# ubc-vision/quadraturefields

Measured on AMD Instinct MI355X. Metric: rays/sec at 800x800 Lego (mesh-quadrature render: ray/mesh intersection + hash-grid/MLP field + compositing), higher is better.
Workload: dtype f32; 1 GPU; Lego 800x800 (configs[1]), 1xMI355X per frame, fp32 hash-grid + tiny-MLP HIP kernels; rays_per_frame=640000, max_hits=25, triangles=983040, log2_hashmap_size=19, up_sample=1, bvh_fallback_frames=0, overflow_repaired_frames=8, reorigin_rule_redone_frames=0, camera_mismatch_frames=0, frames_in_flight=1

## Files before the change

include/qf_hip.h:

```cpp
#ifndef QF_HIP_H
#define QF_HIP_H

#include <stdint.h>

#ifdef __cplusplus
extern "C" {
#endif

#define QF_OK 0
#define QF_ERR_INVALID_ARGUMENT (-1)
#define QF_ERR_HIP (-2)
#define QF_ERR_UNSUPPORTED (-3)
#define QF_ERR_NO_DEVICE (-4)

#define QF_ABI_VERSION 6
#define QF_MAX_LEVELS 16
#define QF_MAX_LOBES 8

const char *qf_status_string(int status);
int qf_abi_version(void);
int qf_device_cu_count(void);

typedef struct qf_grid_desc {
    uint32_t n_levels;
    uint32_t n_features;
    uint32_t log2_hashmap_size;
    uint32_t base_resolution;
    float per_level_scale;
    uint32_t hashed_mask;
    uint32_t offset[QF_MAX_LEVELS + 1];
    uint32_t resolution[QF_MAX_LEVELS];
    float scale[QF_MAX_LEVELS];
} qf_grid_desc;

int qf_grid_desc_init(qf_grid_desc *desc , uint32_t n_levels,
                      uint32_t log2_hashmap_size, uint32_t base_resolution,
                      double per_level_scale);

int qf_grid_encode(const qf_grid_desc *desc , const float *table ,
                   const float *x01, int64_t n, float *out , void *stream);

int qf_grid_encode_backward(const qf_grid_desc *desc , const float *table, const float *x01,
                            const float *dfeat, int64_t n, float *grad_table, float *grad_x01, void *stream);
int64_t qf_grid_backward_workspace_bytes(int64_t n);
int qf_grid_encode_backward_ws(const qf_grid_desc *desc, const float *table, const float *x01,
                               const float *dfeat, int64_t n, float *grad_table, float *grad_x01,
                               void *workspace, int64_t workspace_bytes, void *stream);

int qf_grid_encode_double_backward(const qf_grid_desc *desc , const float *table, const float *x01,
                                   const float *dfeat, const float *v, int64_t n, float *g_dfeat,
                                   float *g_x01, float *grad_table,
                                   void *workspace ,
                                   int64_t workspace_bytes, void *stream);

int qf_grid_mlp_forward(const qf_grid_desc *grid , const float *table, const float *base_w,
                        const float *x01, int64_t n, float *out16, void *stream);

#define QF_HEAD_NONE 0
#define QF_HEAD_NGP 1
#define QF_HEAD_SG 2
#define QF_HEAD_SG_FEATURES 3

typedef struct qf_field_desc {
    qf_grid_desc grid;
    float aabb[6];
    int32_t head;
    int32_t n_lobes;
} qf_field_desc;

typedef struct qf_sg_head {
    const float *w1, *b1, *w2, *b2, *wout, *bout;
} qf_sg_head;

int qf_field_forward(const qf_field_desc *desc , const float *table,
                     const float *base_w, const float *head_ngp_w, const qf_sg_head *head_sg ,
                     const float *xyz, const float *dirs, int64_t n, const int64_t *n_device, const int32_t *order,
                     float *rgb, float *sigma, float *geo, float *features,
                     float *enc_out ,
                     void *stream);

typedef struct qf_sg_head_bf16 {
    const uint16_t *w1, *b1, *w2;
    const float *b2;
    const uint16_t *wout;
    const float *bout;
} qf_sg_head_bf16;
int qf_field_forward_bf16(const qf_field_desc *desc , const uint16_t *table ,
                          const uint16_t *base_w, const uint16_t *head_ngp_w,
                          const qf_sg_head_bf16 *head_sg , const float *xyz, const float *dirs,
                          int64_t n, const int64_t *n_device, const int32_t *order, float *rgb, float *sigma, float *geo,
                          void *stream);

typedef qf_sg_head_bf16 qf_sg_head_f16;
int qf_field_forward_f16(const qf_field_desc *desc , const uint16_t *table ,
                         const uint16_t *base_w, const uint16_t *head_ngp_w,
                         const qf_sg_head_f16 *head_sg , const float *xyz, const float *dirs,
                         int64_t n, const int64_t *n_device, const int32_t *order, float *rgb, float *sigma, float *geo,
                         void *stream);

int qf_ngp_mlp_backward(const float *enc , const float *dirs , const uint8_t *selector,
                        const float *d_rgb, const float *d_sigma, const float *base_w, const float *head_w,
                        int64_t n, float *d_enc , float *grad_base_w, float *grad_head_w,
                        void *stream);

int qf_sg_mlp_backward(const float *enc , const uint8_t *selector, const float *d_features,
                       int64_t d_stride, const float *d_sigma, const float *base_w,
                       const qf_sg_head *head , int32_t n_lobes, int64_t n, float *d_enc,
                       float *grad_base_w, const qf_sg_head *grad_head ,
                       void *stream);

int qf_sg_features_to_rgb(const float *features, int64_t feat_stride, const float *dirs,
                          int64_t n, int32_t n_lobes, float *rgb, void *stream);
int qf_sg_features_to_rgb_backward(const float *features, int64_t feat_stride, const float *dirs,
                                   const float *d_rgb, int64_t n, int32_t n_lobes, float *d_features,
                                   int64_t d_stride, void *stream);

int qf_deform_field_forward(const qf_grid_desc *grid , const float *table, float scale,
                            int32_t hidden, const float *w1, const float *b1, const float *w2,
                            const float *b2, const float *wout, const float *bout,
                            const float *xyz, int64_t n, const int64_t *n_device ,
                            const int32_t *order, float *out , float *enc_out ,
                            void *stream);

int qf_deform_field_forward_f16(const qf_grid_desc *grid , const uint16_t *table ,
                                float scale, int32_t hidden, const float *w1, const float *b1, const float *w2,
                                const float *b2, const float *wout, const float *bout,
                                const float *xyz, int64_t n, const int64_t *n_device, const int32_t *order,
                                float *out , float *enc_out , void *stream);

#define QF_ACT_RELU 0
#define QF_ACT_ELU 1
int qf_field_grid_extract(const qf_grid_desc *grid , const float *table, float scale, int32_t hidden,
                          int32_t activation, const float *w1, const float *b1, const float *w2, const float *b2,
                          const float *wout, const float *bout, const float *axis, int32_t n, int32_t x_begin,
                          int32_t x_count, int32_t pool, const float *xyz, int64_t n_points, const int64_t *n_device,
                          float *value, uint16_t *grad_norm, void *stream);

int qf_field_grid_extract_f16(const qf_grid_desc *grid , const uint16_t *table, float scale, int32_t hidden,
                              int32_t activation, const float *w1, const float *b1, const float *w2, const float *b2,
                              const float *wout, const float *bout, const float *axis, int32_t n, int32_t x_begin,
                              int32_t x_count, int32_t pool, const float *xyz, int64_t n_points,
                              const int64_t *n_device, float *value, uint16_t *grad_norm, void *stream);

int qf_deform_mlp_backward(const float *enc, const float *x01, const float *d_out, const float *w1,
                           const float *b1, const float *w2, const float *b2, const float *wout, int64_t n,
                           float *d_enc, float *d_x01, float *g_w1, float *g_b1, float *g_w2, float *g_b2,
                           float *g_wout, float *g_bout, void *stream);

int qf_adam_step(float *param, const float *grad, float *exp_avg, float *exp_avg_sq, int64_t n, double lr, double beta1,
                 double beta2, double eps, double weight_decay, int32_t maximize, int64_t step, void *stream);

int qf_apply_deformation(const float *f , float scaling, const float *dirs, const float *xyz ,
                         const float *ts , int64_t n, float *xyz_out, float *ts_out, float *dh_out,
                         void *stream);

int qf_mark_pack_boundaries(const int64_t *ridx, int64_t n, uint8_t *boundary ,
                            void *stream);
int qf_exponential_integration(const float *feats , int32_t c, const float *tau ,
                               const int64_t *seg_start, int64_t n_seg, int64_t n, int32_t exclusive,
                               float *out , float *weights , void *stream);
int qf_sum_reduce(const float *feats , int32_t c, const int64_t *seg_start,
                  int64_t n_seg, int64_t n, float *out , void *stream);

#define QF_BG_WHITE 0
#define QF_BG_BLACK 1
#define QF_BG_CUSTOM 2
#define QF_BG_NONE 3
int qf_derive_properties(const float *rgb_s , const float *sigma ,
                         const float *depth , const float *deltas ,
                         float delta_const, const int64_t *index_ray , int64_t n,
                         int64_t n_rays, int32_t bg_mode, const float *bkgd ,
                         const int32_t *sample_index, float *out_rgb, float *out_alpha, float *out_depth,
                         float *weights, void *stream);

int qf_derive_properties_backward(const float *rgb_s, const float *sigma, const float *depth,
                                  const float *deltas , float delta_const,
                                  const int64_t *index_ray, int64_t n, int64_t n_rays, int32_t bg_mode,
                                  const float *bkgd , const float *g_rgb,
                                  const float *g_alpha, const float *g_depth, float *grad_rgb_s,
                                  float *grad_sigma, float *grad_depth, void *stream);

int qf_pack_info(const int64_t *ray_indices , int64_t n, int64_t n_rays,
                 int64_t *packed_info , void *stream);
int qf_exclusive_scan(const float *x, const int64_t *packed_info, int64_t n_rays, int64_t n,
                      int32_t mode, float *out, void *stream);
int qf_accumulate_along_rays(const float *weights, const float *values ,
                             int32_t c, const int64_t *packed_info, int64_t n_rays, int64_t n,
                             float *out , void *stream);
int qf_render_from_density(const float *t_starts, const float *t_ends, const float *sigmas,
                           const float *rgbs , const int64_t *packed_info,
                           int64_t n_rays, int64_t n, const float *bkgd ,
                           float *weights, float *trans, float *alphas, float *colors,
                           float *opacities, float *depths, void *stream);

typedef struct qf_bvh qf_bvh;

int qf_bvh_create(const float *tri_verts , int64_t n_tri, qf_bvh **out);
int qf_bvh_create_ex(const float *tri_verts , int64_t n_tri, int32_t sah_depth, qf_bvh **out);
int qf_bvh_refit(qf_bvh *bvh, const float *tri_verts , int64_t n_tri);
int qf_bvh_refit_device(qf_bvh *bvh, const float *d_tri_verts , int64_t n_tri, void *stream);
void qf_bvh_destroy(qf_bvh *bvh);
int64_t qf_bvh_num_triangles(const qf_bvh *bvh);
int64_t qf_bvh_num_nodes(const qf_bvh *bvh);
int64_t qf_bvh_num_wide_nodes(const qf_bvh *bvh);
int32_t qf_bvh_max_depth(const qf_bvh *bvh);
int32_t qf_bvh_max_stack(const qf_bvh *bvh);
int qf_bvh_copy_nodes(const qf_bvh *bvh, float *nodes_host, int64_t capacity_nodes);
int qf_bvh_copy_wide_nodes(const qf_bvh *bvh, float *nodes_host, int64_t capacity_nodes);
int qf_bvh_copy_tri_ids(const qf_bvh *bvh, int32_t *ids_host, int64_t capacity);

int qf_bvh_set_min_separation(qf_bvh *bvh, float min_separation);
float qf_bvh_min_separation(const qf_bvh *bvh);

int qf_bvh_intersect(const qf_bvh *bvh, const float *rays_o, const float *rays_d, int64_t n_rays,
                     int32_t max_hits, int32_t image_width, int32_t *hit_tri, float *hit_t,
                     int32_t *hit_count, void *stream);
int qf_filter_hits(const qf_bvh *bvh, int64_t n_rays, int32_t max_hits, int32_t *hit_tri, float *hit_t,
                   int32_t *hit_count, void *stream);

typedef struct qf_camera {
    float c2w[12];
    float fx, fy;
    float cx, cy;
    int32_t width, height;
} qf_camera;
int qf_raster_intersect(qf_bvh *bvh, const qf_camera *cam , const float *rays_o,
                        const float *rays_d, int64_t n_rays, int32_t max_hits, int32_t *hit_tri, float *hit_t,
                        int32_t *hit_count, int32_t *overflow, int32_t sort_lists, int32_t cull_chunks,
                        int32_t *ray_flag, void *stream);
int qf_raster_intersect_wide(qf_bvh *bvh, const qf_camera *cam , const float *rays_o,
                             const float *rays_d, int64_t n_rays, int32_t max_hits, int32_t wide_hits,
                             int32_t *wide_tri, float *wide_t, int32_t *hit_tri, float *hit_t, int32_t *hit_count,
                             int32_t *overflow, int32_t cull_chunks, int32_t *ray_flag, void *stream);
int qf_raster_intersect_slabs(qf_bvh *bvh, const qf_camera *cam , const float *rays_o, const float *rays_d,
                              int64_t n_rays, int32_t max_hits, int32_t wide_hits, int32_t n_slabs, uint64_t *wide_keys,
                              int32_t *hit_tri, float *hit_t, int32_t *hit_count, int32_t *overflow, int32_t *ray_flag,
                              void *stream);
int qf_bvh_repair_overflow(const qf_bvh *bvh, const float *rays_o, const float *rays_d, int64_t n_rays,
                           int32_t max_hits, int32_t image_width, int32_t *hit_tri, float *hit_t,
                           int32_t *hit_count, uint64_t *keep_mask, int32_t *raw_count,
                           const int32_t *traverse_all_flag, void *stream);

int qf_grid_march_count(const float *aabb, const int32_t *resolution, const uint8_t *binaries,
                        const float *rays_o, const float *rays_d, const float *t_min, const float *t_max,
                        int64_t n_rays, float near_plane, float far_plane, float step, int32_t *count, void *stream);
int qf_grid_march_write(const float *aabb, const int32_t *resolution, const uint8_t *binaries,
                        const float *rays_o, const float *rays_d, const float *t_min, const float *t_max,
                        int64_t n_rays, float near_plane, float far_plane, float step, const int64_t *offsets,
                        float *t_starts, float *t_ends, int64_t *ray_indices, void *stream);

int qf_generate_rays(const qf_camera *cam , int32_t opengl, float *origins, float *viewdirs, void *stream);

int qf_scatter_max(const float *values, const int64_t *index, int64_t n, int64_t n_out, float *out, void *stream);

#define QF_UNTOUCHED_LAST_FACE 0
#define QF_UNTOUCHED_ZERO 1
int64_t qf_texel_positions_workspace_bytes(int64_t n_faces, int32_t height, int32_t width);
int qf_texel_positions(const double *vertices, int64_t n_vertices, const int64_t *faces, int64_t n_faces,
                       const double *uv, int32_t height, int32_t width, int32_t untouched, float *out,
                       int64_t *tri_size, void *workspace, int64_t workspace_bytes, void *stream);

int64_t qf_marching_cubes_workspace_bytes(int64_t n0, int64_t n1, int64_t n2);
int qf_marching_cubes_count(const float *volume, int64_t n0, int64_t n1, int64_t n2, float level, void *workspace,
                            int64_t workspace_bytes, int64_t *counts, void *stream);
int qf_marching_cubes_emit(const float *volume, int64_t n0, int64_t n1, int64_t n2, float level,
                           const void *workspace, int64_t workspace_bytes, float *verts, int64_t n_verts,
                           int32_t *faces, int64_t n_faces, void *stream);

#define QF_CLUSTER_AVERAGE 0
#define QF_CLUSTER_QUADRIC 1
int64_t qf_vertex_clustering_workspace_bytes(int64_t n_vertices, int64_t n_faces);
int qf_vertex_clustering_count(const double *vertices, int64_t n_vertices, const int64_t *faces, int64_t n_faces,
                               double voxel_size, void *workspace, int64_t workspace_bytes, int64_t *counts,
                               void *stream);
int qf_vertex_clustering_emit(const double *vertices, int64_t n_vertices, const int64_t *faces, int64_t n_faces,
                              double voxel_size, int contraction, void *workspace, int64_t workspace_bytes,
                              double *out_vertices, int64_t n_out_vertices, int64_t *out_faces, int64_t n_out_faces,
                              int64_t *n_fallback, void *stream);

int64_t qf_frame_offsets_temp_bytes(int64_t n_rays);
int qf_frame_offsets(const int32_t *hit_count, int64_t n_rays, int32_t max_hits, int32_t width, int32_t height,
                     int64_t *ray_offset , int64_t *tile_base , void *temp,
                     int64_t temp_bytes, const int32_t *overflow_in, const int32_t *ray_flag_in, int64_t *host_out,
                     int32_t band_rows, void *stream);
int64_t qf_banded_tile_count(int32_t width, int32_t height, int32_t band_rows);

int qf_tile_offsets(const int32_t *hit_count, int32_t max_hits, int32_t width, int32_t height, int64_t *tile_base,
                    int64_t *total, const int32_t *overflow_in, const int32_t *ray_flag_in, int64_t *host_out,
                    int32_t *zero_word , void *stream);

int qf_pack_samples(const float *rays_o, const float *rays_d, int64_t n_rays, int32_t max_hits,
                    const int32_t *hit_tri, const float *hit_t, const int32_t *hit_count,
                    const int64_t *ray_offset, float *xyz, float *dirs, int64_t *index_ray,
                    float *depth, int64_t *index_tri, float *origins, const int32_t *inverse,
                    float *xyz_c, float *dirs_c, float *depth_c , const uint64_t *keep_mask,
                    const int32_t *raw_count, float min_separation, int32_t *close_flag, void *stream);

int qf_pack_tiles(const float *rays_o, const float *rays_d, int32_t width, int32_t height, int32_t max_hits,
                  const int32_t *hit_tri, const float *hit_t, const int32_t *hit_count, const int64_t *tile_base,
                  const int64_t *total, float *xyz_c, float *dirs_c, float *depth_c, int32_t *tri_c ,
                  const uint64_t *keep_mask, const int32_t *raw_count, float min_separation, int32_t *final_count,
                  int32_t *dropped, int64_t *host_out,
                  int32_t dropped_is_zero ,
                  void *stream);

int qf_tile_totals(const int32_t *hit_count, int32_t width, int32_t height, int64_t *tile_total, void *stream);
int qf_coherent_layout(const int32_t *hit_count, const int64_t *ray_offset, const int64_t *tile_base,
                       int32_t width, int32_t height, int32_t *order, int32_t *inverse,
                       int32_t band_rows , void *stream);

int qf_composite_tiles(const float *rgb_c , const float *sigma_c , const float *depth_c ,
                       float delta_const, const int32_t *hit_count , int32_t max_hits,
                       const int64_t *tile_base, int32_t width, int32_t height, int32_t bg_mode,
                       const float *bkgd , float *out_rgb, float *out_alpha, float *out_depth,
                       float *weights_c, float *out_packed, void *stream);

int qf_row_sample_counts(const int32_t *hit_count, int32_t max_hits, int32_t width, int32_t height, float *out_rows,
                         void *stream);

#define QF_FIELD_FP32 0
#define QF_FIELD_BF16 1
#define QF_FIELD_FP16 2
typedef struct qf_frame_job {
    const qf_camera *camera;
    const float *rays_o, *rays_d;
    int64_t n_rays;
    int32_t max_hits;
    int32_t cull_chunks;
    float min_separation;
    int32_t bg_mode;
    float delta_const;
    int32_t field_precision;
    int32_t *hit_tri;
    float *hit_t;
    int32_t *hit_count;
    int32_t *final_count;
    int64_t *tile_base;
    int64_t *total;
    int64_t *host_block;
    int32_t *dropped;
    float *xyz_c, *dirs_c, *depth_c;
    int32_t *tri_c;
    const qf_field_desc *field;
    const void *table, *base_w, *head_ngp_w;
    const void *head_sg;
    float *rgb_c, *sigma_c;
    const float *bkgd;
    float *out_rgb, *out_alpha, *out_depth, *out_packed;
} qf_frame_job;
int qf_frame_render(qf_bvh *bvh, const qf_frame_job *job , void *stream);

int qf_deform_resort_tiles(const float *f_c, float scaling, const float *xyz_c, const float *dirs_c,
                           const float *depth_c, const int32_t *hit_count, int32_t max_hits, const int64_t *tile_base,
                           int64_t total , const int64_t *total_device ,
                           int32_t width, int32_t height, float *xyz_out, float *depth_out, void *stream);

int qf_resort_by_depth(const int64_t *index_ray, const float *depth, int64_t n, int64_t *perm,
                       void *stream);

int qf_resort_samples(const int64_t *index_ray, const float *depth, int64_t n, const float *points,
                      const float *origins, const float *vectors, const int64_t *index_tri,
                      int64_t *perm, float *out_points, float *out_depth, float *out_origins,
                      float *out_vectors, int64_t *out_index_tri, uint8_t *boundary, const int32_t *inverse,
                      float *out_points_c, float *out_vectors_c, void *stream);

int qf_split_layout(const int64_t *index_ray, int64_t n, int32_t width, int32_t height, int32_t *hit_count,
                    int64_t *ray_offset, int64_t *tile_base, int32_t *invalid, int32_t *order, int32_t *inverse,
                    void *stream);

int qf_mesh_update_d(const float *d , const float *w , const int64_t *index_tri, int64_t n,
                     int64_t n_faces, float *cache , int32_t *skipped , void *stream);

typedef struct qf_texture_set {
    const uint8_t *alpha;
    const uint8_t *diffuse;
    const uint8_t *colors[QF_MAX_LOBES];
    const uint8_t *lambda_axis[QF_MAX_LOBES];
    int32_t texture_size;
    int32_t n_lobes;
    int32_t sigmoid_codec;
    float lambda_thres;
} qf_texture_set;

#define QF_TEXEL_TRIANGLE_RECORD_BYTES 128
int qf_texel_records_pack(const double *vertices, const int64_t *faces, const float *uv, int64_t n_faces,
                          void *records, void *stream);
int qf_texel_indices_packed(const void *records, const float *points, const int64_t *index_tri, int64_t n,
                            int32_t texture_size, int64_t *texel, void *stream);
int qf_texture_fetch(const qf_texture_set *tex , const int64_t *texel, int64_t n,
                     float *features, void *stream);

#define QF_TEXEL_RECORD_BYTES 64
int qf_texture_pack(const qf_texture_set *tex , uint8_t *records, void *stream);
int qf_texture_shade_packed(const uint8_t *records, int32_t texture_size, int32_t n_lobes,
                            int32_t sigmoid_codec, float lambda_thres, const int64_t *texel,
                            const float *dirs, int64_t n, float *rgb, float *sigma, void *stream);
int qf_texture_shade_points(const uint8_t *records, int32_t texture_size, int32_t n_lobes, int32_t sigmoid_codec,
                            float lambda_thres, const void *triangle_records, const float *points,
                            const int64_t *index_tri, const int32_t *index_tri32, const float *dirs, int64_t n,
                            const int64_t *n_device, float *rgb, float *sigma, void *stream);

#ifdef __cplusplus
}
#endif
#endif
```

quadraturefields_amd/_C.py:

```python
import ctypes
import os
from ctypes import POINTER, Structure, c_char_p, c_double, c_float, c_int, c_int32, c_int64, c_uint8, c_uint32, c_void_p

import torch

_PKG = os.path.dirname(os.path.abspath(__file__))
LIB_PATH = os.environ.get("QF_HIP_LIBRARY") or os.path.join(_PKG, "libqf_hip.so")

QF_MAX_LEVELS = 16
QF_MAX_LOBES = 8
QF_BVH_MAX_HITS = 64
QF_TEXEL_RECORD_BYTES = 64
QF_TEXEL_TRIANGLE_RECORD_BYTES = 128
HEAD_NONE, HEAD_NGP, HEAD_SG, HEAD_SG_FEATURES = 0, 1, 2, 3
FIELD_FP32, FIELD_BF16, FIELD_FP16 = 0, 1, 2
UNTOUCHED_LAST_FACE, UNTOUCHED_ZERO = 0, 1
BG_WHITE, BG_BLACK, BG_CUSTOM, BG_NONE = 0, 1, 2, 3


class GridDesc(Structure):
    _fields_ = [
        ("n_levels", c_uint32), ("n_features", c_uint32), ("log2_hashmap_size", c_uint32),
        ("base_resolution", c_uint32), ("per_level_scale", c_float), ("hashed_mask", c_uint32),
        ("offset", c_uint32 * (QF_MAX_LEVELS + 1)), ("resolution", c_uint32 * QF_MAX_LEVELS),
        ("scale", c_float * QF_MAX_LEVELS),
    ]


class FieldDesc(Structure):
    _fields_ = [("grid", GridDesc), ("aabb", c_float * 6), ("head", c_int32), ("n_lobes", c_int32)]


class SGHead(Structure):
    _fields_ = [("w1", c_void_p), ("b1", c_void_p), ("w2", c_void_p), ("b2", c_void_p),
                ("wout", c_void_p), ("bout", c_void_p)]


class Camera(Structure):
    _fields_ = [("c2w", c_float * 12), ("fx", c_float), ("fy", c_float), ("cx", c_float), ("cy", c_float),
                ("width", c_int32), ("height", c_int32)]


class FrameJob(Structure):
    _fields_ = [("camera", c_void_p), ("rays_o", c_void_p), ("rays_d", c_void_p), ("n_rays", c_int64),
                ("max_hits", c_int32), ("cull_chunks", c_int32), ("min_separation", c_float), ("bg_mode", c_int32),
                ("delta_const", c_float), ("field_precision", c_int32),
                ("hit_tri", c_void_p), ("hit_t", c_void_p), ("hit_count", c_void_p), ("final_count", c_void_p),
                ("tile_base", c_void_p), ("total", c_void_p), ("host_block", c_void_p), ("dropped", c_void_p),
                ("xyz_c", c_void_p), ("dirs_c", c_void_p), ("depth_c", c_void_p), ("tri_c", c_void_p),
                ("field", c_void_p), ("table", c_void_p), ("base_w", c_void_p), ("head_ngp_w", c_void_p),
                ("head_sg", c_void_p), ("rgb_c", c_void_p), ("sigma_c", c_void_p),
                ("bkgd", c_void_p), ("out_rgb", c_void_p), ("out_alpha", c_void_p), ("out_depth", c_void_p),
                ("out_packed", c_void_p)]


class TextureSet(Structure):
    _fields_ = [("alpha", c_void_p), ("diffuse", c_void_p), ("colors", c_void_p * QF_MAX_LOBES),
                ("lambda_axis", c_void_p * QF_MAX_LOBES), ("texture_size", c_int32), ("n_lobes", c_int32),
                ("sigmoid_codec", c_int32), ("lambda_thres", c_float)]


_P = c_void_p
_SIGNATURES = {
    "qf_status_string": (c_char_p, [c_int]),
    "qf_frame_render": (c_int, [_P, POINTER(FrameJob), _P]),
    "qf_abi_version": (c_int, []),
    "qf_device_cu_count": (c_int, []),
    "qf_grid_desc_init": (c_int, [POINTER(GridDesc), c_uint32, c_uint32, c_uint32, c_double]),
    "qf_grid_encode": (c_int, [POINTER(GridDesc), _P, _P, c_int64, _P, _P]),
    "qf_grid_encode_backward": (c_int, [POINTER(GridDesc), _P, _P, _P, c_int64, _P, _P, _P]),
    "qf_grid_backward_workspace_bytes": (c_int64, [c_int64]),
    "qf_grid_encode_backward_ws": (c_int, [POINTER(GridDesc), _P, _P, _P, c_int64, _P, _P, _P, c_int64, _P]),
    "qf_grid_encode_double_backward": (c_int, [POINTER(GridDesc), _P, _P, _P, _P, c_int64, _P, _P, _P, _P, c_int64, _P]),
    "qf_grid_mlp_forward": (c_int, [POINTER(GridDesc), _P, _P, _P, c_int64, _P, _P]),
    "qf_field_forward": (c_int, [POINTER(FieldDesc), _P, _P, _P, POINTER(SGHead), _P, _P, c_int64, _P, _P, _P, _P, _P, _P, _P, _P]),
    "qf_field_forward_bf16": (c_int, [POINTER(FieldDesc), _P, _P, _P, POINTER(SGHead), _P, _P, c_int64, _P, _P, _P, _P, _P, _P]),
    "qf_field_forward_f16": (c_int, [POINTER(FieldDesc), _P, _P, _P, POINTER(SGHead), _P, _P, c_int64, _P, _P, _P, _P, _P, _P]),
    "qf_ngp_mlp_backward": (c_int, [_P, _P, _P, _P, _P, _P, _P, c_int64, _P, _P, _P, _P]),
    "qf_sg_mlp_backward": (c_int, [_P, _P, _P, c_int64, _P, _P, POINTER(SGHead), c_int32, c_int64, _P, _P, POINTER(SGHead), _P]),
    "qf_sg_features_to_rgb": (c_int, [_P, c_int64, _P, c_int64, c_int32, _P, _P]),
    "qf_sg_features_to_rgb_backward": (c_int, [_P, c_int64, _P, _P, c_int64, c_int32, _P, c_int64, _P]),
    "qf_deform_field_forward": (c_int, [POINTER(GridDesc), _P, c_float, c_int32, _P, _P, _P, _P, _P, _P, _P, c_int64, _P, _P, _P, _P, _P]),
    "qf_deform_field_forward_f16": (c_int, [POINTER(GridDesc), _P, c_float, c_int32, _P, _P, _P, _P, _P, _P, _P, c_int64, _P, _P, _P, _P, _P]),
    "qf_field_grid_extract": (c_int, [POINTER(GridDesc), _P, c_float, c_int32, c_int32, _P, _P, _P, _P, _P, _P, _P, c_int32, c_int32, c_int32, c_int32, _P, c_int64, _P, _P, _P, _P]),
    "qf_field_grid_extract_f16": (c_int, [POINTER(GridDesc), _P, c_float, c_int32, c_int32, _P, _P, _P, _P, _P, _P, _P, c_int32, c_int32, c_int32, c_int32, _P, c_int64, _P, _P, _P, _P]),
    "qf_deform_mlp_backward": (c_int, [_P, _P, _P, _P, _P, _P, _P, _P, c_int64, _P, _P, _P, _P, _P, _P, _P, _P, _P]),
    "qf_adam_step": (c_int, [_P, _P, _P, _P, c_int64, c_double, c_double, c_double, c_double, c_double, c_int32, c_int64, _P]),
    "qf_apply_deformation": (c_int, [_P, c_float, _P, _P, _P, c_int64, _P, _P, _P, _P]),
    "qf_mark_pack_boundaries": (c_int, [_P, c_int64, _P, _P]),
    "qf_exponential_integration": (c_int, [_P, c_int32, _P, _P, c_int64, c_int64, c_int32, _P, _P, _P]),
    "qf_sum_reduce": (c_int, [_P, c_int32, _P, c_int64, c_int64, _P, _P]),
    "qf_derive_properties": (c_int, [_P, _P, _P, _P, c_float, _P, c_int64, c_int64, c_int32, _P, _P, _P, _P, _P, _P, _P]),
    "qf_deform_resort_tiles": (c_int, [_P, c_float, _P, _P, _P, _P, c_int32, _P, c_int64, _P, c_int32, c_int32, _P, _P, _P]),
    "qf_composite_tiles": (c_int, [_P, _P, _P, c_float, _P, c_int32, _P, c_int32, c_int32, c_int32, _P, _P, _P, _P, _P, _P, _P]),
    "qf_row_sample_counts": (c_int, [_P, c_int32, c_int32, c_int32, _P, _P]),
    "qf_derive_properties_backward": (c_int, [_P, _P, _P, _P, c_float, _P, c_int64, c_int64, c_int32, _P, _P, _P, _P, _P, _P, _P, _P]),
    "qf_pack_info": (c_int, [_P, c_int64, c_int64, _P, _P]),
    "qf_exclusive_scan": (c_int, [_P, _P, c_int64, c_int64, c_int32, _P, _P]),
    "qf_accumulate_along_rays": (c_int, [_P, _P, c_int32, _P, c_int64, c_int64, _P, _P]),
    "qf_render_from_density": (c_int, [_P, _P, _P, _P, _P, c_int64, c_int64, _P, _P, _P, _P, _P, _P, _P, _P]),
    "qf_bvh_create": (c_int, [_P, c_int64, POINTER(c_void_p)]),
    "qf_bvh_create_ex": (c_int, [_P, c_int64, c_int32, POINTER(c_void_p)]),
    "qf_bvh_refit": (c_int, [_P, _P, c_int64]),
    "qf_bvh_refit_device": (c_int, [_P, _P, c_int64, _P]),
    "qf_bvh_num_wide_nodes": (c_int64, [_P]),
    "qf_bvh_max_stack": (c_int32, [_P]),
    "qf_bvh_copy_wide_nodes": (c_int, [_P, _P, c_int64]),
    "qf_bvh_set_min_separation": (c_int, [_P, c_float]),
    "qf_bvh_min_separation": (c_float, [_P]),
    "qf_filter_hits": (c_int, [_P, c_int64, c_int32, _P, _P, _P, _P]),
    "qf_bvh_destroy": (None, [_P]),
    "qf_bvh_num_triangles": (c_int64, [_P]),
    "qf_bvh_num_nodes": (c_int64, [_P]),
    "qf_bvh_max_depth": (c_int32, [_P]),
    "qf_bvh_copy_nodes": (c_int, [_P, _P, c_int64]),
    "qf_bvh_copy_tri_ids": (c_int, [_P, _P, c_int64]),
    "qf_bvh_intersect": (c_int, [_P, _P, _P, c_int64, c_int32, c_int32, _P, _P, _P, _P]),
    "qf_bvh_repair_overflow": (c_int, [_P, _P, _P, c_int64, c_int32, c_int32, _P, _P, _P, _P, _P, _P, _P]),
    "qf_raster_intersect": (c_int, [_P, POINTER(Camera), _P, _P, c_int64, c_int32, _P, _P, _P, _P, c_int32, c_int32, _P, _P]),
    "qf_raster_intersect_wide": (c_int, [_P, POINTER(Camera), _P, _P, c_int64, c_int32, c_int32, _P, _P, _P, _P, _P, _P, c_int32, _P,
                                         _P]),
    "qf_raster_intersect_slabs": (c_int, [_P, POINTER(Camera), _P, _P, c_int64, c_int32, c_int32, c_int32, _P, _P, _P, _P, _P, _P,
                                          _P]),
    "qf_grid_march_count": (c_int, [POINTER(c_float), POINTER(c_int32), _P, _P, _P, _P, _P, c_int64, c_float, c_float,
                                    c_float, _P, _P]),
    "qf_grid_march_write": (c_int, [POINTER(c_float), POINTER(c_int32), _P, _P, _P, _P, _P, c_int64, c_float, c_float,
                                    c_float, _P, _P, _P, _P, _P]),
    "qf_generate_rays": (c_int, [POINTER(Camera), c_int32, _P, _P, _P]),
    "qf_scatter_max": (c_int, [_P, _P, c_int64, c_int64, _P, _P]),
    "qf_texel_positions_workspace_bytes": (c_int64, [c_int64, c_int32, c_int32]),
    "qf_texel_positions": (c_int, [_P, c_int64, _P, c_int64, _P, c_int32, c_int32, c_int32, _P, _P, _P, c_int64, _P]),
    "qf_marching_cubes_workspace_bytes": (c_int64, [c_int64, c_int64, c_int64]),
    "qf_marching_cubes_count": (c_int, [_P, c_int64, c_int64, c_int64, c_float, _P, c_int64, _P, _P]),
    "qf_marching_cubes_emit": (c_int, [_P, c_int64, c_int64, c_int64, c_float, _P, c_int64, _P, c_int64, _P, c_int64, _P]),
    "qf_vertex_clustering_workspace_bytes": (c_int64, [c_int64, c_int64]),
    "qf_vertex_clustering_count": (c_int, [_P, c_int64, _P, c_int64, c_double, _P, c_int64, _P, _P]),
    "qf_vertex_clustering_emit": (c_int, [_P, c_int64, _P, c_int64, c_double, c_int, _P, c_int64, _P, c_int64, _P, c_int64,
                                          _P, _P]),
    "qf_frame_offsets_temp_bytes": (c_int64, [c_int64]),
    "qf_frame_offsets": (c_int, [_P, c_int64, c_int32, c_int32, c_int32, _P, _P, _P, c_int64, _P, _P, _P, c_int32, _P]),
    "qf_banded_tile_count": (c_int64, [c_int32, c_int32, c_int32]),
    "qf_tile_offsets": (c_int, [_P, c_int32, c_int32, c_int32, _P, _P, _P, _P, _P, _P, _P]),
    "qf_pack_tiles": (c_int, [_P, _P, c_int32, c_int32, c_int32, _P, _P, _P, _P, _P, _P, _P, _P, _P, _P, _P, c_float, _P, _P, _P, c_int32, _P]),
    "qf_pack_samples": (c_int, [_P, _P, c_int64, c_int32, _P, _P, _P, _P, _P, _P, _P, _P, _P, _P, _P, _P, _P, _P, _P, _P, c_float, _P, _P]),
    "qf_tile_totals": (c_int, [_P, c_int32, c_int32, _P, _P]),
    "qf_coherent_layout": (c_int, [_P, _P, _P, c_int32, c_int32, _P, _P, c_int32, _P]),
    "qf_resort_by_depth": (c_int, [_P, _P, c_int64, _P, _P]),
    "qf_resort_samples": (c_int, [_P, _P, c_int64, _P, _P, _P, _P, _P, _P, _P, _P, _P, _P, _P, _P, _P, _P, _P]),
    "qf_split_layout": (c_int, [_P, c_int64, c_int32, c_int32, _P, _P, _P, _P, _P, _P, _P]),
    "qf_mesh_update_d": (c_int, [_P, _P, _P, c_int64, c_int64, _P, _P, _P]),
    "qf_texel_records_pack": (c_int, [_P, _P, _P, c_int64, _P, _P]),
    "qf_texel_indices_packed": (c_int, [_P, _P, _P, c_int64, c_int32, _P, _P]),
    "qf_texture_fetch": (c_int, [POINTER(TextureSet), _P, c_int64, _P, _P]),
    "qf_texture_pack": (c_int, [POINTER(TextureSet), _P, _P]),
    "qf_texture_shade_packed": (c_int, [_P, c_int32, c_int32, c_int32, c_float, _P, _P, c_int64, _P, _P, _P]),
    "qf_texture_shade_points": (c_int, [_P, c_int32, c_int32, c_int32, c_float, _P, _P, _P, _P, _P, c_int64, _P, _P, _P, _P]),
}
EXPORTED_SYMBOLS = tuple(_SIGNATURES)
ABI_VERSION = 6

_lib = None


def lib() -> ctypes.CDLL:
    global _lib
    if _lib is None:
        if not os.path.exists(LIB_PATH):
            raise RuntimeError(
                f"{LIB_PATH} is missing: build it with `python -m quadraturefields_amd.build` "
                "(hipcc --offload-arch=gfx950).  quadraturefields_amd has no CPU fallback.")
        handle = ctypes.CDLL(LIB_PATH)
        for name, (restype, argtypes) in _SIGNATURES.items():
            fn = getattr(handle, name)
            fn.restype = restype
            fn.argtypes = argtypes
        version = handle.qf_abi_version()
        experiment = os.environ.get("QF_HIP_LIBRARY_EXPERIMENT") == "1" and version == ABI_VERSION + 1000
        if version != ABI_VERSION and not experiment:
            raise RuntimeError(f"{LIB_PATH}: ABI version {version}, expected {ABI_VERSION} (an experiment build "
                               "reports +1000 and is only loaded with QF_HIP_LIBRARY_EXPERIMENT=1)")
        _lib = handle
    return _lib


class QFError(RuntimeError):
    pass


def check(status: int, what: str = "") -> None:
    if status != 0:
        msg = lib().qf_status_string(status).decode()
        if status == -1:
            raise ValueError(f"{what}: {msg}")
        raise QFError(f"{what}: {msg} (status {status})")


def ptr(t, dtype=None, device_required: bool = True):
    if t is None:
        return None
    if not isinstance(t, torch.Tensor):
        raise TypeError("expected a torch.Tensor")
    if dtype is not None and t.dtype != dtype:
        raise TypeError(f"expected dtype {dtype}, got {t.dtype}")
    if not t.is_contiguous():
        raise ValueError("tensor must be contiguous")
    if device_required and not t.is_cuda:
        raise RuntimeError("quadraturefields_amd kernels need tensors on the HIP device (no CPU fallback)")
    return c_void_p(t.data_ptr())


_OWNER_PID = os.getpid()
_FORKED = False


def _after_fork_in_child():
    global _FORKED
    _FORKED = True


os.register_at_fork(after_in_child=_after_fork_in_child)


def raw_stream() -> int:
    return torch._C._cuda_getCurrentRawStream(torch._C._cuda_getDevice())


def stream():
    if _FORKED:
        raise RuntimeError(
            "quadraturefields_amd was called from a forked child process (a DataLoader worker?): the HIP kernels must run "
            f"in the process that imported the package (pid {_OWNER_PID}).  Use num_workers=0 for the device path, or a "
            "'spawn' multiprocessing context.")
    return c_void_p(raw_stream())


def resolve_device(device) -> torch.device:
    dev = torch.device(device)
    if dev.type == "cuda" and dev.index is None:
        dev = torch.device("cuda", torch.cuda.current_device())
    return dev


def f32c(t: torch.Tensor) -> torch.Tensor:
    return t.to(torch.float32).contiguous()


def i64c(t: torch.Tensor) -> torch.Tensor:
    return t.to(torch.int64).contiguous()


def make_grid_desc(n_levels: int, log2_hashmap_size: int, base_resolution: int, per_level_scale: float) -> GridDesc:
    d = GridDesc()
    check(lib().qf_grid_desc_init(ctypes.byref(d), n_levels, log2_hashmap_size, base_resolution,
                                  float(per_level_scale)), "qf_grid_desc_init")
    return d


def grid_encode_backward(desc, table, x01, dfeat, n: int, grad_table, grad_x01) -> None:
    ws, ws_bytes = None, 0
    if grad_table is not None and n >= (1 << 15):
        ws_bytes = int(lib().qf_grid_backward_workspace_bytes(n))
        ws = torch.empty((ws_bytes,), dtype=torch.uint8, device=x01.device)
    check(lib().qf_grid_encode_backward_ws(desc, ptr(table), ptr(x01), ptr(dfeat), n, ptr(grad_table), ptr(grad_x01),
                                           ptr(ws), ws_bytes, stream()), "qf_grid_encode_backward")
```

quadraturefields_amd/csrc/frame.cpp:

```cpp
#include "qf_common.h"

extern "C" int qf_frame_render(qf_bvh *bvh, const qf_frame_job *job, void *stream)
{
    if (!bvh || !job || !job->camera) return QF_ERR_INVALID_ARGUMENT;
    const qf_frame_job &j = *job;
    const int32_t w = j.camera->width, h = j.camera->height;
    if (w < 1 || h < 1 || j.n_rays != (int64_t)w * h || j.max_hits < 1) return QF_ERR_INVALID_ARGUMENT;
    if (!j.rays_o || !j.rays_d || !j.hit_tri || !j.hit_t || !j.hit_count || !j.final_count || !j.tile_base || !j.total ||
        !j.dropped || !j.xyz_c || !j.dirs_c || !j.depth_c)
        return QF_ERR_INVALID_ARGUMENT;
    if (j.field_precision < QF_FIELD_FP32 || j.field_precision > QF_FIELD_FP16) return QF_ERR_INVALID_ARGUMENT;
    if (j.field) {
        const qf_field_desc &f = *j.field;
        if (!j.rgb_c || !j.sigma_c || !j.table || !j.base_w) return QF_ERR_INVALID_ARGUMENT;
        if (f.head == QF_HEAD_NGP) {
            if (!j.head_ngp_w) return QF_ERR_INVALID_ARGUMENT;
        } else if (f.head == QF_HEAD_SG) {
            if (!j.head_sg) return QF_ERR_INVALID_ARGUMENT;
            if (j.field_precision == QF_FIELD_FP32) {
                const qf_sg_head *s = static_cast<const qf_sg_head *>(j.head_sg);
                if (!s->w1 || !s->b1 || !s->w2 || !s->b2 || !s->wout || !s->bout) return QF_ERR_INVALID_ARGUMENT;
            } else {
                const qf_sg_head_bf16 *s = static_cast<const qf_sg_head_bf16 *>(j.head_sg);
                if (!s->w1 || !s->b1 || !s->w2 || !s->b2 || !s->wout || !s->bout) return QF_ERR_INVALID_ARGUMENT;
            }
            if (f.n_lobes < 1 || f.n_lobes > QF_MAX_LOBES) return QF_ERR_UNSUPPORTED;
        } else {
            return QF_ERR_INVALID_ARGUMENT;
        }
        for (int k = 0; k < 3; ++k)
            if (!(f.aabb[3 + k] > f.aabb[k])) return QF_ERR_INVALID_ARGUMENT;
        if (j.bg_mode < 0 || j.bg_mode > 3) return QF_ERR_INVALID_ARGUMENT;
        if (!j.out_packed && (!j.out_rgb || !j.out_alpha || !j.out_depth)) return QF_ERR_INVALID_ARGUMENT;
        if (j.bg_mode == QF_BG_CUSTOM && !j.bkgd) return QF_ERR_INVALID_ARGUMENT;
    }
    const int64_t cap = j.n_rays * (int64_t)j.max_hits;
    int32_t *overflow = j.hit_count + j.n_rays;
    int rc = qf_raster_intersect(bvh, j.camera, j.rays_o, j.rays_d, j.n_rays, j.max_hits, j.hit_tri, j.hit_t, j.hit_count,
                                 overflow, j.tri_c ? 0 : 2 , j.cull_chunks,
                                 overflow + 1, stream);
    if (rc != QF_OK) return rc;
    rc = qf_bvh_repair_overflow(bvh, j.rays_o, j.rays_d, j.n_rays, j.max_hits, w, j.hit_tri, j.hit_t, j.hit_count, nullptr,
                                nullptr, overflow + 1, stream);
    if (rc != QF_OK) return rc;
    rc = qf_tile_offsets(j.hit_count, j.max_hits, w, h, j.tile_base, j.total, overflow, overflow + 1, j.host_block, j.dropped,
                         stream);
    if (rc != QF_OK) return rc;
    rc = qf_pack_tiles(j.rays_o, j.rays_d, w, h, j.max_hits, j.hit_tri, j.hit_t, j.hit_count, j.tile_base, j.total, j.xyz_c,
                       j.dirs_c, j.depth_c, j.tri_c, nullptr, nullptr, j.min_separation, j.final_count, j.dropped, nullptr, 1,
                       stream);
    if (rc != QF_OK) return rc;
    if (!j.field) return QF_OK;
    if (j.field_precision == QF_FIELD_FP32) {
        rc = qf_field_forward(j.field, static_cast<const float *>(j.table), static_cast<const float *>(j.base_w),
                              static_cast<const float *>(j.head_ngp_w), static_cast<const qf_sg_head *>(j.head_sg),
                              j.xyz_c, j.dirs_c, cap, j.total, nullptr, j.rgb_c, j.sigma_c, nullptr, nullptr, nullptr,
                              stream);
    } else {
        auto fwd = j.field_precision == QF_FIELD_BF16 ? qf_field_forward_bf16 : qf_field_forward_f16;
        rc = fwd(j.field, static_cast<const uint16_t *>(j.table), static_cast<const uint16_t *>(j.base_w),
                 static_cast<const uint16_t *>(j.head_ngp_w), static_cast<const qf_sg_head_bf16 *>(j.head_sg), j.xyz_c,
                 j.dirs_c, cap, j.total, nullptr, j.rgb_c, j.sigma_c, nullptr, stream);
    }
    if (rc != QF_OK) return rc;
    return qf_composite_tiles(j.rgb_c, j.sigma_c, j.depth_c, j.delta_const, j.final_count, j.max_hits, j.tile_base, w, h,
                              j.bg_mode, j.bkgd, j.out_rgb, j.out_alpha, j.out_depth, nullptr, j.out_packed, stream);
}
```

quadraturefields_amd/csrc/raster.hip:

```cpp
#include <type_traits>

#include "exact_common.h"

#pragma clang fp contract(off)

namespace {

struct RasterCam {
    float r00, r01, r02, r10, r11, r12, r20, r21, r22;
    float cx, cy, cz;
    float fx, fy, px0, py0;
    int w, h;
};

constexpr float kRasterGuard = 0.25f;

struct SlabArgs {
    float t_lo, t_hi;
    int stop_at;
    uint64_t *keys;
    const float4 *ray_rec;
};

struct TriSetup {
    int x0, x1, y0, y1;
    bool use_edges;
    float ea[3], eb[3], ec[3];
};

__device__ __forceinline__ bool tri_setup(const float4 a, const float4 b, const float4 c, const RasterCam &cam, TriSetup &s)
{
    float minx = INFINITY, maxx = -INFINITY, miny = INFINITY, maxy = -INFINITY;
    int behind = 0;
    const float4 vs[3] = {a, b, c};
    float sxs[3], sys[3];
#pragma unroll
    for (int k = 0; k < 3; ++k) {
        const float dx = vs[k].x - cam.cx, dy = vs[k].y - cam.cy, dz = vs[k].z - cam.cz;
        const float xc = cam.r00 * dx + cam.r10 * dy + cam.r20 * dz;
        const float yc = cam.r01 * dx + cam.r11 * dy + cam.r21 * dz;
        const float zc = cam.r02 * dx + cam.r12 * dy + cam.r22 * dz;
        const float zv = -zc;
        if (!(zv > 1e-6f)) { ++behind; sxs[k] = sys[k] = 0.0f; continue; }
        const float sx = cam.fx * (xc / zv) + cam.px0;
        const float sy = -cam.fy * (yc / zv) + cam.py0;
        sxs[k] = sx; sys[k] = sy;
        minx = fminf(minx, sx); maxx = fmaxf(maxx, sx);
        miny = fminf(miny, sy); maxy = fmaxf(maxy, sy);
    }
    if (behind == 3) return false;
    s.use_edges = false;
    if (behind > 0) {
        s.x0 = 0; s.y0 = 0; s.x1 = cam.w - 1; s.y1 = cam.h - 1;
    } else {
        s.x0 = (int)fmaxf(floorf(minx - kRasterGuard), 0.0f);
        s.y0 = (int)fmaxf(floorf(miny - kRasterGuard), 0.0f);
        s.x1 = (int)fminf(ceilf(maxx + kRasterGuard), (float)(cam.w - 1));
        s.y1 = (int)fminf(ceilf(maxy + kRasterGuard), (float)(cam.h - 1));
        if (!(maxx + kRasterGuard >= 0.0f) || !(maxy + kRasterGuard >= 0.0f) ||
            !(minx - kRasterGuard <= (float)(cam.w - 1)) || !(miny - kRasterGuard <= (float)(cam.h - 1)))
            return false;
        const float area2 = (sxs[1] - sxs[0]) * (sys[2] - sys[0]) - (sys[1] - sys[0]) * (sxs[2] - sxs[0]);
        if (fabsf(area2) > 1e-2f) {
            s.use_edges = true;
            const float sgn = area2 > 0.0f ? 1.0f : -1.0f;
#pragma unroll
            for (int k = 0; k < 3; ++k) {
                const int k1 = (k + 1) % 3;
                const float ex = sxs[k1] - sxs[k], ey = sys[k1] - sys[k];
                s.ea[k] = -sgn * ey;
                s.eb[k] = sgn * ex;
                s.ec[k] = -(s.ea[k] * sxs[k] + s.eb[k] * sys[k]) + (kRasterGuard + 0.05f) * (fabsf(ex) + fabsf(ey)) + 1e-3f;
            }
        }
    }
    return true;
}

template <int kRasterLanes, bool kWide, bool kSlab = false>
__device__ __forceinline__ void raster_triangle(const float4 *__restrict__ tris, int64_t tri_i, int sub, const RasterCam &cam,
                                                const float *__restrict__ rays_o, const float *__restrict__ rays_d,
                                                int max_hits, int32_t *__restrict__ hit_tri, float *__restrict__ hit_t,
                                                int32_t *__restrict__ hit_count, int32_t *__restrict__ overflow,
                                                const bool cam_origin, const SlabArgs slab = SlabArgs())
{
    const float4 a = tris[tri_i * 3 + 0], b = tris[tri_i * 3 + 1], c = tris[tri_i * 3 + 2];
    const int id = __float_as_int(a.w);
    TriSetup ts;
    if (!tri_setup(a, b, c, cam, ts)) return;
    const int x0 = ts.x0, x1 = ts.x1, y0 = ts.y0, y1 = ts.y1;
    const bool use_edges = ts.use_edges;
    const float *ea = ts.ea, *eb = ts.eb, *ec = ts.ec;
    const int bw = x1 - x0 + 1;
    const int total = bw * (y1 - y0 + 1);
    int px = x0 + sub % bw, py = y0 + sub / bw;
    for (int q = sub; q < total; q += kRasterLanes) {
        const int cx_ = px, cy_ = py;
        px += kRasterLanes;
        while (px > x1) { px -= bw; ++py; }
        if (use_edges) {
            const float fx_ = (float)cx_, fy_ = (float)cy_;
            if (ea[0] * fx_ + eb[0] * fy_ + ec[0] < 0.0f || ea[1] * fx_ + eb[1] * fy_ + ec[1] < 0.0f ||
                ea[2] * fx_ + eb[2] * fy_ + ec[2] < 0.0f)
                continue;
        }
        const int64_t ray = (int64_t)cy_ * cam.w + cx_;
        float dx, dy, dz;
        if (kSlab && slab.ray_rec) {
            const float4 rr = slab.ray_rec[ray];
            if (__float_as_int(rr.w) >= slab.stop_at) continue;
            dx = rr.x; dy = rr.y; dz = rr.z;
        } else {
            dx = rays_d[ray * 3]; dy = rays_d[ray * 3 + 1]; dz = rays_d[ray * 3 + 2];
        }
        float ox = cam.cx, oy = cam.cy, oz = cam.cz;
        if (!cam_origin) { ox = rays_o[ray * 3]; oy = rays_o[ray * 3 + 1]; oz = rays_o[ray * 3 + 2]; }
        asm volatile("" : "+v"(ox), "+v"(oy), "+v"(oz), "+v"(dx), "+v"(dy), "+v"(dz));
        float t;
        if (!mt_hit(a, b, c, ox, oy, oz, dx, dy, dz, &t)) continue;
        if (kSlab) {
            if (!(t >= slab.t_lo && t < slab.t_hi)) continue;
            const int slot = atomicAdd(&hit_count[ray], 1);
            if (slot < max_hits) slab.keys[(int64_t)slot * ((int64_t)cam.w * cam.h) + ray] = hit_key(t, id);
            else atomicAdd(overflow, 1);
            continue;
        }
        const int slot = atomicAdd(&hit_count[ray], 1);
        if (slot < max_hits) {
            const int64_t at = kWide ? (int64_t)slot * ((int64_t)cam.w * cam.h) + ray : ray * max_hits + slot;
            hit_t[at] = t;
            if (hit_tri) hit_tri[at] = id;
        } else {
            atomicAdd(overflow, 1);
        }
    }
}

template <int kRasterLanes, bool kWide>
__global__ __launch_bounds__(256) void raster_kernel(const float4 *__restrict__ tris, int64_t n_tri, RasterCam cam,
                                                     const float *__restrict__ rays_o, const float *__restrict__ rays_d,
                                                     int max_hits, int32_t *__restrict__ hit_tri, float *__restrict__ hit_t,
                                                     int32_t *__restrict__ hit_count, int32_t *__restrict__ overflow,
                                                     const int32_t *__restrict__ ray_flag)
{
    const int64_t gid = (int64_t)blockIdx.x * blockDim.x + threadIdx.x;
    const int64_t tri_i = gid / kRasterLanes;
    const int sub = (int)(gid % kRasterLanes);
    if (tri_i >= n_tri) return;
    if (ray_flag && *ray_flag) return;
    const bool cam_origin = ray_flag != nullptr;
    raster_triangle<kRasterLanes, kWide>(tris, tri_i, sub, cam, rays_o, rays_d, max_hits, hit_tri, hit_t, hit_count, overflow,
                                         cam_origin);
}

constexpr float kRayPixelTol = 0.02f;
constexpr float kRayUnitTol = 1e-4f;

__device__ __forceinline__ void camera_rays_check(const uint32_t *__restrict__ o_bits, const float *__restrict__ rays_d,
                                                  int64_t n_rays, const RasterCam &cam, int32_t *__restrict__ flag,
                                                  int64_t first, int64_t stride)
{
    const uint32_t c0 = __float_as_uint(cam.cx), c1 = __float_as_uint(cam.cy), c2 = __float_as_uint(cam.cz);
    bool bad = false;
    for (int64_t r = first; r < n_rays; r += stride) {
        const uint32_t o0 = o_bits[r * 3], o1 = o_bits[r * 3 + 1], o2 = o_bits[r * 3 + 2];
        const float dx = rays_d[r * 3], dy = rays_d[r * 3 + 1], dz = rays_d[r * 3 + 2];
        bad = bad || o0 != c0 || o1 != c1 || o2 != c2;
        const float xc = cam.r00 * dx + cam.r10 * dy + cam.r20 * dz;
        const float yc = cam.r01 * dx + cam.r11 * dy + cam.r21 * dz;
        const float zv = -(cam.r02 * dx + cam.r12 * dy + cam.r22 * dz);
        const float sx = cam.fx * (xc / zv) + cam.px0, sy = -cam.fy * (yc / zv) + cam.py0;
        const float px = (float)(int)(r % cam.w), py = (float)(int)(r / cam.w);
        bad = bad || !(zv > 0.0f) || !(fabsf(sx - px) <= kRayPixelTol) || !(fabsf(sy - py) <= kRayPixelTol) ||
              !(fabsf(dx * dx + dy * dy + dz * dz - 1.0f) <= kRayUnitTol);
    }
    if (bad) *flag = 1;
}

__global__ void camera_rays_check_kernel(const uint32_t *__restrict__ o_bits, const float *__restrict__ rays_d, int64_t n_rays,
                                         RasterCam cam, int32_t *__restrict__ flag)
{
    camera_rays_check(o_bits, rays_d, n_rays, cam, flag, (int64_t)blockIdx.x * blockDim.x + threadIdx.x,
                      (int64_t)gridDim.x * blockDim.x);
}

constexpr int kCullChunk = 64;

__global__ __launch_bounds__(256) void chunk_boxes_kernel(const float4 *__restrict__ tris, int64_t n_tri, int n_chunks,
                                                          float4 *__restrict__ boxes)
{
    const int chunk = (int)(((int64_t)blockIdx.x * blockDim.x + threadIdx.x) >> 6), lane = threadIdx.x & 63;
    if (chunk >= n_chunks) return;
    const int64_t t = (int64_t)chunk * kCullChunk + lane;
    float lo[3] = {INFINITY, INFINITY, INFINITY}, hi[3] = {-INFINITY, -INFINITY, -INFINITY};
    if (t < n_tri) {
#pragma unroll
        for (int k = 0; k < 3; ++k) {
            const float4 v = tris[t * 3 + k];
            lo[0] = fminf(lo[0], v.x); lo[1] = fminf(lo[1], v.y); lo[2] = fminf(lo[2], v.z);
            hi[0] = fmaxf(hi[0], v.x); hi[1] = fmaxf(hi[1], v.y); hi[2] = fmaxf(hi[2], v.z);
        }
    }
#pragma unroll
    for (int off = 32; off > 0; off >>= 1) {
#pragma unroll
        for (int k = 0; k < 3; ++k) {
            lo[k] = fminf(lo[k], __shfl_xor(lo[k], off, 64));
            hi[k] = fmaxf(hi[k], __shfl_xor(hi[k], off, 64));
        }
    }
    if (lane == 0) {
        boxes[chunk * 2 + 0] = make_float4(lo[0], lo[1], lo[2], 0.0f);
        boxes[chunk * 2 + 1] = make_float4(hi[0], hi[1], hi[2], 0.0f);
    }
}

__global__ void cull_chunks_kernel(const float4 *__restrict__ boxes, int n_chunks, RasterCam cam, int32_t *__restrict__ visible,
                                   int32_t *__restrict__ counters, int parity, const uint32_t *__restrict__ o_bits,
                                   const float *__restrict__ rays_d, int64_t n_rays, int32_t *__restrict__ ray_flag)
{
    const int chunk = blockIdx.x * blockDim.x + threadIdx.x;
    if (chunk == 0) counters[parity ^ 1] = 0;
    if (ray_flag) camera_rays_check(o_bits, rays_d, n_rays, cam, ray_flag, chunk, (int64_t)gridDim.x * blockDim.x);
    if (chunk >= n_chunks) return;
    const float4 lo = boxes[chunk * 2], hi = boxes[chunk * 2 + 1];
    if (!(lo.x <= hi.x)) return;
    float minx = INFINITY, maxx = -INFINITY, miny = INFINITY, maxy = -INFINITY;
    bool keep = false;
#pragma unroll
    for (int k = 0; k < 8; ++k) {
        const float dx = ((k & 1) ? hi.x : lo.x) - cam.cx, dy = ((k & 2) ? hi.y : lo.y) - cam.cy, dz = ((k & 4) ? hi.z : lo.z) - cam.cz;
        const float xc = cam.r00 * dx + cam.r10 * dy + cam.r20 * dz;
        const float yc = cam.r01 * dx + cam.r11 * dy + cam.r21 * dz;
        const float zc = cam.r02 * dx + cam.r12 * dy + cam.r22 * dz;
        const float zv = -zc;
        if (!(zv > 1e-4f)) { keep = true; continue; }
        const float sx = cam.fx * (xc / zv) + cam.px0, sy = -cam.fy * (yc / zv) + cam.py0;
        minx = fminf(minx, sx); maxx = fmaxf(maxx, sx);
        miny = fminf(miny, sy); maxy = fmaxf(maxy, sy);
    }
    const float g = kRasterGuard + 1.0f;
    if (!keep)
        keep = (maxx + g >= 0.0f) && (maxy + g >= 0.0f) && (minx - g <= (float)(cam.w - 1)) && (miny - g <= (float)(cam.h - 1));
    if (keep) visible[atomicAdd(&counters[parity], 1)] = chunk;
}

template <int kRasterLanes, bool kWide>
__global__ __launch_bounds__(256) void raster_culled_kernel(const float4 *__restrict__ tris, int64_t n_tri, RasterCam cam,
                                                            const float *__restrict__ rays_o, const float *__restrict__ rays_d,
                                                            int max_hits, int32_t *__restrict__ hit_tri, float *__restrict__ hit_t,
                                                            int32_t *__restrict__ hit_count, int32_t *__restrict__ overflow,
                                                            const int32_t *__restrict__ visible, const int32_t *__restrict__ n_visible,
                                                            const int32_t *__restrict__ ray_flag)
{
    if (ray_flag && *ray_flag) return;
    const bool cam_origin = ray_flag != nullptr;
    constexpr int kTrisPerBlock = 256 / kRasterLanes;
    constexpr int kBlocksPerChunk = kCullChunk / kTrisPerBlock;
    const int n_items = *n_visible * kBlocksPerChunk;
    const int sub = threadIdx.x % kRasterLanes;
    for (int item = blockIdx.x; item < n_items; item += gridDim.x) {
        const int chunk = visible[item / kBlocksPerChunk];
        const int64_t tri_i = (int64_t)chunk * kCullChunk + (item % kBlocksPerChunk) * kTrisPerBlock + threadIdx.x / kRasterLanes;
        if (tri_i < n_tri)
            raster_triangle<kRasterLanes, kWide>(tris, tri_i, sub, cam, rays_o, rays_d, max_hits, hit_tri, hit_t, hit_count, overflow,
                                                 cam_origin);
    }
}

constexpr int kMaxSlabs = 16;

struct SlabCtl {
    uint32_t dist_min_bits, dist_max_bits;
    int32_t n_visible;
    int32_t slab_count[kMaxSlabs];
};

__device__ __forceinline__ void slab_range(const SlabCtl *ctl, int n_slabs, float *lo, float *width)
{
    const float dmin = __uint_as_float(ctl->dist_min_bits) * 0.999f, dmax = __uint_as_float(ctl->dist_max_bits) * 1.001f;
    *lo = dmin;
    *width = fmaxf(dmax - dmin, 1e-12f) / (float)n_slabs;
}

__device__ __forceinline__ void slab_edges(const SlabCtl *ctl, int n_slabs, int j, float *t_lo, float *t_hi)
{
#pragma clang fp contract(off)
    float lo, w;
    slab_range(ctl, n_slabs, &lo, &w);
    *t_lo = j == 0 ? -INFINITY : lo + (float)j * w;
    *t_hi = j == n_slabs - 1 ? INFINITY : lo + (float)(j + 1) * w;
}

__global__ void slab_init_kernel(SlabCtl *ctl)
{
    ctl->dist_min_bits = 0x7f800000u;
    ctl->dist_max_bits = 0u;
    ctl->n_visible = 0;
    for (int j = 0; j < kMaxSlabs; ++j) ctl->slab_count[j] = 0;
}

__global__ void slab_cull_kernel(const float4 *__restrict__ boxes, int n_chunks, RasterCam cam, int32_t *__restrict__ visible,
                                 float2 *__restrict__ range, SlabCtl *ctl)
{
    const int chunk = blockIdx.x * blockDim.x + threadIdx.x;
    if (chunk >= n_chunks) return;
    const float4 lo = boxes[chunk * 2], hi = boxes[chunk * 2 + 1];
    if (!(lo.x <= hi.x)) return;
    float minx = INFINITY, maxx = -INFINITY, miny = INFINITY, maxy = -INFINITY;
    bool keep = false;
#pragma unroll
    for (int k = 0; k < 8; ++k) {
        const float dx = ((k & 1) ? hi.x : lo.x) - cam.cx, dy = ((k & 2) ? hi.y : lo.y) - cam.cy, dz = ((k & 4) ? hi.z : lo.z) - cam.cz;
        const float xc = cam.r00 * dx + cam.r10 * dy + cam.r20 * dz;
        const float yc = cam.r01 * dx + cam.r11 * dy + cam.r21 * dz;
        const float zc = cam.r02 * dx + cam.r12 * dy + cam.r22 * dz;
        const float zv = -zc;
        if (!(zv > 1e-4f)) { keep = true; continue; }
        const float sx = cam.fx * (xc / zv) + cam.px0, sy = -cam.fy * (yc / zv) + cam.py0;
        minx = fminf(minx, sx); maxx = fmaxf(maxx, sx);
        miny = fminf(miny, sy); maxy = fmaxf(maxy, sy);
    }
    const float g = kRasterGuard + 1.0f;
    if (!keep)
        keep = (maxx + g >= 0.0f) && (maxy + g >= 0.0f) && (minx - g <= (float)(cam.w - 1)) && (miny - g <= (float)(cam.h - 1));
    if (!keep) return;
    const float nx = fmaxf(fmaxf(lo.x - cam.cx, cam.cx - hi.x), 0.0f), ny = fmaxf(fmaxf(lo.y - cam.cy, cam.cy - hi.y), 0.0f);
    const float nz = fmaxf(fmaxf(lo.z - cam.cz, cam.cz - hi.z), 0.0f);
    const float fx = fmaxf(fabsf(lo.x - cam.cx), fabsf(hi.x - cam.cx)), fy = fmaxf(fabsf(lo.y - cam.cy), fabsf(hi.y - cam.cy));
    const float fz = fmaxf(fabsf(lo.z - cam.cz), fabsf(hi.z - cam.cz));
    const float dmin = sqrtf(nx * nx + ny * ny + nz * nz) * 0.9999f, dmax = sqrtf(fx * fx + fy * fy + fz * fz) * 1.0001f + 1e-30f;
    visible[atomicAdd(&ctl->n_visible, 1)] = chunk;
    range[chunk] = make_float2(dmin, dmax);
    atomicMin(&ctl->dist_min_bits, __float_as_uint(dmin));
    atomicMax(&ctl->dist_max_bits, __float_as_uint(dmax));
}

__global__ __launch_bounds__(256) void slab_assign_kernel(const int32_t *__restrict__ visible, const float2 *__restrict__ range,
                                                          SlabCtl *ctl, int n_slabs, int n_chunks, int32_t *__restrict__ lists)
{
    __shared__ int s_cnt[kMaxSlabs], s_base[kMaxSlabs];
    if (threadIdx.x < kMaxSlabs) s_cnt[threadIdx.x] = 0;
    __syncthreads();
    const int e = blockIdx.x * blockDim.x + threadIdx.x;
    int chunk = -1, j0 = 0, j1 = -1;
    if (e < ctl->n_visible) {
        chunk = visible[e];
        const float2 r = range[chunk];
        const float dlo = r.x * 0.999f, dhi = r.y * 1.001f;
        j0 = n_slabs;
        for (int j = 0; j < n_slabs; ++j) {
            float t_lo, t_hi;
            slab_edges(ctl, n_slabs, j, &t_lo, &t_hi);
            if (t_hi > dlo && t_lo <= dhi) { j0 = j < j0 ? j : j0; j1 = j; }
        }
        for (int j = j0; j <= j1; ++j) atomicAdd(&s_cnt[j], 1);
    }
    __syncthreads();
    if (threadIdx.x < n_slabs) s_base[threadIdx.x] = s_cnt[threadIdx.x] ? atomicAdd(&ctl->slab_count[threadIdx.x], s_cnt[threadIdx.x]) : 0;
    __syncthreads();
    for (int j = j0; j <= j1; ++j) lists[(int64_t)j * n_chunks + atomicAdd(&s_base[j], 1)] = chunk;
}

__global__ void slab_ray_records_kernel(const float *__restrict__ rays_d, const int32_t *__restrict__ hit_count, int64_t n,
                                        float4 *__restrict__ rec)
{
    for (int64_t i = (int64_t)blockIdx.x * blockDim.x + threadIdx.x; i < n; i += (int64_t)gridDim.x * blockDim.x)
        rec[i] = make_float4(rays_d[i * 3], rays_d[i * 3 + 1], rays_d[i * 3 + 2], __int_as_float(hit_count[i]));
}

template <int kRasterLanes>
__global__ __launch_bounds__(256) void raster_slab_kernel(const float4 *__restrict__ tris, int64_t n_tri, RasterCam cam,
                                                          const float *__restrict__ rays_o, const float *__restrict__ rays_d,
                                                          int capacity, uint64_t *__restrict__ keys, int32_t *__restrict__ hit_count,
                                                          int32_t *__restrict__ overflow, const int32_t *__restrict__ list,
                                                          const SlabCtl *__restrict__ ctl, int slab_j, int n_slabs, int stop_at,
                                                          const float4 *__restrict__ ray_rec,
                                                          const int32_t *__restrict__ ray_flag)
{
    if (ray_flag && *ray_flag) return;
    const bool cam_origin = ray_flag != nullptr;
    constexpr int kTrisPerBlock = 256 / kRasterLanes;
    constexpr int kBlocksPerChunk = kCullChunk / kTrisPerBlock;
    const int n_items = ctl->slab_count[slab_j] * kBlocksPerChunk;
    SlabArgs sa;
    slab_edges(ctl, n_slabs, slab_j, &sa.t_lo, &sa.t_hi);
    sa.stop_at = stop_at;
    sa.keys = keys;
    sa.ray_rec = ray_rec;
    const int sub = threadIdx.x % kRasterLanes;
    for (int item = blockIdx.x; item < n_items; item += gridDim.x) {
        const int chunk = list[item / kBlocksPerChunk];
        const int64_t tri_i = (int64_t)chunk * kCullChunk + (item % kBlocksPerChunk) * kTrisPerBlock + threadIdx.x / kRasterLanes;
        if (tri_i < n_tri)
            raster_triangle<kRasterLanes, true, true>(tris, tri_i, sub, cam, rays_o, rays_d, capacity, nullptr, nullptr,
                                                      hit_count, overflow, cam_origin, sa);
    }
}

constexpr int kSelectBlock = 64;
constexpr int kSelectHeadroom = 8;
__host__ __device__ inline int select_capacity(int max_hits, int wide, float min_sep)
{
    const int cap = min_sep > 0.0f ? max_hits + kSelectHeadroom : max_hits;
    return cap < wide ? cap : wide;
}
__device__ __forceinline__ void write_row_from_keys(const uint64_t *lk, int count, float *row_t, int32_t *row_i)
{
    int i = 0;
    for (; i + 4 <= count; i += 4) {
        f32x4u t4;
        i32x4u i4;
#pragma unroll
        for (int e = 0; e < 4; ++e) {
            const uint64_t k = lk[(i + e) * kSelectBlock];
            t4[e] = key_t(k);
            i4[e] = key_id(k);
        }
        *reinterpret_cast<f32x4u *>(row_t + i) = t4;
        *reinterpret_cast<i32x4u *>(row_i + i) = i4;
    }
    for (; i < count; ++i) {
        const uint64_t k = lk[i * kSelectBlock];
        row_t[i] = key_t(k);
        row_i[i] = key_id(k);
    }
}

template <bool kKeys>
__global__ __launch_bounds__(kSelectBlock) void select_nearest_kernel(int64_t n_rays, int wide, int max_hits, float min_sep,
                                                                      const int32_t *__restrict__ wide_tri,
                                                                      const float *__restrict__ wide_t,
                                                                      const uint64_t *__restrict__ wide_key,
                                                                      int32_t *__restrict__ hit_tri, float *__restrict__ hit_t,
                                                                      int32_t *__restrict__ hit_count)
{
    extern __shared__ __attribute__((aligned(8))) unsigned char select_lds[];
    const int cap = select_capacity(max_hits, wide, min_sep);
    uint64_t *lk = reinterpret_cast<uint64_t *>(select_lds) + threadIdx.x;
    const int64_t r = (int64_t)blockIdx.x * kSelectBlock + threadIdx.x;
    if (r >= n_rays) return;
    const int cnt = hit_count[r];
    if (cnt > wide) return;
    float *row_t = hit_t + r * max_hits;
    int32_t *row_i = hit_tri + r * max_hits;
    if (cnt <= max_hits) {
        constexpr int kCopy = 8;
        for (int i0 = 0; i0 < cnt; i0 += kCopy) {
            float tb[kCopy];
            int ib[kCopy];
#pragma unroll
            for (int u = 0; u < kCopy; ++u) {
                const int i = i0 + u < cnt ? i0 + u : cnt - 1;
                if (kKeys) {
                    const uint64_t k = wide_key[(int64_t)i * n_rays + r];
                    tb[u] = key_t(k);
                    ib[u] = key_id(k);
                } else {
                    tb[u] = wide_t[(int64_t)i * n_rays + r];
                    ib[u] = wide_tri[(int64_t)i * n_rays + r];
                }
            }
#pragma unroll
            for (int q = 0; q < kCopy / 4; ++q) {
                if (i0 + 4 * q + 4 <= cnt) {
                    *reinterpret_cast<f32x4u *>(row_t + i0 + 4 * q) = (f32x4u){tb[4 * q], tb[4 * q + 1], tb[4 * q + 2], tb[4 * q + 3]};
                    *reinterpret_cast<i32x4u *>(row_i + i0 + 4 * q) = (i32x4u){ib[4 * q], ib[4 * q + 1], ib[4 * q + 2], ib[4 * q + 3]};
                } else {
#pragma unroll
                    for (int e = 0; e < 4; ++e)
                        if (i0 + 4 * q + e < cnt) { row_t[i0 + 4 * q + e] = tb[4 * q + e]; row_i[i0 + 4 * q + e] = ib[4 * q + e]; }
                }
            }
        }
        return;
    }
    const int held = cnt < cap ? cnt : cap;
    constexpr int kBatch = 8;
    int n = 0;
    uint64_t max_key = 0;
    for (int i0 = 0; i0 < cnt; i0 += kBatch) {
        uint64_t kb[kBatch];
#pragma unroll
        for (int u = 0; u < kBatch; ++u) {
            const int i = i0 + u < cnt ? i0 + u : cnt - 1;
            if (kKeys) kb[u] = wide_key[(int64_t)i * n_rays + r];
            else kb[u] = hit_key(wide_t[(int64_t)i * n_rays + r], wide_tri[(int64_t)i * n_rays + r]);
        }
#pragma unroll
        for (int u = 0; u < kBatch; ++u) {
            if (i0 + u >= cnt) break;
            const uint64_t key = kb[u];
            int m;
            if (n < held) {
                m = n;
                ++n;
            } else {
                if (!(key < max_key)) continue;
                m = n - 1;
            }
            int lo = 0, hi = m;
            while (lo < hi) {
                const int mid = (lo + hi) >> 1;
                if (lk[mid * kSelectBlock] < key) lo = mid + 1;
                else hi = mid;
            }
            int j = m - 1;
            for (; j - 3 >= lo; j -= 4) {
                const uint64_t a0 = lk[j * kSelectBlock], a1 = lk[(j - 1) * kSelectBlock], a2 = lk[(j - 2) * kSelectBlock],
                               a3 = lk[(j - 3) * kSelectBlock];
                lk[(j + 1) * kSelectBlock] = a0;
                lk[j * kSelectBlock] = a1;
                lk[(j - 1) * kSelectBlock] = a2;
                lk[(j - 2) * kSelectBlock] = a3;
            }
            for (; j >= lo; --j) lk[(j + 1) * kSelectBlock] = lk[j * kSelectBlock];
            lk[lo * kSelectBlock] = key;
            max_key = lk[(n - 1) * kSelectBlock];
        }
    }
    if (min_sep <= 0.0f) {
        write_row_from_keys(lk, max_hits, row_t, row_i);
        hit_count[r] = max_hits;
        return;
    }
    float last_t = key_t(lk[0]);
    int kept = 1;
    for (int i = 1; i < held && kept < max_hits; ++i) {
        const uint64_t k = lk[i * kSelectBlock];
        const float t = key_t(k);
        if (!(t > last_t + min_sep)) continue;
        last_t = t;
        lk[kept * kSelectBlock] = k;
        ++kept;
    }
    if (kept < max_hits && cnt > held) return;
    write_row_from_keys(lk, kept, row_t, row_i);
    hit_count[r] = kept;
}

constexpr int kFilterRays = 128;
__global__ __launch_bounds__(kFilterRays) void filter_hits_kernel(int64_t n_rays, int max_hits, float min_sep,
                                                                  int32_t *__restrict__ hit_tri, float *__restrict__ hit_t,
                                                                  int32_t *__restrict__ hit_count)
{
    extern __shared__ __attribute__((aligned(16))) unsigned char filter_smem[];
    const int K = max_hits, Kp = max_hits | 1;
    float *s_t = reinterpret_cast<float *>(filter_smem);
    int32_t *s_tri = reinterpret_cast<int32_t *>(s_t + kFilterRays * Kp);
    const int tid = threadIdx.x;
    const int64_t ray0 = (int64_t)blockIdx.x * kFilterRays;
    const int nr = (int)((n_rays - ray0) < kFilterRays ? (n_rays - ray0) : kFilterRays);
    for (int i = tid; i < nr * K; i += kFilterRays) {
        const int r = i / K, k = i - r * K;
        s_t[r * Kp + k] = hit_t[ray0 * K + i];
        s_tri[r * Kp + k] = hit_tri[ray0 * K + i];
    }
    __syncthreads();
    if (tid < nr) {
        int cnt = hit_count[ray0 + tid];
        if (cnt > K) cnt = K;
        float *row_t = s_t + tid * Kp;
        int32_t *row_i = s_tri + tid * Kp;
        if (K <= 32) {
            if (cnt > 1) sort_row_32<true>(row_t, row_i, cnt);
        } else {
            for (int i = 1; i < cnt; ++i) {
                const float t = row_t[i];
                const int id = row_i[i];
                int j = i - 1;
                while (j >= 0 && hit_less(t, id, row_t[j], row_i[j])) { row_t[j + 1] = row_t[j]; row_i[j + 1] = row_i[j]; --j; }
                row_t[j + 1] = t;
                row_i[j + 1] = id;
            }
        }
        if (min_sep > 0.0f && cnt > 1) {
            int kept = 1;
            float last_t = row_t[0];
            for (int i = 1; i < cnt; ++i) {
                const float t = row_t[i];
                if (t > last_t + min_sep) { row_t[kept] = t; row_i[kept] = row_i[i]; ++kept; last_t = t; }
            }
            cnt = kept;
        }
        for (int i = cnt; i < K; ++i) { row_t[i] = INFINITY; row_i[i] = -1; }
        hit_count[ray0 + tid] = cnt;
    }
    __syncthreads();
    for (int i = tid; i < nr * K; i += kFilterRays) {
        const int r = i / K, k = i - r * K;
        hit_t[ray0 * K + i] = s_t[r * Kp + k];
        hit_tri[ray0 * K + i] = s_tri[r * Kp + k];
    }
}

}

static int filter_launch(int64_t n_rays, int32_t max_hits, float min_sep, int32_t *hit_tri, float *hit_t,
                         int32_t *hit_count, hipStream_t st)
{
    const int Kp = max_hits | 1;
    const size_t lds = (size_t)kFilterRays * Kp * 8;
    const int64_t blocks = qf_div_up(n_rays, kFilterRays);
    if (blocks > 0x7fffffff) return QF_ERR_UNSUPPORTED;
    hipLaunchKernelGGL(filter_hits_kernel, dim3((unsigned)blocks), dim3(kFilterRays), lds, st, n_rays, (int)max_hits, min_sep,
                       hit_tri, hit_t, hit_count);
    QF_LAUNCH_CHECK();
    return QF_OK;
}

extern "C" int qf_filter_hits(const qf_bvh *bvh, int64_t n_rays, int32_t max_hits, int32_t *hit_tri, float *hit_t,
                              int32_t *hit_count, void *stream)
{
    if (!bvh || n_rays < 0 || max_hits < 1 || max_hits > kMaxHits) return QF_ERR_INVALID_ARGUMENT;
    if (n_rays == 0 || !(bvh->min_sep > 0.0f)) return QF_OK;
    if (!hit_tri || !hit_t || !hit_count) return QF_ERR_INVALID_ARGUMENT;
    return filter_launch(n_rays, max_hits, bvh->min_sep, hit_tri, hit_t, hit_count, qf_stream(stream));
}

static RasterCam make_raster_cam(const qf_camera *cam)
{
    RasterCam rc;
    const float *m = cam->c2w;
    rc.r00 = m[0]; rc.r01 = m[1]; rc.r02 = m[2]; rc.cx = m[3];
    rc.r10 = m[4]; rc.r11 = m[5]; rc.r12 = m[6]; rc.cy = m[7];
    rc.r20 = m[8]; rc.r21 = m[9]; rc.r22 = m[10]; rc.cz = m[11];
    rc.fx = cam->fx; rc.fy = cam->fy;
    rc.px0 = cam->cx - 0.5f;
    rc.py0 = cam->cy - 0.5f;
    rc.w = cam->width; rc.h = cam->height;
    return rc;
}

static int ensure_chunk_boxes(qf_bvh *bvh, hipStream_t st)
{
    const int64_t n_chunks = qf_div_up(bvh->n_tri, kCullChunk);
    if (n_chunks > 0x3fffffff) return QF_ERR_UNSUPPORTED;
    if (!bvh->d_chunk_box) {
        QF_HIP_TRY(hipMalloc((void **)&bvh->d_chunk_box, (size_t)n_chunks * 2 * sizeof(float4)));
        QF_HIP_TRY(hipMalloc((void **)&bvh->d_visible, (size_t)(n_chunks + 2) * sizeof(int32_t)));
        QF_HIP_TRY(hipMemsetAsync(bvh->d_visible, 0, 2 * sizeof(int32_t), st));
        bvh->chunk_dirty = true;
        bvh->cull_parity = 0;
    }
    if (bvh->chunk_dirty) {
        hipLaunchKernelGGL(chunk_boxes_kernel, dim3((unsigned)qf_div_up(n_chunks * 64, 256)), dim3(256), 0, st,
                           reinterpret_cast<const float4 *>(bvh->d_tris), bvh->n_tri, (int)n_chunks,
                           reinterpret_cast<float4 *>(bvh->d_chunk_box));
        QF_LAUNCH_CHECK();
        bvh->chunk_dirty = false;
    }
    return QF_OK;
}

static int raster_zero(int64_t n_rays, int32_t *hit_count, int32_t *overflow, int32_t *origin_flag, hipStream_t st)
{
    int64_t words = n_rays;
    bool ovf_done = false, flag_done = origin_flag == nullptr;
    if (overflow == hit_count + words) { ++words; ovf_done = true; }
    if (ovf_done && origin_flag == hit_count + words) { ++words; flag_done = true; }
    QF_HIP_TRY(hipMemsetAsync(hit_count, 0, (size_t)words * sizeof(int32_t), st));
    if (!ovf_done) QF_HIP_TRY(hipMemsetAsync(overflow, 0, sizeof(int32_t), st));
    if (!flag_done) QF_HIP_TRY(hipMemsetAsync(origin_flag, 0, sizeof(int32_t), st));
    return QF_OK;
}

static int raster_lanes(int64_t n_rays, int64_t n_tri)
{
    const int64_t pixels_per_tri = n_rays / n_tri;
    return pixels_per_tri > 64 ? 16 : (pixels_per_tri > 8 ? 8 : 4);
}

template <typename F>
static void with_lanes(int lanes, F &&f)
{
    switch (lanes) {
    case 16: f(std::integral_constant<int, 16>()); break;
    case 8: f(std::integral_constant<int, 8>()); break;
    default: f(std::integral_constant<int, 4>()); break;
    }
}

static unsigned chunk_grid(int64_t n_chunks, int lanes)
{
    const int64_t items = n_chunks * (kCullChunk * lanes / 256);
    const int64_t cap = (int64_t)qf_cu_count_cached() * 8;
    return (unsigned)(items < cap ? items : cap);
}

static void camera_check_launch(const RasterCam &rc, const float *rays_o, const float *rays_d, int64_t n_rays,
                                int32_t *origin_flag, hipStream_t st)
{
    if (origin_flag)
        hipLaunchKernelGGL(camera_rays_check_kernel, dim3(qf_grid_1d(n_rays, 256)), dim3(256), 0, st,
                           reinterpret_cast<const uint32_t *>(rays_o), rays_d, n_rays, rc, origin_flag);
}

static int raster_launch(qf_bvh *bvh, const qf_camera *cam, const float *rays_o, const float *rays_d, int64_t n_rays,
                         int capacity, bool wide, int32_t *hit_tri, float *hit_t, int32_t *hit_count, int32_t *overflow,
                         int32_t *origin_flag, bool cull, hipStream_t st, bool skip_ids = false)
{
    if (skip_ids) hit_tri = nullptr;
    const int rc_zero = raster_zero(n_rays, hit_count, overflow, origin_flag, st);
    if (rc_zero != QF_OK) return rc_zero;
    if (bvh->n_tri == 0) return QF_OK;
    const RasterCam rc = make_raster_cam(cam);
    const float4 *tris4 = reinterpret_cast<const float4 *>(bvh->d_tris);
    const int lanes = raster_lanes(n_rays, bvh->n_tri);
    const int64_t blocks = qf_div_up(bvh->n_tri * lanes, 256);
    if (blocks > 0x7fffffff) return QF_ERR_UNSUPPORTED;
    if (cull) {
        const int64_t n_chunks = qf_div_up(bvh->n_tri, kCullChunk);
        const int rc_boxes = ensure_chunk_boxes(bvh, st);
        if (rc_boxes != QF_OK) return rc_boxes;
        float4 *boxes = reinterpret_cast<float4 *>(bvh->d_chunk_box);
        int32_t *counters = bvh->d_visible, *visible = bvh->d_visible + 2;
        const int parity = bvh->cull_parity;
        bvh->cull_parity ^= 1;
        hipLaunchKernelGGL(cull_chunks_kernel, dim3((unsigned)qf_div_up(n_chunks, 256)), dim3(256), 0, st, boxes,
                           (int)n_chunks, rc, visible, counters, parity, reinterpret_cast<const uint32_t *>(rays_o), rays_d,
                           n_rays, origin_flag);
        QF_LAUNCH_CHECK();
        with_lanes(lanes, [&](auto L) {
            auto *kernel = wide ? raster_culled_kernel<decltype(L)::value, true> : raster_culled_kernel<decltype(L)::value, false>;
            hipLaunchKernelGGL(kernel, dim3(chunk_grid(n_chunks, lanes)), dim3(256), 0, st, tris4, bvh->n_tri, rc, rays_o, rays_d,
                               capacity, hit_tri, hit_t, hit_count, overflow, visible, counters + parity, origin_flag);
        });
    } else {
        camera_check_launch(rc, rays_o, rays_d, n_rays, origin_flag, st);
        QF_LAUNCH_CHECK();
        with_lanes(lanes, [&](auto L) {
            auto *kernel = wide ? raster_kernel<decltype(L)::value, true> : raster_kernel<decltype(L)::value, false>;
            hipLaunchKernelGGL(kernel, dim3((unsigned)blocks), dim3(256), 0, st, tris4, bvh->n_tri, rc, rays_o, rays_d, capacity,
                               hit_tri, hit_t, hit_count, overflow, origin_flag);
        });
    }
    QF_LAUNCH_CHECK();
    return QF_OK;
}

static bool raster_args_ok(const qf_bvh *bvh, const qf_camera *cam, int64_t n_rays, int32_t max_hits)
{
    if (!bvh || !cam || n_rays < 0 || max_hits < 1 || max_hits > kMaxHits) return false;
    if (cam->width < 1 || cam->height < 1 || (int64_t)cam->width * cam->height != n_rays) return false;
    return cam->fx > 0.0f && cam->fy > 0.0f;
}

extern "C" int qf_raster_intersect(qf_bvh *bvh, const qf_camera *cam, const float *rays_o, const float *rays_d,
                                   int64_t n_rays, int32_t max_hits, int32_t *hit_tri, float *hit_t, int32_t *hit_count,
                                   int32_t *overflow, int32_t sort_lists, int32_t cull_chunks, int32_t *origin_flag,
                                   void *stream)
{
    if (!raster_args_ok(bvh, cam, n_rays, max_hits)) return QF_ERR_INVALID_ARGUMENT;
    if (!rays_o || !rays_d || !hit_tri || !hit_t || !hit_count || !overflow) return QF_ERR_INVALID_ARGUMENT;
    if (sort_lists < 0 || sort_lists > 2) return QF_ERR_INVALID_ARGUMENT;
    hipStream_t st = qf_stream(stream);
    const int rc = raster_launch(bvh, cam, rays_o, rays_d, n_rays, (int)max_hits, false, hit_tri, hit_t, hit_count, overflow,
                                 origin_flag, cull_chunks != 0, st, sort_lists == 2);
    if (rc != QF_OK) return rc;
    if (sort_lists == 1 && n_rays > 0) return filter_launch(n_rays, max_hits, bvh->min_sep, hit_tri, hit_t, hit_count, st);
    return QF_OK;
}

extern "C" int qf_raster_intersect_wide(qf_bvh *bvh, const qf_camera *cam, const float *rays_o, const float *rays_d,
                                        int64_t n_rays, int32_t max_hits, int32_t wide_hits, int32_t *wide_tri,
                                        float *wide_t, int32_t *hit_tri, float *hit_t, int32_t *hit_count,
                                        int32_t *overflow, int32_t cull_chunks, int32_t *origin_flag, void *stream)
{
    if (!raster_args_ok(bvh, cam, n_rays, max_hits)) return QF_ERR_INVALID_ARGUMENT;
    if (wide_hits < max_hits || wide_hits > 4096) return QF_ERR_INVALID_ARGUMENT;
    if (!rays_o || !rays_d || !wide_tri || !wide_t || !hit_tri || !hit_t || !hit_count || !overflow)
        return QF_ERR_INVALID_ARGUMENT;
    hipStream_t st = qf_stream(stream);
    const int rc = raster_launch(bvh, cam, rays_o, rays_d, n_rays, (int)wide_hits, true, wide_tri, wide_t, hit_count, overflow,
                                 origin_flag, cull_chunks != 0, st);
    if (rc != QF_OK) return rc;
    if (n_rays == 0) return QF_OK;
    const size_t lds = (size_t)select_capacity(max_hits, wide_hits, bvh->min_sep) * kSelectBlock * 2 * sizeof(float);
    hipLaunchKernelGGL(select_nearest_kernel<false>, dim3((unsigned)qf_div_up(n_rays, kSelectBlock)), dim3(kSelectBlock), lds, st,
                       n_rays, (int)wide_hits, (int)max_hits, bvh->min_sep, wide_tri, wide_t, (const uint64_t *)nullptr, hit_tri,
                       hit_t, hit_count);
    QF_LAUNCH_CHECK();
    return QF_OK;
}

extern "C" int qf_raster_intersect_slabs(qf_bvh *bvh, const qf_camera *cam, const float *rays_o, const float *rays_d,
                                         int64_t n_rays, int32_t max_hits, int32_t wide_hits, int32_t n_slabs,
                                         uint64_t *wide_keys, int32_t *hit_tri, float *hit_t, int32_t *hit_count,
                                         int32_t *overflow, int32_t *origin_flag, void *stream)
{
    if (!raster_args_ok(bvh, cam, n_rays, max_hits)) return QF_ERR_INVALID_ARGUMENT;
    if (n_slabs < 2 || n_slabs > kMaxSlabs) return QF_ERR_INVALID_ARGUMENT;
    const int sel_cap = select_capacity(max_hits, wide_hits, bvh->min_sep);
    if (wide_hits <= sel_cap + 1 || wide_hits > 4096) return QF_ERR_INVALID_ARGUMENT;
    if (!rays_o || !rays_d || !wide_keys || !hit_tri || !hit_t || !hit_count || !overflow) return QF_ERR_INVALID_ARGUMENT;
    hipStream_t st = qf_stream(stream);
    const int rc_zero = raster_zero(n_rays, hit_count, overflow, origin_flag, st);
    if (rc_zero != QF_OK) return rc_zero;
    if (n_rays == 0 || bvh->n_tri == 0) return QF_OK;
    const int rc_boxes = ensure_chunk_boxes(bvh, st);
    if (rc_boxes != QF_OK) return rc_boxes;
    const int64_t n_chunks = qf_div_up(bvh->n_tri, kCullChunk);
    if (!bvh->d_slab_range) {
        QF_HIP_TRY(hipMalloc((void **)&bvh->d_slab_range, (size_t)n_chunks * sizeof(float2)));
        QF_HIP_TRY(hipMalloc((void **)&bvh->d_slab_lists, (size_t)n_chunks * kMaxSlabs * sizeof(int32_t)));
        QF_HIP_TRY(hipMalloc((void **)&bvh->d_slab_ctl, sizeof(SlabCtl)));
    }
    const RasterCam rc = make_raster_cam(cam);
    const float4 *tris4 = reinterpret_cast<const float4 *>(bvh->d_tris);
    const float4 *boxes = reinterpret_cast<const float4 *>(bvh->d_chunk_box);
    int32_t *visible = bvh->d_visible + 2;
    float2 *range = reinterpret_cast<float2 *>(bvh->d_slab_range);
    SlabCtl *ctl = reinterpret_cast<SlabCtl *>(bvh->d_slab_ctl);
    camera_check_launch(rc, rays_o, rays_d, n_rays, origin_flag, st);
    hipLaunchKernelGGL(slab_init_kernel, dim3(1), dim3(1), 0, st, ctl);
    hipLaunchKernelGGL(slab_cull_kernel, dim3((unsigned)qf_div_up(n_chunks, 256)), dim3(256), 0, st, boxes, (int)n_chunks, rc,
                       visible, range, ctl);
    hipLaunchKernelGGL(slab_assign_kernel, dim3((unsigned)qf_div_up(n_chunks, 256)), dim3(256), 0, st, visible, range, ctl,
                       (int)n_slabs, (int)n_chunks, bvh->d_slab_lists);
    QF_LAUNCH_CHECK();
    const int lanes = raster_lanes(n_rays, bvh->n_tri);
    const unsigned grid = chunk_grid(n_chunks, lanes);
    const int stop_at = sel_cap + 1;
    if (bvh->slab_snapshot_rays < n_rays) {
        const int64_t grown = bvh->slab_snapshot_rays * 2 > n_rays ? bvh->slab_snapshot_rays * 2 : n_rays;
        if (bvh->d_slab_snapshot) (void)hipFree(bvh->d_slab_snapshot);
        bvh->d_slab_snapshot = nullptr;
        bvh->slab_snapshot_rays = 0;
        QF_HIP_TRY(hipMalloc((void **)&bvh->d_slab_snapshot, (size_t)grown * sizeof(float4)));
        bvh->slab_snapshot_rays = grown;
    }
    float4 *snapshot = reinterpret_cast<float4 *>(bvh->d_slab_snapshot);
    for (int j = 0; j < n_slabs; ++j) {
        if (j > 0) {
            hipLaunchKernelGGL(slab_ray_records_kernel, dim3(qf_grid_1d(n_rays, 256)), dim3(256), 0, st, rays_d, hit_count,
                               n_rays, snapshot);
            QF_LAUNCH_CHECK();
        }
        const int32_t *list = bvh->d_slab_lists + (int64_t)j * n_chunks;
        with_lanes(lanes, [&](auto L) {
            hipLaunchKernelGGL(raster_slab_kernel<decltype(L)::value>, dim3(grid), dim3(256), 0, st, tris4, bvh->n_tri, rc, rays_o,
                               rays_d, (int)wide_hits, wide_keys, hit_count, overflow, list, ctl, j, (int)n_slabs, stop_at,
                               j == 0 ? (const float4 *)nullptr : snapshot, origin_flag);
        });
    }
    QF_LAUNCH_CHECK();
    const size_t lds = (size_t)sel_cap * kSelectBlock * 2 * sizeof(float);
    hipLaunchKernelGGL(select_nearest_kernel<true>, dim3((unsigned)qf_div_up(n_rays, kSelectBlock)), dim3(kSelectBlock), lds, st,
                       n_rays, (int)wide_hits, (int)max_hits, bvh->min_sep, (const int32_t *)nullptr, (const float *)nullptr,
                       wide_keys, hit_tri, hit_t, hit_count);
    QF_LAUNCH_CHECK();
    return QF_OK;
}
```

quadraturefields_amd/csrc/sample_pack.hip:

```cpp
#include "exact_common.h"

#pragma clang fp contract(off)

namespace {

template <int kN, bool kTri>
__device__ __forceinline__ void load_sort_row(const float *__restrict__ g_t, const int32_t *__restrict__ g_i, int K,
                                              int cnt, int deepest, float *row_t, int32_t *row_i)
{
    float t[kN];
    int32_t id[kN];
#pragma unroll
    for (int j = 0; j < kN / 4; ++j) {
        f32x4u v = {INFINITY, INFINITY, INFINITY, INFINITY};
        i32x4u w = {-1, -1, -1, -1};
        if (4 * j < deepest) {
            if (4 * j + 3 < K) {
                v = *reinterpret_cast<const f32x4u *>(g_t + 4 * j);
                if (kTri) w = *reinterpret_cast<const i32x4u *>(g_i + 4 * j);
            } else {
#pragma unroll
                for (int e = 0; e < 3; ++e)
                    if (4 * j + e < K) {
                        v[e] = g_t[4 * j + e];
                        if (kTri) w[e] = g_i[4 * j + e];
                    }
            }
        }
#pragma unroll
        for (int e = 0; e < 4; ++e) { t[4 * j + e] = v[e]; id[4 * j + e] = w[e]; }
    }
    if (kTri) {
        uint64_t key[kN];
#pragma unroll
        for (int k = 0; k < kN; ++k) key[k] = k < cnt ? hit_key(t[k], id[k]) : ~0ull;
#pragma unroll
        for (int k = 2; k <= kN; k <<= 1) {
#pragma unroll
            for (int i = 0; i < kN; ++i) {
                const int l = i ^ (k - 1);
                if (l > i) { const uint64_t a = key[i], b = key[l]; key[i] = a < b ? a : b; key[l] = a < b ? b : a; }
            }
#pragma unroll
            for (int j = k >> 2; j > 0; j >>= 1) {
#pragma unroll
                for (int i = 0; i < kN; ++i) {
                    const int l = i ^ j;
                    if (l > i) { const uint64_t a = key[i], b = key[l]; key[i] = a < b ? a : b; key[l] = a < b ? b : a; }
                }
            }
        }
#pragma unroll
        for (int k = 0; k < kN; ++k)
            if (k < cnt) { row_t[k] = key_t(key[k]); row_i[k] = key_id(key[k]); }
    } else {
#pragma unroll
        for (int k = 0; k < kN; ++k) t[k] = k < cnt ? t[k] : INFINITY;
#pragma unroll
        for (int k = 2; k <= kN; k <<= 1) {
#pragma unroll
            for (int i = 0; i < kN; ++i) {
                const int l = i ^ (k - 1);
                if (l > i) { const float a = t[i], b = t[l]; t[i] = fminf(a, b); t[l] = fmaxf(a, b); }
            }
#pragma unroll
            for (int j = k >> 2; j > 0; j >>= 1) {
#pragma unroll
                for (int i = 0; i < kN; ++i) {
                    const int l = i ^ j;
                    if (l > i) { const float a = t[i], b = t[l]; t[i] = fminf(a, b); t[l] = fmaxf(a, b); }
                }
            }
        }
#pragma unroll
        for (int k = 0; k < kN; ++k)
            if (k < cnt) row_t[k] = t[k];
    }
}

constexpr int kPackRays = 128;

__device__ __forceinline__ double sample_depth64(float t, const double o[3], const double d[3], double p[3])
{
    const double td = (double)t;
    p[0] = o[0] + td * d[0];
    p[1] = o[1] + td * d[1];
    p[2] = o[2] + td * d[2];
    const double qx = p[0] - o[0], qy = p[1] - o[1], qz = p[2] - o[2];
    return sqrt((qx * qx + qy * qy) + qz * qz);
}

__global__ __launch_bounds__(kPackRays) void pack_samples_kernel(
    const float *__restrict__ rays_o, const float *__restrict__ rays_d, int64_t n_rays, int max_hits,
    const int32_t *__restrict__ hit_tri, const float *__restrict__ hit_t, const int32_t *__restrict__ hit_count,
    const int64_t *__restrict__ ray_offset, float *__restrict__ xyz, float *__restrict__ dirs,
    int64_t *__restrict__ index_ray, float *__restrict__ depth, int64_t *__restrict__ index_tri,
    float *__restrict__ origins, const int32_t *__restrict__ inverse, float *__restrict__ xyz_c,
    float *__restrict__ dirs_c, float *__restrict__ depth_c, const uint64_t *__restrict__ keep_mask,
    const int32_t *__restrict__ raw_count, float min_sep, int32_t *__restrict__ close_flag)
{
    extern __shared__ __attribute__((aligned(16))) unsigned char smem[];
    const int K = max_hits, Kp = max_hits | 1;
    float *s_t = reinterpret_cast<float *>(smem);
    int32_t *s_tri = reinterpret_cast<int32_t *>(s_t + kPackRays * Kp);
    uint16_t *s_map = reinterpret_cast<uint16_t *>(s_tri + kPackRays * Kp);
    __shared__ int s_region;

    const int tid = threadIdx.x;
    const int64_t ray0 = (int64_t)blockIdx.x * kPackRays;
    const int nr = (int)((n_rays - ray0) < kPackRays ? (n_rays - ray0) : kPackRays);
    int cnt = 0;
    if (tid < nr) {
        cnt = keep_mask ? raw_count[ray0 + tid] : hit_count[ray0 + tid];
        if (cnt > K) cnt = K;
    }
    if (K <= 32) {
        int deepest = cnt;
#pragma unroll
        for (int off = 32; off > 0; off >>= 1) {
            const int other = __shfl_xor(deepest, off, 64);
            deepest = other > deepest ? other : deepest;
        }
        const int64_t own = tid < nr ? ray0 + tid : ray0;
        if (deepest > 16) load_sort_row<32, true>(hit_t + own * K, hit_tri + own * K, K, cnt, deepest, s_t + tid * Kp, s_tri + tid * Kp);
        else if (deepest > 0) load_sort_row<16, true>(hit_t + own * K, hit_tri + own * K, K, cnt, deepest, s_t + tid * Kp, s_tri + tid * Kp);
    } else {
        for (int i = tid; i < nr * K; i += kPackRays) {
            const int r = i / K, k = i - r * K;
            s_t[r * Kp + k] = hit_t[ray0 * K + i];
            s_tri[r * Kp + k] = hit_tri[ray0 * K + i];
        }
    }
    if (tid == 0) s_region = 0;
    __syncthreads();

    const int64_t block_base = ray_offset[ray0];
    if (tid < nr) {
        const int64_t ray = ray0 + tid;
        float *row_t = s_t + tid * Kp;
        int32_t *row_i = s_tri + tid * Kp;
        if (K > 32) {
            for (int i = 1; i < cnt; ++i) {
                const float t = row_t[i];
                const int id = row_i[i];
                int j = i - 1;
                while (j >= 0 && hit_less(t, id, row_t[j], row_i[j])) { row_t[j + 1] = row_t[j]; row_i[j + 1] = row_i[j]; --j; }
                row_t[j + 1] = t;
                row_i[j + 1] = id;
            }
        }
        if (keep_mask) {
            const uint64_t mask = keep_mask[ray];
            int kept = 0;
            for (int i = 0; i < cnt; ++i)
                if ((mask >> i) & 1ull) { row_t[kept] = row_t[i]; row_i[kept] = row_i[i]; ++kept; }
            cnt = kept;
        } else if (close_flag && min_sep > 0.0f) {
            bool drop = false;
            for (int i = 1; i < cnt; ++i) drop |= !(row_t[i] > row_t[i - 1] + min_sep);
            if (drop) *close_flag = 1;
        }
        if (cnt > 1) {
            const double o64[3] = {(double)rays_o[ray * 3], (double)rays_o[ray * 3 + 1], (double)rays_o[ray * 3 + 2]};
            const double d64[3] = {(double)rays_d[ray * 3], (double)rays_d[ray * 3 + 1], (double)rays_d[ray * 3 + 2]};
            double p[3];
            double prev = sample_depth64(row_t[0], o64, d64, p);
            bool sorted = true;
            for (int k = 1; k < cnt; ++k) {
                const double dk = sample_depth64(row_t[k], o64, d64, p);
                sorted = sorted && !(prev > dk);
                prev = dk;
            }
            if (!sorted) {
                for (int i = 1; i < cnt; ++i) {
                    const float t = row_t[i];
                    const int id = row_i[i];
                    const double di = sample_depth64(t, o64, d64, p);
                    int j = i - 1;
                    while (j >= 0 && sample_depth64(row_t[j], o64, d64, p) > di) { row_t[j + 1] = row_t[j]; row_i[j + 1] = row_i[j]; --j; }
                    row_t[j + 1] = t;
                    row_i[j + 1] = id;
                }
            }
        }
        const int local = (int)(ray_offset[ray] - block_base);
        for (int k = 0; k < cnt; ++k) s_map[local + k] = (uint16_t)((tid << 8) | k);
        if (tid == nr - 1) s_region = local + cnt;
    }
    __syncthreads();

    const int region = s_region;
    for (int j = tid; j < region; j += kPackRays) {
        const int m = s_map[j];
        const int rl = m >> 8, k = m & 255;
        const int64_t ray = ray0 + rl;
        const float ox = rays_o[ray * 3], oy = rays_o[ray * 3 + 1], oz = rays_o[ray * 3 + 2];
        const float dx = rays_d[ray * 3], dy = rays_d[ray * 3 + 1], dz = rays_d[ray * 3 + 2];
        const double o64[3] = {(double)ox, (double)oy, (double)oz};
        const double d64[3] = {(double)dx, (double)dy, (double)dz};
        double p[3];
        const double dep = sample_depth64(s_t[rl * Kp + k], o64, d64, p);
        const float nrm = sqrtf((dx * dx + dy * dy) + dz * dz) + 1e-7f;
        const int64_t o = block_base + j;
        if (xyz) {
            xyz[o * 3 + 0] = (float)p[0];
            xyz[o * 3 + 1] = (float)p[1];
            xyz[o * 3 + 2] = (float)p[2];
            dirs[o * 3 + 0] = dx / nrm;
            dirs[o * 3 + 1] = dy / nrm;
            dirs[o * 3 + 2] = dz / nrm;
            origins[o * 3 + 0] = ox;
            origins[o * 3 + 1] = oy;
            origins[o * 3 + 2] = oz;
        }
        index_ray[o] = ray;
        depth[o] = (float)dep;
        index_tri[o] = (int64_t)s_tri[rl * Kp + k];
        if (inverse) {
            const int64_t c = inverse[o];
            xyz_c[c * 3 + 0] = (float)p[0];
            xyz_c[c * 3 + 1] = (float)p[1];
            xyz_c[c * 3 + 2] = (float)p[2];
            dirs_c[c * 3 + 0] = dx / nrm;
            dirs_c[c * 3 + 1] = dy / nrm;
            dirs_c[c * 3 + 2] = dz / nrm;
            if (depth_c) depth_c[c] = (float)dep;
        }
    }
}

template <bool kTri>
__global__ __launch_bounds__(64) void pack_tiles_kernel(
    const float *__restrict__ rays_o, const float *__restrict__ rays_d, int w, int h, int tiles_x, int n_tiles, int max_hits,
    const int32_t *__restrict__ hit_tri, const float *__restrict__ hit_t, const int32_t *__restrict__ hit_count,
    const int64_t *__restrict__ tile_base, const int64_t *__restrict__ total, float *__restrict__ xyz_c,
    float *__restrict__ dirs_c, float *__restrict__ depth_c, int32_t *__restrict__ tri_c, const uint64_t *__restrict__ keep_mask,
    const int32_t *__restrict__ raw_count, float min_sep, int32_t *__restrict__ final_count, int32_t *__restrict__ dropped)
{
    extern __shared__ __attribute__((aligned(16))) unsigned char smem[];
    const int K = max_hits, Kp = max_hits | 1;
    float *s_t = reinterpret_cast<float *>(smem);
    int32_t *s_tri = reinterpret_cast<int32_t *>(s_t + 64 * Kp);
    const int tile = blockIdx.x, lane = threadIdx.x;
    const int px0 = (tile % tiles_x) * 8, py0 = (tile / tiles_x) * 8;
    const int cols = (w - px0) < 8 ? (w - px0) : 8, rows = (h - py0) < 8 ? (h - py0) : 8;
    const int px = px0 + (lane & 7), py = py0 + (lane >> 3);
    const bool inside = px < w && py < h;
    const int64_t ray = inside ? (int64_t)py * w + px : 0;
    int cnt = 0;
    if (inside) {
        cnt = keep_mask ? raw_count[ray] : hit_count[ray];
        if (cnt > K) cnt = K;
    }
    int deepest = cnt;
#pragma unroll
    for (int off = 32; off > 0; off >>= 1) {
        const int other = __shfl_xor(deepest, off, 64);
        deepest = other > deepest ? other : deepest;
    }
    if (deepest == 0) {
        if (final_count && inside) final_count[ray] = 0;
        return;
    }
    float *row_t = s_t + lane * Kp;
    int32_t *row_i = s_tri + lane * Kp;
    const float ox = rays_o[ray * 3], oy = rays_o[ray * 3 + 1], oz = rays_o[ray * 3 + 2];
    const float dx = rays_d[ray * 3], dy = rays_d[ray * 3 + 1], dz = rays_d[ray * 3 + 2];
    int64_t base = tile_base[tile];
    if (K <= 32) {
        if (deepest <= 16) load_sort_row<16, kTri>(hit_t + ray * K, hit_tri + ray * K, K, cnt, deepest, row_t, row_i);
        else load_sort_row<32, kTri>(hit_t + ray * K, hit_tri + ray * K, K, cnt, deepest, row_t, row_i);
    } else {
        for (int yy = 0; yy < rows; ++yy) {
            const int64_t row_ray0 = (int64_t)(py0 + yy) * w + px0;
            for (int i = lane; i < cols * deepest; i += 64) {
                const int r = i / deepest, k = i - r * deepest;
                s_t[(yy * 8 + r) * Kp + k] = hit_t[(row_ray0 + r) * K + k];
                if (kTri) s_tri[(yy * 8 + r) * Kp + k] = hit_tri[(row_ray0 + r) * K + k];
            }
        }
        __syncthreads();
    }
    double o64[3] = {0.0, 0.0, 0.0}, d64[3] = {0.0, 0.0, 0.0};
    float dn[3] = {0.0f, 0.0f, 0.0f};
    int n_dropped = 0;
    if (inside) {
        if (K > 32) {
            for (int i = 1; i < cnt; ++i) {
                const float t = row_t[i];
                const int id = kTri ? row_i[i] : 0;
                int j = i - 1;
                while (j >= 0 && (kTri ? hit_less(t, id, row_t[j], row_i[j]) : t < row_t[j])) {
                    row_t[j + 1] = row_t[j];
                    if (kTri) row_i[j + 1] = row_i[j];
                    --j;
                }
                row_t[j + 1] = t;
                if (kTri) row_i[j + 1] = id;
            }
        }
        if (keep_mask) {
            const uint64_t mask = keep_mask[ray];
            int kept = 0;
            for (int i = 0; i < cnt; ++i)
                if ((mask >> i) & 1ull) { row_t[kept] = row_t[i]; if (kTri) row_i[kept] = row_i[i]; ++kept; }
            cnt = kept;
        } else if (min_sep > 0.0f && cnt > 1) {
            float last_t = row_t[0];
            int kept = 1;
            for (int i = 1; i < cnt; ++i) {
                const float t = row_t[i];
                if (t > last_t + min_sep) { row_t[kept] = t; if (kTri) row_i[kept] = row_i[i]; ++kept; last_t = t; }
            }
            n_dropped = cnt - kept;
            cnt = kept;
        }
        if (cnt > 0) {
            o64[0] = (double)ox; o64[1] = (double)oy; o64[2] = (double)oz;
            d64[0] = (double)dx; d64[1] = (double)dy; d64[2] = (double)dz;
            const float nrm = sqrtf((dx * dx + dy * dy) + dz * dz) + 1e-7f;
            dn[0] = dx / nrm; dn[1] = dy / nrm; dn[2] = dz / nrm;
        }
        if (cnt > 1) {
            double p[3];
            double prev = sample_depth64(row_t[0], o64, d64, p);
            bool sorted = true;
            for (int k = 1; k < cnt; ++k) {
                const double dk = sample_depth64(row_t[k], o64, d64, p);
                sorted = sorted && !(prev > dk);
                prev = dk;
            }
            if (!sorted) {
                for (int i = 1; i < cnt; ++i) {
                    const float t = row_t[i];
                    const int id = kTri ? row_i[i] : 0;
                    const double di = sample_depth64(t, o64, d64, p);
                    int j = i - 1;
                    while (j >= 0 && sample_depth64(row_t[j], o64, d64, p) > di) {
                        row_t[j + 1] = row_t[j];
                        if (kTri) row_i[j + 1] = row_i[j];
                        --j;
                    }
                    row_t[j + 1] = t;
                    if (kTri) row_i[j + 1] = id;
                }
            }
        }
    }
    if (final_count && inside) final_count[ray] = cnt;
    const unsigned long long below = (1ull << lane) - 1ull;
    float first_xyz[3] = {0.0f, 0.0f, 0.0f};
    for (int k = 0;; ++k) {
        const unsigned long long mask = __ballot(cnt > k);
        if (mask == 0ull) break;
        if (cnt > k) {
            const int64_t c = base + __popcll(mask & below);
            double p[3];
            const double dep = sample_depth64(row_t[k], o64, d64, p);
            xyz_c[c * 3 + 0] = (float)p[0];
            xyz_c[c * 3 + 1] = (float)p[1];
            xyz_c[c * 3 + 2] = (float)p[2];
            dirs_c[c * 3 + 0] = dn[0];
            dirs_c[c * 3 + 1] = dn[1];
            dirs_c[c * 3 + 2] = dn[2];
            depth_c[c] = (float)dep;
            if (kTri) tri_c[c] = (int32_t)row_i[k];
            if (k == 0) { first_xyz[0] = (float)p[0]; first_xyz[1] = (float)p[1]; first_xyz[2] = (float)p[2]; }
        }
        base += __popcll(mask);
    }
    const unsigned long long any_drop = __ballot(n_dropped > 0);
    if (any_drop) {
        const int64_t end = tile + 1 < n_tiles ? tile_base[tile + 1] : *total;
        const int src = __ffsll((long long)__ballot(cnt > 0)) - 1;
        const float gx = __shfl(first_xyz[0], src, 64), gy = __shfl(first_xyz[1], src, 64), gz = __shfl(first_xyz[2], src, 64);
        const float hx = __shfl(dn[0], src, 64), hy = __shfl(dn[1], src, 64), hz = __shfl(dn[2], src, 64);
        const int gtri = kTri ? __shfl((int)row_i[0], src, 64) : 0;
        for (int64_t c = base + lane; c < end; c += 64) {
            xyz_c[c * 3 + 0] = gx; xyz_c[c * 3 + 1] = gy; xyz_c[c * 3 + 2] = gz;
            dirs_c[c * 3 + 0] = hx; dirs_c[c * 3 + 1] = hy; dirs_c[c * 3 + 2] = hz;
            depth_c[c] = 0.0f;
            if (kTri) tri_c[c] = (int32_t)gtri;
        }
        int sum = n_dropped;
#pragma unroll
        for (int off = 32; off > 0; off >>= 1) sum += __shfl_xor(sum, off, 64);
        if (lane == 0 && dropped) atomicAdd(dropped, sum);
    }
}

__global__ void publish_dropped_kernel(int32_t *dropped, int64_t *host_out)
{
    host_out[2] = (int64_t)*dropped;
    *dropped = 0;
}

__global__ void resort_kernel(const int64_t *index_ray, const float *depth, int64_t n, int64_t *perm)
{
    for (int64_t i = (int64_t)blockIdx.x * blockDim.x + threadIdx.x; i < n; i += (int64_t)gridDim.x * blockDim.x) {
        const int64_t ray = index_ray[i];
        if (i != 0 && index_ray[i - 1] == ray) continue;
        perm[i] = i;
        for (int64_t k = i + 1; k < n && index_ray[k] == ray; ++k) {
            const float dk = depth[k];
            int64_t j = k - 1;
            while (j >= i && depth[perm[j]] > dk) { perm[j + 1] = perm[j]; --j; }
            perm[j + 1] = k;
        }
    }
}

constexpr int RS_THREADS = 256;
constexpr int RS_CHUNK = 1024;
constexpr int RS_HALO = 64;
constexpr int RS_STAGE = RS_CHUNK + RS_HALO;

__global__ __launch_bounds__(RS_THREADS) void resort_samples_kernel(
    const int64_t *index_ray, const float *depth, int64_t n, const float *points, const float *origins,
    const float *vectors, const int64_t *index_tri, int64_t *perm, float *out_points, float *out_depth,
    float *out_origins, float *out_vectors, int64_t *out_index_tri, uint8_t *boundary, const int32_t *inverse,
    float *out_points_c, float *out_vectors_c)
{
    __shared__ float s_depth[RS_STAGE];
    __shared__ int64_t s_ray[RS_STAGE + 1];
    __shared__ int s_src[RS_STAGE];
    __shared__ uint8_t s_mine[RS_STAGE];
    __shared__ int s_heads[RS_CHUNK];
    __shared__ int s_nheads;
    const int64_t n_chunks = (n + RS_CHUNK - 1) / RS_CHUNK;
    for (int64_t chunk = blockIdx.x; chunk < n_chunks; chunk += gridDim.x) {
        const int64_t b0 = chunk * RS_CHUNK;
        const int staged = (int)((n - b0 < RS_STAGE) ? (n - b0) : RS_STAGE);
        const int own = (int)((n - b0 < RS_CHUNK) ? (n - b0) : RS_CHUNK);
        if (threadIdx.x == 0) {
            s_ray[0] = b0 > 0 ? index_ray[b0 - 1] : 0;
            s_nheads = 0;
        }
        for (int k = threadIdx.x; k < staged; k += RS_THREADS) {
            s_depth[k] = depth[b0 + k];
            s_ray[k + 1] = index_ray[b0 + k];
            s_mine[k] = 0;
        }
        __syncthreads();
        for (int k = threadIdx.x; k < own; k += RS_THREADS) {
            const bool head = (b0 + k == 0) || s_ray[k] != s_ray[k + 1];
            if (boundary) boundary[b0 + k] = head ? 1 : 0;
            if (head) s_heads[atomicAdd(&s_nheads, 1)] = k;
        }
        __syncthreads();
        const int n_heads = s_nheads;
        for (int h = threadIdx.x; h < n_heads; h += RS_THREADS) {
            const int k = s_heads[h];
            const int64_t ray = s_ray[k + 1];
            int end = k + 1;
            while (end < staged && s_ray[end + 1] == ray) ++end;
            const bool spills = end == staged && b0 + staged < n && index_ray[b0 + staged] == ray;
            if (!spills) {
                s_src[k] = k;
                s_mine[k] = 1;
                for (int q = k + 1; q < end; ++q) {
                    const float dq = s_depth[q];
                    int j = q - 1;
                    while (j >= k && s_depth[s_src[j]] > dq) { s_src[j + 1] = s_src[j]; --j; }
                    s_src[j + 1] = q;
                    s_mine[q] = 1;
                }
            } else {
                const int64_t i = b0 + k;
                int64_t e = i + 1;
                while (e < n && index_ray[e] == ray) ++e;
                for (int64_t q = i; q < e; ++q) {
                    const float dq = depth[q];
                    int64_t rank = 0;
                    for (int64_t r = i; r < e; ++r) {
                        const float dr = depth[r];
                        rank += (dr < dq) || (dr == dq && r < q);
                    }
                    const int64_t dst = i + rank;
                    if (perm) perm[dst] = q;
                    out_depth[dst] = dq;
                    if (out_index_tri) out_index_tri[dst] = index_tri[q];
                    const int64_t pos_c = inverse ? (int64_t)inverse[dst] : 0;
                    for (int c = 0; c < 3; ++c) {
                        out_points[dst * 3 + c] = points[q * 3 + c];
                        if (out_origins) out_origins[dst * 3 + c] = origins[q * 3 + c];
                        out_vectors[dst * 3 + c] = vectors[q * 3 + c];
                        if (inverse) {
                            out_points_c[pos_c * 3 + c] = points[q * 3 + c];
                            out_vectors_c[pos_c * 3 + c] = vectors[q * 3 + c];
                        }
                    }
                }
            }
        }
        __syncthreads();
        for (int k = threadIdx.x; k < staged; k += RS_THREADS) {
            if (!s_mine[k]) continue;
            const int64_t src = b0 + s_src[k], dst = b0 + k;
            if (perm) perm[dst] = src;
            out_depth[dst] = s_depth[s_src[k]];
            if (out_index_tri) out_index_tri[dst] = index_tri[src];
        }
        for (int e = threadIdx.x; e < 3 * staged; e += RS_THREADS) {
            const int k = e / 3, c = e - 3 * k;
            if (!s_mine[k]) continue;
            const int64_t src = (b0 + s_src[k]) * 3 + c, dst = b0 * 3 + e;
            const float pv = points[src], vv = vectors[src];
            out_points[dst] = pv;
            if (out_origins) out_origins[dst] = origins[src];
            out_vectors[dst] = vv;
            if (inverse) {
                const int64_t pc = (int64_t)inverse[b0 + k] * 3 + c;
                out_points_c[pc] = pv;
                out_vectors_c[pc] = vv;
            }
        }
        __syncthreads();
    }
}

}

extern "C" int qf_pack_samples(const float *rays_o, const float *rays_d, int64_t n_rays, int32_t max_hits,
                               const int32_t *hit_tri, const float *hit_t, const int32_t *hit_count,
                               const int64_t *ray_offset, float *xyz, float *dirs, int64_t *index_ray, float *depth,
                               int64_t *index_tri, float *origins, const int32_t *inverse, float *xyz_c, float *dirs_c,
                               float *depth_c, const uint64_t *keep_mask, const int32_t *raw_count,
                               float min_separation, int32_t *close_flag, void *stream)
{
    if ((keep_mask == nullptr) != (raw_count == nullptr)) return QF_ERR_INVALID_ARGUMENT;
    if (n_rays < 0 || max_hits < 1 || max_hits > kMaxHits) return QF_ERR_INVALID_ARGUMENT;
    if (n_rays == 0) return QF_OK;
    if (!rays_o || !rays_d || !hit_tri || !hit_t || !hit_count || !ray_offset) return QF_ERR_INVALID_ARGUMENT;
    if (inverse && (!xyz_c || !dirs_c)) return QF_ERR_INVALID_ARGUMENT;
    if (!index_ray || !depth || !index_tri) return QF_ERR_INVALID_ARGUMENT;
    if ((xyz || dirs || origins) && (!xyz || !dirs || !origins)) return QF_ERR_INVALID_ARGUMENT;
    if (!xyz && !inverse) return QF_ERR_INVALID_ARGUMENT;
    const int Kp = max_hits | 1;
    const size_t lds = (size_t)kPackRays * Kp * 8 + (size_t)kPackRays * max_hits * 2 + 64;
    const int64_t blocks = qf_div_up(n_rays, kPackRays);
    if (blocks > 0x7fffffff) return QF_ERR_UNSUPPORTED;
    hipLaunchKernelGGL(pack_samples_kernel, dim3((unsigned)blocks), dim3(kPackRays), lds, qf_stream(stream), rays_o, rays_d,
                       n_rays, (int)max_hits, hit_tri, hit_t, hit_count, ray_offset, xyz, dirs, index_ray, depth, index_tri,
                       origins, inverse, xyz_c, dirs_c, depth_c, keep_mask, raw_count, min_separation, close_flag);
    QF_LAUNCH_CHECK();
    return QF_OK;
}

extern "C" int qf_pack_tiles(const float *rays_o, const float *rays_d, int32_t width, int32_t height, int32_t max_hits,
                             const int32_t *hit_tri, const float *hit_t, const int32_t *hit_count, const int64_t *tile_base,
                             const int64_t *total, float *xyz_c, float *dirs_c, float *depth_c, int32_t *tri_c,
                             const uint64_t *keep_mask, const int32_t *raw_count, float min_separation,
                             int32_t *final_count, int32_t *dropped, int64_t *host_out, int32_t dropped_is_zero,
                             void *stream)
{
    if ((keep_mask == nullptr) != (raw_count == nullptr)) return QF_ERR_INVALID_ARGUMENT;
    if (width < 1 || height < 1 || max_hits < 1 || max_hits > kMaxHits) return QF_ERR_INVALID_ARGUMENT;
    if (!rays_o || !rays_d || !hit_t || !hit_count || !tile_base || !total || !xyz_c || !dirs_c || !depth_c)
        return QF_ERR_INVALID_ARGUMENT;
    if (tri_c && !hit_tri) return QF_ERR_INVALID_ARGUMENT;
    const bool rule_here = !keep_mask && min_separation > 0.0f;
    if (rule_here && (!final_count || !dropped)) return QF_ERR_INVALID_ARGUMENT;
    if (host_out && !dropped) return QF_ERR_INVALID_ARGUMENT;
    hipStream_t st = qf_stream(stream);
    if (dropped && !host_out && !dropped_is_zero) QF_HIP_TRY(hipMemsetAsync(dropped, 0, sizeof(int32_t), st));
    const int tiles_x = (width + 7) / 8, tiles_y = (height + 7) / 8;
    const float sep = rule_here ? min_separation : 0.0f;
    auto *kernel = tri_c ? pack_tiles_kernel<true> : pack_tiles_kernel<false>;
    const size_t lds = (size_t)64 * (max_hits | 1) * (tri_c ? 8 : 4);
    hipLaunchKernelGGL(kernel, dim3((unsigned)(tiles_x * tiles_y)), dim3(64), lds, st, rays_o, rays_d, (int)width, (int)height,
                       tiles_x, tiles_x * tiles_y, (int)max_hits, hit_tri, hit_t, hit_count, tile_base, total, xyz_c, dirs_c,
                       depth_c, tri_c, keep_mask, raw_count, sep, final_count, dropped);
    if (host_out) hipLaunchKernelGGL(publish_dropped_kernel, dim3(1), dim3(1), 0, st, dropped, host_out);
    QF_LAUNCH_CHECK();
    return QF_OK;
}

extern "C" int qf_resort_by_depth(const int64_t *index_ray, const float *depth, int64_t n, int64_t *perm, void *stream)
{
    if (n < 0) return QF_ERR_INVALID_ARGUMENT;
    if (n == 0) return QF_OK;
    if (!index_ray || !depth || !perm) return QF_ERR_INVALID_ARGUMENT;
    QF_SIMPLE_LAUNCH(resort_kernel, n, index_ray, depth, n, perm);
    return QF_OK;
}

extern "C" int qf_resort_samples(const int64_t *index_ray, const float *depth, int64_t n, const float *points,
                                 const float *origins, const float *vectors, const int64_t *index_tri, int64_t *perm,
                                 float *out_points, float *out_depth, float *out_origins, float *out_vectors,
                                 int64_t *out_index_tri, uint8_t *boundary, const int32_t *inverse, float *out_points_c,
                                 float *out_vectors_c, void *stream)
{
    if (n < 0) return QF_ERR_INVALID_ARGUMENT;
    if (n == 0) return QF_OK;
    if (!index_ray || !depth || !points || !vectors || !out_points || !out_depth || !out_vectors ||
        (out_origins && !origins) || (out_index_tri && !index_tri) || (inverse && (!out_points_c || !out_vectors_c)))
        return QF_ERR_INVALID_ARGUMENT;
    const int64_t n_chunks = (n + RS_CHUNK - 1) / RS_CHUNK;
    hipLaunchKernelGGL(resort_samples_kernel, dim3((unsigned)(n_chunks < 65536 ? n_chunks : 65536)), dim3(RS_THREADS), 0,
                       qf_stream(stream), index_ray, depth, n, points, origins, vectors, index_tri, perm, out_points,
                       out_depth, out_origins, out_vectors, out_index_tri, boundary, inverse, out_points_c, out_vectors_c);
    QF_LAUNCH_CHECK();
    return QF_OK;
}
```

quadraturefields_amd/mesh_utils.py:

```python
import ctypes
import os
from types import SimpleNamespace
from typing import Optional

import numpy as np
import torch

from . import _C, spc_render
from .mesh_io import TriMesh, load_mesh


def _as_device_f32(x, device) -> torch.Tensor:
    if isinstance(x, np.ndarray):
        x = torch.from_numpy(np.ascontiguousarray(x, dtype=np.float32))
    return x.to(device=device, dtype=torch.float32).contiguous()


def make_camera(c2w, focal: float, width: int, height: int) -> _C.Camera:
    m = np.asarray(c2w.detach().cpu() if isinstance(c2w, torch.Tensor) else c2w, dtype=np.float32)[:3, :4]
    cam = _C.Camera()
    for i, v in enumerate(m.reshape(-1).tolist()):
        cam.c2w[i] = v
    cam.fx = cam.fy = float(focal)
    cam.cx, cam.cy = width / 2.0, height / 2.0
    cam.width, cam.height = int(width), int(height)
    return cam


def _on_device(fn):
    import functools

    @functools.wraps(fn)
    def wrapped(self, *args, **kwargs):
        if torch._C._cuda_getDevice() == self.device.index:
            return fn(self, *args, **kwargs)
        with torch.cuda.device(self.device):
            return fn(self, *args, **kwargs)
    return wrapped


def mesh_depth_complexity(vertices, faces) -> float:
    v = np.asarray(vertices, dtype=np.float64).reshape(-1, 3)
    f = np.asarray(faces).reshape(-1, 3)
    if v.shape[0] == 0 or f.shape[0] == 0:
        return 0.0
    area = 0.5 * np.linalg.norm(np.cross(v[f[:, 1]] - v[f[:, 0]], v[f[:, 2]] - v[f[:, 0]]), axis=1).sum()
    e = v.max(axis=0) - v.min(axis=0)
    box = 2.0 * (e[0] * e[1] + e[1] * e[2] + e[0] * e[2])
    return float(2.0 * area / box) if box > 0 else 0.0


def trimesh_ray_offset(vertices) -> float:
    v = np.asarray(vertices, dtype=np.float64).reshape(-1, 3)
    if v.shape[0] == 0:
        return 1e-8
    diag = float(np.sqrt(((v.max(axis=0) - v.min(axis=0)) ** 2).sum()))
    if not diag > 0:
        return 1e-8
    return float(np.clip(1e-4 * (100.0 / diag), 1e-8, np.inf))


_resolve_device = _C.resolve_device


class _PermuteRowsFn(torch.autograd.Function):

    @staticmethod
    def forward(ctx, x, perm):
        ctx.save_for_backward(perm)
        return x[perm]

    @staticmethod
    def backward(ctx, grad):
        (perm,) = ctx.saved_tensors
        out = torch.empty_like(grad)
        out[perm] = grad
        return out, None


def _permute_rows(x, perm):
    return _PermuteRowsFn.apply(x, perm) if x.requires_grad else x[perm]


class SampleSet(tuple):

    def __new__(cls, arrays, **meta):
        obj = super().__new__(cls, arrays)
        obj.__dict__.update(meta)
        return obj


class SampleWindow(tuple):

    def __new__(cls, arrays, **meta):
        obj = super().__new__(cls, arrays)
        obj.__dict__.update(meta)
        return obj


class _InterView:

    def __init__(self, owner):
        self._owner = owner

    def find_intersections(self, rays):
        return self._owner.find_intersections(rays)

    def update_vertices(self, vertices):
        self._owner.update_intersector(vertices)


class RayIntersector:

    def __init__(self, mesh: TriMesh, max_hits: int = 10, device="cuda:0", sah_depth: int = 32,
                 min_separation="trimesh"):
        if max_hits < 1 or max_hits > _C.QF_BVH_MAX_HITS:
            raise ValueError(f"max_hits must be in 1..{_C.QF_BVH_MAX_HITS}")
        self.mesh = mesh
        self.max_hits = int(max_hits)
        self.device = _resolve_device(device)
        self._min_separation_auto = isinstance(min_separation, str)
        if min_separation is None:
            min_separation = 0.0
        elif isinstance(min_separation, str):
            if min_separation != "trimesh":
                raise ValueError("min_separation: 'trimesh', a distance, 0 or None")
            min_separation = trimesh_ray_offset(mesh.vertices)
        self.min_separation = max(float(min_separation), 0.0)
        self.last_order = None
        self._raster_backoff = 0
        self.repaired_frames = 0
        self.camera_mismatch_frames = 0
        self._warned_mismatch = False
        self._raster_streak = 0
        self._raster_trying = False
        self.scratch_slot = 0
        self._rule_upfront = 0
        self._rule_pending = None
        self.rule_redone_frames = 0
        self.raster_wide = 0
        self.depth_complexity = mesh_depth_complexity(mesh.vertices, mesh.faces)
        self._policy_seeded = False
        self.raster_slabs = int(os.environ.get("QF_RASTER_SLABS", self.RASTER_SLABS))
        self._wide_scratch = {}
        self._scratch = {}
        self.last_layout = None
        self.last_frame = None
        self.last_image_shape = None
        self._deferred_policy = None
        self._fused_pending = []
        self._fused_parity = 0
        self._split_scratch = {}
        self._handle = ctypes.c_void_p()
        tri = np.ascontiguousarray(mesh.vertices.astype(np.float32)[mesh.faces].reshape(-1, 9))
        with torch.cuda.device(self.device):
            _C.check(_C.lib().qf_bvh_create_ex(tri.ctypes.data_as(ctypes.c_void_p), tri.shape[0], int(sah_depth),
                                               ctypes.byref(self._handle)), "qf_bvh_create_ex")
            _C.check(_C.lib().qf_bvh_set_min_separation(self._handle, self.min_separation), "qf_bvh_set_min_separation")

    def __del__(self):
        h = getattr(self, "_handle", None)
        if h is not None and h.value:
            try:
                _C.lib().qf_bvh_destroy(h)
            except Exception:
                pass
            self._handle = ctypes.c_void_p()

    @property
    def num_nodes(self) -> int:
        return int(_C.lib().qf_bvh_num_nodes(self._handle))

    @property
    def max_depth(self) -> int:
        return int(_C.lib().qf_bvh_max_depth(self._handle))

    @property
    def num_wide_nodes(self) -> int:
        return int(_C.lib().qf_bvh_num_wide_nodes(self._handle))

    @property
    def max_stack(self) -> int:
        return int(_C.lib().qf_bvh_max_stack(self._handle))

    @property
    def inter(self):
        return _InterView(self)

    @inter.setter
    def inter(self, new) -> None:
        core = getattr(new, "core", None)
        if not isinstance(core, RayIntersector):
            raise TypeError("inter: expected a quadraturefields_amd.intersector.Intersector")
        if core.mesh.faces.shape[0] != self.mesh.faces.shape[0] or core.device != self.device:
            raise ValueError("inter: the new intersector must hold the same triangles on the same device")
        self._handle, core._handle = core._handle, self._handle
        if self._min_separation_auto:
            self._apply_min_separation(trimesh_ray_offset(core.mesh.vertices))
        else:
            self._apply_min_separation(self.min_separation)

    def set_min_separation(self, min_separation: float) -> None:
        self._min_separation_auto = False
        self._apply_min_separation(min_separation)

    def _apply_min_separation(self, min_separation: float) -> None:
        self.min_separation = max(float(min_separation or 0.0), 0.0)
        _C.check(_C.lib().qf_bvh_set_min_separation(self._handle, self.min_separation), "qf_bvh_set_min_separation")

    def update_intersector(self, vertices) -> None:
        n_tri = self.mesh.faces.shape[0]
        if self._min_separation_auto:
            if isinstance(vertices, torch.Tensor):
                vv = vertices.detach().reshape(-1, 3)
                ext = torch.stack([vv.min(dim=0).values, vv.max(dim=0).values]).double().cpu().numpy()
            else:
                vv = np.asarray(vertices, dtype=np.float64).reshape(-1, 3)
                ext = np.stack([vv.min(axis=0), vv.max(axis=0)])
            self._apply_min_separation(trimesh_ray_offset(ext))
        if isinstance(vertices, torch.Tensor) and vertices.is_cuda:
            v = vertices.detach().to(device=self.device, dtype=torch.float32)
            if v.numel() == n_tri * 9 and tuple(v.shape) != tuple(self.mesh.vertices.shape):
                tri = v.reshape(-1, 9).contiguous()
            else:
                if getattr(self, "_faces_dev", None) is None:
                    self._faces_dev = torch.from_numpy(np.ascontiguousarray(self.mesh.faces, dtype=np.int64)).to(self.device)
                tri = v.reshape(-1, 3)[self._faces_dev].reshape(-1, 9).contiguous()
            with torch.cuda.device(self.device):
                _C.check(_C.lib().qf_bvh_refit_device(self._handle, _C.ptr(tri), n_tri, _C.stream()), "qf_bvh_refit_device")
            return
        v = np.asarray(vertices.detach().cpu() if isinstance(vertices, torch.Tensor) else vertices, dtype=np.float32)
        if v.size == n_tri * 9 and v.shape != tuple(self.mesh.vertices.shape):
            tri = np.ascontiguousarray(v.reshape(-1, 9))
        else:
            tri = np.ascontiguousarray(v.reshape(-1, 3)[self.mesh.faces].reshape(-1, 9))
        with torch.cuda.device(self.device):
            _C.check(_C.lib().qf_bvh_refit(self._handle, tri.ctypes.data_as(ctypes.c_void_p), tri.shape[0]), "qf_bvh_refit")

    RASTER_BACKOFF_MAX = 64

    def want_raster(self, camera) -> bool:
        if camera is None:
            return False
        if self._raster_backoff > 0:
            self._raster_backoff -= 1
            return False
        if self._raster_trying:
            self._raster_streak = 0
        self._raster_trying = True
        return True

    def camera_mismatch(self) -> None:
        self.camera_mismatch_frames += 1
        if not self._warned_mismatch:
            import warnings
            self._warned_mismatch = True
            warnings.warn("RayIntersector: the rays passed with camera= are not that camera's pixel grid (origin, direction "
                          "within 0.02 px of the own pixel centre, unit length -- e.g. jittered directions, a stale "
                          "make_camera, another up_sample or ray order); the frame was intersected exactly through the BVH "
                          "instead of the camera-coherent pass (about 5x slower).  Pass camera=None for such rays.",
                          stacklevel=3)
        self.raster_overflowed()

    def raster_overflowed(self) -> None:
        self._raster_trying = False
        self._raster_streak += 1
        self._raster_backoff = min(self.RASTER_BACKOFF_MAX, 1 << min(self._raster_streak - 1, 30))

    RASTER_WIDE_FACTOR = 4
    RASTER_WIDE_MAX = 128
    RASTER_SLABS = 3
    SLAB_ROOM = 32

    def _alloc_hits(self, n, k):
        return (torch.empty((n, k), dtype=torch.int32, device=self.device),
                torch.empty((n, k), dtype=torch.float32, device=self.device),
                torch.empty((n,), dtype=torch.int32, device=self.device))

    @_on_device
    def _hits_bvh(self, o, d, k, image_width):
        n = o.shape[0]
        hit_tri, hit_t, hit_count = self._alloc_hits(n, k)
        _C.check(_C.lib().qf_bvh_intersect(self._handle, _C.ptr(o), _C.ptr(d), n, k, int(image_width),
                                           _C.ptr(hit_tri), _C.ptr(hit_t), _C.ptr(hit_count), _C.stream()),
                 "qf_bvh_intersect")
        return hit_tri, hit_t, hit_count

    @_on_device
    def _hits_raster(self, o, d, k, camera, sort_lists=True):
        n = o.shape[0]
        hit_tri, hit_t, _ = self._alloc_hits(n, k)
        counts = torch.empty((n + 2,), dtype=torch.int32, device=self.device)
        hit_count, overflow = counts[:n], counts[n:n + 1]
        self._raster_words = counts[n:]
        _C.check(_C.lib().qf_raster_intersect(self._handle, ctypes.byref(camera), _C.ptr(o), _C.ptr(d), n, k,
                                              _C.ptr(hit_tri), _C.ptr(hit_t), _C.ptr(hit_count), _C.ptr(overflow),
                                              1 if sort_lists else 0, 0, _C.ptr(counts[n + 1:]), _C.stream()),
                 "qf_raster_intersect")
        return hit_tri, hit_t, hit_count, overflow

    @_on_device
    def hits(self, origins, vectors, max_hits: Optional[int] = None, image_width: int = 0, camera=None):
        k = self.max_hits if max_hits is None else int(max_hits)
        o = _as_device_f32(origins, self.device).reshape(-1, 3)
        d = _as_device_f32(vectors, self.device).reshape(-1, 3)
        if o.shape != d.shape:
            raise ValueError("origins and vectors must have the same shape")
        if camera is not None:
            image_width = camera.width
        if self.want_raster(camera):
            hit_tri, hit_t, hit_count, overflow = self._hits_raster(o, d, k, camera)
            ovf, bad_rays = self._raster_words.tolist()
            if ovf == 0 and bad_rays == 0:
                return hit_tri, hit_t, hit_count, o, d
            if bad_rays:
                self.camera_mismatch()
            else:
                self.raster_overflowed()
        hit_tri, hit_t, hit_count = self._hits_bvh(o, d, k, image_width)
        return hit_tri, hit_t, hit_count, o, d

    def find_intersections(self, rays) -> np.ndarray:
        r = np.asarray(rays, dtype=np.float32).reshape(-1, 6)
        hit_tri, _, _, _, _ = self.hits(r[:, :3], r[:, 3:])
        return hit_tri.reshape(-1).cpu().numpy()

    def _frame_scratch(self, n):
        key = (_C.raw_stream(), self.scratch_slot)
        s = self._scratch.get(key)
        if s is None:
            host = torch.zeros((4,), dtype=torch.int64).pin_memory()
            dropped = torch.zeros((1,), dtype=torch.int32, device=self.device)
            s = self._scratch[key] = [0, None, None, host, (torch.cuda.Event(), torch.cuda.Event()), dropped, 0]
        if n > s[0]:
            cap = max(n, 2 * s[0]) if s[0] else n
            nbytes = int(_C.lib().qf_frame_offsets_temp_bytes(cap))
            if nbytes < 0:
                raise _C.QFError("qf_frame_offsets_temp_bytes failed")
            s[1] = torch.zeros((cap + 3,), dtype=torch.int64, device=self.device)
            s[2] = torch.empty((nbytes,), dtype=torch.uint8, device=self.device)
            s[0] = cap
        s[6] += 1
        self._scratch_stamp = (s, s[6])
        return s[1][:n + 3], s[2], s[3], s[4], s[5]

    def _stamp(self, frame):
        frame._scratch, frame._seq = self._scratch_stamp
        return frame

    @_on_device
    def _hits_raster_frame(self, o, d, k, camera):
        n = o.shape[0]
        hit_tri, hit_t, _ = self._alloc_hits(n, k)
        counts = torch.empty((n + 2,), dtype=torch.int32, device=self.device)
        hit_count, overflow, origin_flag = counts[:n], counts[n:], counts[n + 1:]
        self._seed_policy(k)
        wide = max(int(self.raster_wide), 0)
        cull = 1 if getattr(camera, "cull", False) else 0
        if wide > k and self.raster_slabs >= 2:
            sel_cap = k + 8 if self.min_separation > 0 else k
            wide_s = min(sel_cap + 1 + self.SLAB_ROOM, 4096)
            key = (n, -wide_s, _C.raw_stream())
            keys = self._wide_scratch.get(key)
            if keys is None:
                self._wide_scratch.clear()
                keys = self._wide_scratch[key] = torch.empty((wide_s, n), dtype=torch.int64, device=self.device)
            _C.check(_C.lib().qf_raster_intersect_slabs(self._handle, ctypes.byref(camera), _C.ptr(o), _C.ptr(d), n, k, wide_s,
                                                        int(self.raster_slabs), _C.ptr(keys), _C.ptr(hit_tri), _C.ptr(hit_t),
                                                        _C.ptr(hit_count), _C.ptr(overflow), _C.ptr(origin_flag), _C.stream()),
                     "qf_raster_intersect_slabs")
        elif wide > k:
            key = (n, wide, _C.raw_stream())
            lists = self._wide_scratch.get(key)
            if lists is None:
                self._wide_scratch.clear()
                lists = self._wide_scratch[key] = (torch.empty((wide, n), dtype=torch.int32, device=self.device),
                                                   torch.empty((wide, n), dtype=torch.float32, device=self.device))
            _C.check(_C.lib().qf_raster_intersect_wide(self._handle, ctypes.byref(camera), _C.ptr(o), _C.ptr(d), n, k, wide,
                                                       _C.ptr(lists[0]), _C.ptr(lists[1]), _C.ptr(hit_tri), _C.ptr(hit_t),
                                                       _C.ptr(hit_count), _C.ptr(overflow), cull, _C.ptr(origin_flag),
                                                       _C.stream()),
                     "qf_raster_intersect_wide")
        else:
            _C.check(_C.lib().qf_raster_intersect(self._handle, ctypes.byref(camera), _C.ptr(o), _C.ptr(d), n, k,
                                                  _C.ptr(hit_tri), _C.ptr(hit_t), _C.ptr(hit_count), _C.ptr(overflow),
                                                  0, cull, _C.ptr(origin_flag), _C.stream()), "qf_raster_intersect")
        upfront = self.min_separation > 0 and self._rule_upfront > 0
        if upfront:
            self._rule_upfront -= 1
        self._repair(o, d, k, int(camera.width), hit_tri, hit_t, hit_count, with_mask=upfront, all_flag=origin_flag)
        return hit_tri, hit_t, hit_count, overflow

    RULE_UPFRONT_FRAMES = 64

    def _repair(self, o, d, k, width, hit_tri, hit_t, hit_count, with_mask, all_flag=None):
        n = o.shape[0]
        mask = raw = None
        if with_mask:
            mask = torch.empty((n,), dtype=torch.int64, device=self.device)
            raw = torch.empty((n,), dtype=torch.int32, device=self.device)
        _C.check(_C.lib().qf_bvh_repair_overflow(self._handle, _C.ptr(o), _C.ptr(d), n, k, int(width),
                                                 _C.ptr(hit_tri), _C.ptr(hit_t), _C.ptr(hit_count), _C.ptr(mask), _C.ptr(raw),
                                                 _C.ptr(all_flag), _C.stream()), "qf_bvh_repair_overflow")
        hit_count._qf_keep = (mask, raw) if mask is not None else None

    def pack_hits(self, o, d, k, hit_tri, hit_t, hit_count, overflow, width, lean=False, layout=True,
                  defer_rule_check=False, want_tri=False, band_rows=0):
        return self.pack_hits_end(self.pack_hits_begin(o, d, k, hit_tri, hit_t, hit_count, overflow, width, lean, layout,
                                                       want_tri, band_rows=band_rows), defer_rule_check)

    @_on_device
    def pack_hits_begin(self, o, d, k, hit_tri, hit_t, hit_count, overflow, width, lean=False, layout=True,
                        want_tri=False, publish=True, band_rows=0):
        n = o.shape[0]
        dev = self.device
        buf, temp, host, (ev, ev_flag), dropped = self._frame_scratch(n)
        cap = n * k
        image = bool(layout) and width > 0 and n % width == 0
        self.last_image_shape = (int(width), n // int(width)) if width > 0 and n % width == 0 else None
        tile_base = None
        band_rows = int(band_rows) if (image and not lean and band_rows and band_rows > 0) else 0
        tile_band = band_rows if (band_rows and band_rows < n // width) else 0
        self.last_band_cuts = None
        if image:
            height = n // width
            n_tiles = ((width + 7) // 8) * ((height + 7) // 8) if not tile_band else \
                int(_C.lib().qf_banded_tile_count(int(width), height, tile_band))
            tile_base = torch.empty((n_tiles,), dtype=torch.int64, device=dev)
        ray_flag = overflow[1:] if (overflow is not None and overflow.numel() >= 2) else None
        if bool(lean) and image:
            _C.check(_C.lib().qf_tile_offsets(_C.ptr(hit_count), k, int(width), n // int(width), _C.ptr(tile_base),
                                              _C.ptr(buf[n:]), _C.ptr(overflow), _C.ptr(ray_flag),
                                              ctypes.c_void_p(host.data_ptr()), _C.ptr(dropped), _C.stream()),
                     "qf_tile_offsets")
        else:
            _C.check(_C.lib().qf_frame_offsets(_C.ptr(hit_count), n, k, int(width) if image else 0, n // width if image else 0,
                                               _C.ptr(buf), _C.ptr(tile_base), _C.ptr(temp), temp.numel(), _C.ptr(overflow),
                                               _C.ptr(ray_flag), ctypes.c_void_p(host.data_ptr()), tile_band, _C.stream()),
                     "qf_frame_offsets")
            if band_rows:
                edges = self._band_edges(n, int(width), band_rows)
                cuts_host = self._band_cut_buffer(edges.shape[0])
                cuts_host.copy_(buf.index_select(0, edges), non_blocking=True)
                self.last_band_cuts = (cuts_host, band_rows * int(width))
        ev.record()
        lean = bool(lean) and image
        want_layout = layout
        keep = getattr(hit_count, "_qf_keep", None) or (None, None)
        optimistic = keep[0] is None and self.min_separation > 0
        flag = None
        if optimistic:
            host[2] = 0
            flag = ctypes.c_void_p(host.data_ptr() + 16)
        min_sep = float(self.min_separation) if optimistic else 0.0
        xyz = dirs = org = index_ray = index_tri = depth = None
        order = inverse = xyz_c = dirs_c = depth_c = layout = frame = None
        if image:
            xyz_c = torch.empty((cap, 3), dtype=torch.float32, device=dev)
            dirs_c = torch.empty((cap, 3), dtype=torch.float32, device=dev)
            depth_c = torch.empty((cap,), dtype=torch.float32, device=dev)
            frame = SimpleNamespace(depth_c=depth_c, hit_count=hit_count, max_hits=int(k), tile_base=tile_base,
                                    width=int(width), height=n // int(width), total=0, tri_c=None,
                                    total_dev=buf[n:n + 1])
            self._stamp(frame)
        if lean:
            layout = (None, xyz_c, dirs_c)
            optimistic = False
            final_count = torch.empty((n,), dtype=torch.int32, device=dev)
            frame.tri_c = torch.empty((cap,), dtype=torch.int32, device=dev) if want_tri else None
            _C.check(_C.lib().qf_pack_tiles(_C.ptr(o), _C.ptr(d), int(width), n // int(width), k, _C.ptr(hit_tri),
                                            _C.ptr(hit_t), _C.ptr(hit_count), _C.ptr(tile_base), _C.ptr(buf[n:]),
                                            _C.ptr(xyz_c), _C.ptr(dirs_c), _C.ptr(depth_c), _C.ptr(frame.tri_c),
                                            _C.ptr(keep[0]), _C.ptr(keep[1]),
                                            float(self.min_separation) if keep[0] is None else 0.0,
                                            _C.ptr(final_count), _C.ptr(dropped),
                                            ctypes.c_void_p(host.data_ptr()) if publish else None, 1, _C.stream()),
                     "qf_pack_tiles")
            frame.hit_count = final_count
            frame.dropped_dev = None if publish else dropped
            ev_flag.record()
        else:
            xyz = torch.empty((cap, 3), dtype=torch.float32, device=dev)
            dirs = torch.empty((cap, 3), dtype=torch.float32, device=dev)
            org = torch.empty((cap, 3), dtype=torch.float32, device=dev)
            index_ray = torch.empty((cap,), dtype=torch.int64, device=dev)
            index_tri = torch.empty((cap,), dtype=torch.int64, device=dev)
            depth = torch.empty((cap,), dtype=torch.float32, device=dev)
            if image:
                order, inverse = self.coherent_layout(hit_count, buf, cap, width, tile_base, want_order=True,
                                                      band_rows=tile_band)
                layout = (inverse, xyz_c, dirs_c)
                if tile_band:
                    frame.band_rows = tile_band
            _C.check(_C.lib().qf_pack_samples(_C.ptr(o), _C.ptr(d), n, k, _C.ptr(hit_tri), _C.ptr(hit_t),
                                              _C.ptr(hit_count), _C.ptr(buf), _C.ptr(xyz), _C.ptr(dirs),
                                              _C.ptr(index_ray), _C.ptr(depth), _C.ptr(index_tri), _C.ptr(org),
                                              _C.ptr(inverse), _C.ptr(xyz_c), _C.ptr(dirs_c), _C.ptr(depth_c),
                                              _C.ptr(keep[0]), _C.ptr(keep[1]), min_sep, flag, _C.stream()),
                     "qf_pack_samples")
        if optimistic:
            ev_flag.record()
        return (o, d, k, width, (lean, want_layout, band_rows), host, (ev, ev_flag if (optimistic or lean) else None),
                [xyz, dirs, index_ray, depth, index_tri, org], order, layout,
                (hit_tri, hit_t, hit_count, keep),
                frame)

    @_on_device
    def pack_hits_end(self, pending, defer_rule_check=False):
        o, d, k, width, lean, host, (ev, ev_flag), arrays, order, layout, _lists, frame = pending
        ev.synchronize()
        total, ovf = int(host[0]), int(host[1])
        if int(host[3]):
            self.camera_mismatch()
        self._rule_pending = None
        if ev_flag is not None and not lean[0]:
            if defer_rule_check:
                self._rule_pending = (ev_flag, host)
            else:
                ev_flag.synchronize()
                if int(host[2]) != 0:
                    return self._repack_exact(pending)
        self._overflow_policy(ovf, o.shape[0], k)
        self.last_layout = self.last_frame = None
        if total == 0:
            return None, None
        if layout is not None:
            self.last_layout = tuple(None if t is None else t[:total] for t in layout)
            frame.depth_c = frame.depth_c[:total]
            if frame.tri_c is not None:
                frame.tri_c = frame.tri_c[:total]
            frame.total = total
            frame.samples = None if lean[0] else total
            frame.dropped_src = (ev_flag, host) if lean[0] else None
            self.last_frame = frame
        return [None if t is None else t[:total] for t in arrays], (order[:total] if order is not None else None)

    SEED_WIDE_AT = 0.5

    def _seed_policy(self, k: int) -> None:
        if self._policy_seeded:
            return
        self._policy_seeded = True
        wide = min(self.RASTER_WIDE_FACTOR * k, self.RASTER_WIDE_MAX)
        if self.raster_wide == 0 and wide > k and self.depth_complexity >= self.SEED_WIDE_AT * k:
            self.raster_wide = wide

    def _overflow_policy(self, ovf: int, n_rays: int, k: int) -> None:
        if ovf:
            self.repaired_frames += 1
            if ovf > 0.05 * n_rays:
                wide = min(self.RASTER_WIDE_FACTOR * k, self.RASTER_WIDE_MAX)
                if self.raster_wide < wide and wide > k:
                    self.raster_wide = wide
                else:
                    self.raster_overflowed()

    def _settle_deferred_policy(self) -> None:
        pend, self._deferred_policy = self._deferred_policy, None
        if pend is not None:
            ev, host, n_rays, k = pend
            ev.synchronize()
            if int(host[3]):
                self.camera_mismatch()
            self._overflow_policy(int(host[1]), n_rays, k)
        while self._fused_pending:
            self._settle_fused_policy(0)

    def _settle_fused_policy(self, keep: int = 1) -> None:
        while len(self._fused_pending) > keep:
            ev, host, n_rays, k = self._fused_pending.pop(0)
            ev.synchronize()
            if int(host[3]):
                self.camera_mismatch()
            self._overflow_policy(int(host[1]), n_rays, k)

    def pack_hits_device(self, pending):
        o, d, k, width, lean, host, (ev, ev_flag), arrays, order, layout, _lists, frame = pending
        if not lean[0] or frame is None or layout is None:
            raise ValueError("pack_hits_device: a lean image-shaped pack is required")
        self._rule_pending = None
        self._deferred_policy = (ev, host, o.shape[0], k)
        self.last_layout = layout
        frame.total = int(frame.depth_c.shape[0])
        frame.samples = None
        frame.total_src = (ev, host)
        frame.dropped_src = (ev_flag, host)
        frame._keep = _lists
        self.last_frame = frame
        return frame

    def frame_samples(self, frame=None) -> int:
        f = self.last_frame if frame is None else frame
        if f is None:
            return 0
        if f.samples is None:
            sc = getattr(f, "_scratch", None)
            if sc is not None and sc[6] != f._seq:
                raise RuntimeError("frame_samples: this render-only frame's counts have not been read yet and a later frame "
                                   "has since reused the words they live in (same stream and scratch slot); ask for a "
                                   "frame's sample count before the next frame is sampled")
            total = f.total
            src = getattr(f, "total_src", None)
            if src is not None:
                src[0].synchronize()
                total = int(src[1][0])
                f.total_src = None
            if getattr(f, "dropped_dev", None) is not None:
                f.samples = total - int(f.dropped_dev.item())
                f.dropped_dev = None
            else:
                ev_flag, host = f.dropped_src
                ev_flag.synchronize()
                f.samples = total - int(host[2])
            f.dropped_src = None
        return f.samples

    def rule_violated(self) -> bool:
        pend, self._rule_pending = self._rule_pending, None
        if pend is None:
            return False
        ev_flag, host = pend
        ev_flag.synchronize()
        if int(host[2]) == 0:
            return False
        self._rule_violation()
        return True

    def _rule_violation(self):
        self._rule_window = min(4096, 2 * getattr(self, "_rule_window", self.RULE_UPFRONT_FRAMES // 2))
        self._rule_upfront = self._rule_window
        self.rule_redone_frames += 1

    def _repack_exact(self, pending):
        o, d, k, width, (lean, want_layout, band_rows), _host, _evs, _arrays, _order, _layout, (hit_tri, hit_t, hit_count, _keep), _frame = pending
        self._rule_violation()
        self._repair(o, d, k, width, hit_tri, hit_t, hit_count, with_mask=True)
        return self.pack_hits_end(self.pack_hits_begin(o, d, k, hit_tri, hit_t, hit_count, None, width, lean, want_layout,
                                                       band_rows=band_rows))

    @_on_device
    def sample_device(self, origins, vectors, max_hits: Optional[int] = None, image_width: int = 0, camera=None,
                      lean: bool = False, layout: bool = True, defer_rule_check: bool = False, want_tri: bool = False,
                      band_rows: int = 0):
        k = self.max_hits if max_hits is None else int(max_hits)
        o = _as_device_f32(origins, self.device).reshape(-1, 3)
        d = _as_device_f32(vectors, self.device).reshape(-1, 3)
        n = o.shape[0]
        if n == 0:
            return None
        if camera is not None:
            image_width = camera.width
        self._settle_deferred_policy()
        if self.want_raster(camera):
            hit_tri, hit_t, hit_count, overflow = self._hits_raster_frame(o, d, k, camera)
        else:
            hit_tri, hit_t, hit_count = self._hits_bvh(o, d, k, image_width)
            overflow = None
        data, self.last_order = self.pack_hits(o, d, k, hit_tri, hit_t, hit_count, overflow, int(image_width), lean,
                                               layout, defer_rule_check, want_tri, band_rows)
        return data

    @_on_device
    def sample_frame_device(self, origins, vectors, max_hits: Optional[int] = None, camera=None, want_tri: bool = False):
        if camera is None:
            raise ValueError("sample_frame_device: the rays must be a camera's pixel grid")
        k = self.max_hits if max_hits is None else int(max_hits)
        o = _as_device_f32(origins, self.device).reshape(-1, 3)
        d = _as_device_f32(vectors, self.device).reshape(-1, 3)
        if o.shape[0] != camera.width * camera.height:
            raise ValueError("sample_frame_device: origins / vectors must be the camera's full pixel grid")
        self._settle_deferred_policy()
        if self.want_raster(camera):
            hit_tri, hit_t, hit_count, overflow = self._hits_raster_frame(o, d, k, camera)
        else:
            hit_tri, hit_t, hit_count = self._hits_bvh(o, d, k, camera.width)
            overflow = None
        self.last_order = None
        return self.pack_hits_device(self.pack_hits_begin(o, d, k, hit_tri, hit_t, hit_count, overflow, int(camera.width),
                                                          lean=True, layout=True, want_tri=want_tri, publish=False))

    def fused_frame_ready(self, camera, max_hits: Optional[int] = None) -> bool:
        k = self.max_hits if max_hits is None else int(max_hits)
        self._seed_policy(k)
        return (camera is not None and self._raster_backoff <= 0 and int(self.raster_wide) <= k
                and not (self.min_separation > 0 and self._rule_upfront > 0))

    @_on_device
    def fused_frame_job(self, origins, vectors, max_hits: Optional[int] = None, camera=None, want_tri: bool = False):
        k = self.max_hits if max_hits is None else int(max_hits)
        o = _as_device_f32(origins, self.device).reshape(-1, 3)
        d = _as_device_f32(vectors, self.device).reshape(-1, 3)
        n = o.shape[0]
        w, h = int(camera.width), int(camera.height)
        if n != w * h:
            raise ValueError("fused_frame_job: origins / vectors must be the camera's full pixel grid")
        if self._deferred_policy is not None:
            self._settle_deferred_policy()
        self._settle_fused_policy(1)
        if not self.fused_frame_ready(camera, k) or not self.want_raster(camera):
            return None
        dev = self.device
        cap = n * k
        hit_tri, hit_t, _ = self._alloc_hits(n, k)
        counts = torch.empty((n + 2,), dtype=torch.int32, device=dev)
        final_count = torch.empty((n,), dtype=torch.int32, device=dev)
        tile_base = torch.empty((((w + 7) // 8) * ((h + 7) // 8),), dtype=torch.int64, device=dev)
        xyz_c = torch.empty((cap, 3), dtype=torch.float32, device=dev)
        dirs_c = torch.empty((cap, 3), dtype=torch.float32, device=dev)
        depth_c = torch.empty((cap,), dtype=torch.float32, device=dev)
        tri_c = torch.empty((cap,), dtype=torch.int32, device=dev) if want_tri else None
        buf, _temp, host, events, dropped = self._frame_scratch(n)
        self._fused_parity ^= 1
        ev, ev_flag = events[self._fused_parity], events[self._fused_parity ^ 1]
        job = _C.FrameJob()
        job.camera = ctypes.addressof(camera)
        job.rays_o, job.rays_d, job.n_rays, job.max_hits = o.data_ptr(), d.data_ptr(), n, k
        job.cull_chunks = 1 if getattr(camera, "cull", False) else 0
        job.min_separation = float(self.min_separation)
        job.hit_tri, job.hit_t, job.hit_count = hit_tri.data_ptr(), hit_t.data_ptr(), counts.data_ptr()
        job.final_count, job.tile_base = final_count.data_ptr(), tile_base.data_ptr()
        job.total, job.host_block, job.dropped = buf.data_ptr() + 8 * n, host.data_ptr(), dropped.data_ptr()
        job.xyz_c, job.dirs_c, job.depth_c = xyz_c.data_ptr(), dirs_c.data_ptr(), depth_c.data_ptr()
        job.tri_c = tri_c.data_ptr() if want_tri else None
        frame = SimpleNamespace(depth_c=depth_c, hit_count=final_count, max_hits=k, tile_base=tile_base, width=w, height=h,
                                total=cap, tri_c=tri_c, total_dev=buf[n:n + 1], samples=None, total_src=(ev, host),
                                dropped_src=(ev_flag, host), dropped_dev=dropped,
                                _keep=(hit_tri, hit_t, counts, o, d, camera))
        self._stamp(frame)
        return job, frame, (ev, host, n, k, xyz_c, dirs_c)

    def fused_frame_done(self, frame, token) -> None:
        ev, host, n, k, xyz_c, dirs_c = token
        ev.record()
        self._rule_pending = None
        self._fused_pending.append((ev, host, n, k))
        self.last_order = None
        self.last_image_shape = (frame.width, frame.height)
        self.last_layout = (None, xyz_c, dirs_c)
        self.last_frame = frame

    @_on_device
    def _band_edges(self, n_rays: int, width: int, band_rows: int) -> torch.Tensor:
        key = (n_rays, width, band_rows)
        cache = self.__dict__.setdefault("_band_edge_cache", {})
        e = cache.get(key)
        if e is None:
            if len(cache) > 8:
                cache.clear()
            step = band_rows * width
            e = cache[key] = torch.tensor(list(range(0, n_rays, step)) + [n_rays], dtype=torch.int64, device=self.device)
        return e

    def _band_cut_buffer(self, m: int) -> torch.Tensor:
        ring = self.__dict__.setdefault("_band_cut_ring", {})
        r = ring.get(m)
        if r is None:
            r = ring[m] = [[torch.empty((m,), dtype=torch.int64).pin_memory() for _ in range(4)], 0]
        r[1] += 1
        return r[0][r[1] % len(r[0])]

    def coherent_layout(self, hit_count, ray_offset, total: int, width: int, tile_base=None, want_order=True,
                        band_rows: int = 0):
        height = hit_count.shape[0] // width
        tiles = ((width + 7) // 8) * ((height + 7) // 8)
        dev = hit_count.device
        if tile_base is None:
            totals = torch.empty((tiles,), dtype=torch.int64, device=dev)
            _C.check(_C.lib().qf_tile_totals(_C.ptr(hit_count), width, height, _C.ptr(totals), _C.stream()), "qf_tile_totals")
            tile_base = (torch.cumsum(totals, dim=0) - totals).contiguous()
        order = torch.empty((total,), dtype=torch.int32, device=dev) if want_order else None
        inverse = torch.empty((total,), dtype=torch.int32, device=dev)
        _C.check(_C.lib().qf_coherent_layout(_C.ptr(hit_count), _C.ptr(ray_offset), _C.ptr(tile_base), width, height,
                                             _C.ptr(order), _C.ptr(inverse), int(band_rows), _C.stream()),
                 "qf_coherent_layout")
        return order, inverse

    @_on_device
    def split_layout(self, index_ray: torch.Tensor, width: int, height: int, want_order: bool = True):
        index_ray = _C.i64c(index_ray)
        n = index_ray.shape[0]
        n_rays = int(width) * int(height)
        if n == 0:
            empty = torch.empty((0,), dtype=torch.int32, device=self.device)
            return (empty if want_order else None), empty.clone(), torch.zeros((1,), dtype=torch.int32, device=self.device)
        key = (n_rays, int(width), _C.raw_stream())
        sc = self._split_scratch.get(key)
        if sc is None:
            if len(self._split_scratch) > 4:
                self._split_scratch.clear()
            tiles = ((width + 7) // 8) * ((height + 7) // 8)
            sc = self._split_scratch[key] = (torch.empty((n_rays,), dtype=torch.int32, device=self.device),
                                             torch.empty((n_rays + 1,), dtype=torch.int64, device=self.device),
                                             torch.empty((tiles,), dtype=torch.int64, device=self.device),
                                             torch.zeros((1,), dtype=torch.int32, device=self.device))
        hit_count, ray_offset, tile_base, invalid = sc
        order = torch.empty((n,), dtype=torch.int32, device=self.device) if want_order else None
        inverse = torch.empty((n,), dtype=torch.int32, device=self.device)
        _C.check(_C.lib().qf_split_layout(_C.ptr(index_ray), n, int(width), int(height), _C.ptr(hit_count),
                                          _C.ptr(ray_offset), _C.ptr(tile_base), _C.ptr(invalid), _C.ptr(order),
                                          _C.ptr(inverse), _C.stream()), "qf_split_layout")
        return order, inverse, invalid

    @torch.no_grad()
    def _warn_if_not_unit(self, vectors) -> None:
        if self.min_separation <= 0 or getattr(self, "_warned_unit", False) or not isinstance(vectors, np.ndarray):
            return
        if vectors.size == 0:
            return
        nrm = np.linalg.norm(np.asarray(vectors, dtype=np.float64).reshape(-1, 3), axis=1)
        if float(np.abs(nrm - 1.0).max()) > 1e-3:
            import warnings
            self._warned_unit = True
            warnings.warn("RayIntersector: ray directions are not unit vectors; the multi-hit rule's separation "
                          f"({self.min_separation:.3g}) is applied to the ray parameter t, i.e. scaled by 1/|d| -- normalise "
                          "the directions (as trimesh does) or set min_separation for your parametrisation", stacklevel=3)

    def intersects_id(self, origins, vectors, multiple_hits=True, return_locations=True, max_hits=10):
        k = int(max_hits) if multiple_hits else 1
        self._warn_if_not_unit(vectors)
        out = self.sample_device(origins, vectors, k)
        if out is None:
            return np.zeros(0, np.int64), np.zeros(0, np.int64), np.zeros((0, 3), np.float64)
        xyz, _, index_ray, _, index_tri, _ = out
        return index_tri.cpu().numpy(), index_ray.cpu().numpy(), xyz.cpu().numpy().astype(np.float64)


class MeshFinetune:

    def __init__(self, vertices, faces, scaling, device="cuda:0") -> None:
        self.vertices = np.array(vertices).astype(np.float32)
        self.device = _resolve_device(device)
        self.faces = torch.from_numpy(np.asarray(faces)).to(self.device).long()
        self._cache = torch.zeros((self.faces.shape[0], 4), device=self.device)
        self.cache_d = self._cache[:, :3]
        self.cache_w = self._cache[:, 3]
        self.cache_w[:] = 1e-8
        self.scaling = scaling
        self._skipped = torch.zeros((1,), dtype=torch.int32, device=self.device)

    @torch.no_grad()
    def update_d(self, d, w, index_tri):
        n = int(w.shape[0])
        if n == 0:
            return
        with torch.cuda.device(self.device):
            _C.check(_C.lib().qf_mesh_update_d(
                _C.ptr(_C.f32c(d.reshape(-1, 3))) if d is not None else None, _C.ptr(_C.f32c(w.reshape(-1))),
                _C.ptr(_C.i64c(index_tri.reshape(-1))), n, int(self.faces.shape[0]), _C.ptr(self._cache),
                _C.ptr(self._skipped), _C.stream()), "qf_mesh_update_d")

    def check_ids(self) -> None:
        bad = int(self._skipped.item())
        if bad:
            self._skipped.zero_()
            raise IndexError(f"MeshFinetune.update_d: {bad} sample(s) carried a triangle id outside [0, "
                             f"{int(self.faces.shape[0])}) and were skipped (stale samples after a mesh swap?)")

    @torch.no_grad()
    def update_faces(self):
        self.check_ids()
        deformation = torch.clip(self.cache_d / self.cache_w.unsqueeze(1), -self.scaling, self.scaling)
        df_vertices = torch.repeat_interleave(deformation, dim=0, repeats=3)
        flat = self.faces.flatten()
        n_v = self.vertices.shape[0]
        dv = torch.zeros((n_v, 3), device=self.device).index_add_(0, flat, df_vertices)
        cnt = torch.zeros(n_v, device=self.device).index_add_(0, flat, torch.ones_like(flat, dtype=torch.float32))
        self.vertices += (dv / cnt.clamp_min(1.0)[:, None]).cpu().numpy()

    @torch.no_grad()
    def reset_d(self):
        self.cache_d[:] = 0
        self.cache_w[:] = 1e-8


class MeshIntersection:

    def __init__(self, mesh_path, simplify_mesh=True, scale=1.0, num_repeat=16, optix=False, voxel_size=512,
                 num_intersections=20, render_step_size=0.005, device="cuda:0", min_hit_separation="trimesh"):
        if isinstance(mesh_path, TriMesh):
            self.mesh = TriMesh(mesh_path.vertices.copy(), mesh_path.faces.copy(), mesh_path.visual.uv)
        else:
            self.mesh = load_mesh(mesh_path)
        if simplify_mesh:
            raise NotImplementedError("simplify_mesh=True: vertex-clustering simplification is offline mesh tooling (out "
                                      "of scope) -- and the reference's own default path raises AttributeError (its open3d "
                                      "branch is disabled, mesh_utils.py:186,199); its scripts pass simplify_mesh=False")
        self.num_repeat = num_repeat
        self.num_intersections = num_intersections
        self.render_step_size = render_step_size
        self.device = _resolve_device(device)
        self.mesh.vertices *= scale
        self.vertices = torch.from_numpy(self.mesh.vertices.astype(np.float32)).to(self.device)
        self.rayintersector = RayIntersector(self.mesh, max_hits=self.num_intersections, device=self.device,
                                             min_separation=min_hit_separation)

    def find_deltas(self, boundary, depth):
        return torch.full((depth.shape[0],), self.render_step_size, dtype=torch.float32, device=self.device)

    def sampling_raytrace_device(self, vectors, origins, image_width: int = 0, camera=None, layout: bool = True,
                                 window_rays: int = 0):
        ri = self.rayintersector
        width = int(camera.width) if camera is not None else int(image_width)
        band_rows = 0
        if layout and window_rays and width > 0 and window_rays % width == 0:
            band_rows = int(window_rays) // width
        data = ri.sample_device(origins, vectors, self.num_intersections, image_width, camera, layout=layout,
                                band_rows=band_rows)
        if data is None or not band_rows or ri.last_band_cuts is None or ri.last_layout is None:
            return data
        cuts_host, band_rays = ri.last_band_cuts
        inverse, xyz_c, dirs_c = ri.last_layout
        n_rays = int(vectors.shape[0]) if hasattr(vectors, "shape") else int(len(vectors))
        return SampleSet(data, cuts=cuts_host.tolist(), window_rays=band_rays, num_rays=n_rays, inverse=inverse,
                         order=ri.last_order, xyz_c=xyz_c, dirs_c=dirs_c, width=width)

    def sampling_raytrace_numpy(self, vectors, origins, random=0):
        self.rayintersector._warn_if_not_unit(vectors)
        out = self.sampling_raytrace_device(vectors, origins)
        if out is None:
            return None
        xyz, dirs, index_ray, depth, index_tri, org = [t.cpu().numpy() for t in out]
        return xyz, dirs, index_ray, depth, index_tri, 0, org

    def sampling_indexing(self, points, origins, vectors, index_ray, depth, index_tri, random=0, layout_inverse=None,
                          lean=False):
        self.last_resort_layout = None
        index_ray = _C.i64c(index_ray)
        n = depth.shape[0]
        dev = depth.device
        if torch.is_grad_enabled() and any(t.requires_grad for t in (points, depth, origins, vectors)):
            depth_c = _C.f32c(depth.detach())
            perm = torch.empty((n,), dtype=torch.int64, device=dev)
            _C.check(_C.lib().qf_resort_by_depth(_C.ptr(index_ray), _C.ptr(depth_c), n, _C.ptr(perm), _C.stream()),
                     "qf_resort_by_depth")
            index_tri, index_ray = index_tri[perm], index_ray[perm]
            points, depth, origins, vectors = (_permute_rows(t, perm) for t in (points, depth, origins, vectors))
            boundary = spc_render.mark_pack_boundaries(index_ray)
            return points, self.find_deltas(boundary, depth), boundary, vectors, index_ray, depth, index_tri, origins
        points, depth, vectors = (_C.f32c(t.detach()) for t in (points, depth, vectors))
        if lean:
            origins = index_tri = o_origins = o_tri = None
        else:
            origins, index_tri = _C.f32c(origins.detach()), _C.i64c(index_tri)
            o_origins, o_tri = torch.empty_like(origins), torch.empty_like(index_tri)
        o_points, o_vectors = torch.empty_like(points), torch.empty_like(vectors)
        o_depth = torch.empty_like(depth)
        boundary = torch.empty((n,), dtype=torch.bool, device=dev)
        points_c = vectors_c = None
        if layout_inverse is not None:
            if layout_inverse.shape[0] != n:
                raise ValueError(f"layout_inverse has {layout_inverse.shape[0]} entries for {n} samples")
            points_c, vectors_c = torch.empty_like(points), torch.empty_like(vectors)
        _C.check(_C.lib().qf_resort_samples(
            _C.ptr(index_ray), _C.ptr(depth), n, _C.ptr(points), _C.ptr(origins), _C.ptr(vectors), _C.ptr(index_tri),
            None, _C.ptr(o_points), _C.ptr(o_depth), _C.ptr(o_origins), _C.ptr(o_vectors), _C.ptr(o_tri),
            _C.ptr(boundary), _C.ptr(layout_inverse, torch.int32), _C.ptr(points_c), _C.ptr(vectors_c), _C.stream()),
            "qf_resort_samples")
        if layout_inverse is not None:
            self.last_resort_layout = (points_c, vectors_c)
        return o_points, self.find_deltas(boundary, o_depth), boundary, o_vectors, index_ray, o_depth, o_tri, o_origins
```

Before: 399.1 million rays/s.

## Bin raster hits into per-tile records instead of per-ray hit lists

Adds a tile-binned raster path. Each triangle-pixel hit is appended as a packed (t, id, pixel) record to an 8x8 tile bin, staged in LDS and flushed with wave-aggregated atomics. A count kernel then builds per-pixel counts and overflow masks, and a bins-aware pack kernel reads the tile bins directly. The goal is to cut per-ray atomic contention and scattered hit-list writes. In exchange it reuses the rgb/sigma buffers as scratch, adds an extra kernel, and adds more complex overflow handling.

```diff
diff --git a/include/qf_hip.h b/include/qf_hip.h
--- a/include/qf_hip.h
+++ b/include/qf_hip.h
@@ -241,6 +241,12 @@
                            int32_t *hit_count, uint64_t *keep_mask, int32_t *raw_count,
                            const int32_t *traverse_all_flag, void *stream);
 
+int64_t qf_hit_bins_bytes(int32_t width, int32_t height, int32_t max_hits);
+int qf_raster_intersect_tiles(qf_bvh *bvh, const qf_camera *cam , const float *rays_o, const float *rays_d,
+                              int64_t n_rays, int32_t max_hits, int32_t *tile_cursor, uint64_t *tile_mask, void *bins,
+                              int64_t bins_bytes, int32_t *hit_count, int32_t *overflow, int32_t *ray_flag ,
+                              void *stream);
+
 int qf_grid_march_count(const float *aabb, const int32_t *resolution, const uint8_t *binaries,
                         const float *rays_o, const float *rays_d, const float *t_min, const float *t_max,
                         int64_t n_rays, float near_plane, float far_plane, float step, int32_t *count, void *stream);
@@ -304,6 +310,13 @@
                   int32_t dropped_is_zero ,
                   void *stream);
 
+int qf_pack_tiles_bins(const float *rays_o, const float *rays_d, int32_t width, int32_t height, int32_t max_hits,
+                       const int32_t *hit_tri, const float *hit_t, const int32_t *hit_count, const int64_t *tile_base,
+                       const int64_t *total, float *xyz_c, float *dirs_c, float *depth_c, int32_t *tri_c ,
+                       float min_separation, int32_t *final_count, int32_t *dropped, int64_t *host_out,
+                       int32_t dropped_is_zero, const int32_t *tile_cursor, const uint64_t *tile_mask, const void *bins,
+                       const int32_t *ray_flag, void *stream);
+
 int qf_tile_totals(const int32_t *hit_count, int32_t width, int32_t height, int64_t *tile_total, void *stream);
 int qf_coherent_layout(const int32_t *hit_count, const int64_t *ray_offset, const int64_t *tile_base,
                        int32_t width, int32_t height, int32_t *order, int32_t *inverse,
@@ -318,6 +331,7 @@
 int qf_row_sample_counts(const int32_t *hit_count, int32_t max_hits, int32_t width, int32_t height, float *out_rows,
                          void *stream);
 
+#define QF_FRAME_PER_RAY_LISTS 2
 #define QF_FIELD_FP32 0
 #define QF_FIELD_BF16 1
 #define QF_FIELD_FP16 2
diff --git a/quadraturefields_amd/_C.py b/quadraturefields_amd/_C.py
--- a/quadraturefields_amd/_C.py
+++ b/quadraturefields_amd/_C.py
@@ -141,6 +141,10 @@
     "qf_frame_offsets": (c_int, [_P, c_int64, c_int32, c_int32, c_int32, _P, _P, _P, c_int64, _P, _P, _P, c_int32, _P]),
     "qf_banded_tile_count": (c_int64, [c_int32, c_int32, c_int32]),
     "qf_tile_offsets": (c_int, [_P, c_int32, c_int32, c_int32, _P, _P, _P, _P, _P, _P, _P]),
+    "qf_hit_bins_bytes": (c_int64, [c_int32, c_int32, c_int32]),
+    "qf_raster_intersect_tiles": (c_int, [_P, POINTER(Camera), _P, _P, c_int64, c_int32, _P, _P, _P, c_int64, _P, _P, _P, _P]),
+    "qf_pack_tiles_bins": (c_int, [_P, _P, c_int32, c_int32, c_int32, _P, _P, _P, _P, _P, _P, _P, _P, _P, c_float, _P, _P, _P,
+                                   c_int32, _P, _P, _P, _P, _P]),
     "qf_pack_tiles": (c_int, [_P, _P, c_int32, c_int32, c_int32, _P, _P, _P, _P, _P, _P, _P, _P, _P, _P, _P, c_float, _P, _P, _P, c_int32, _P]),
     "qf_pack_samples": (c_int, [_P, _P, c_int64, c_int32, _P, _P, _P, _P, _P, _P, _P, _P, _P, _P, _P, _P, _P, _P, _P, _P, c_float, _P, _P]),
     "qf_tile_totals": (c_int, [_P, c_int32, c_int32, _P, _P]),
diff --git a/quadraturefields_amd/csrc/frame.cpp b/quadraturefields_amd/csrc/frame.cpp
--- a/quadraturefields_amd/csrc/frame.cpp
+++ b/quadraturefields_amd/csrc/frame.cpp
@@ -36,20 +36,46 @@
     }
     const int64_t cap = j.n_rays * (int64_t)j.max_hits;
     int32_t *overflow = j.hit_count + j.n_rays;
-    int rc = qf_raster_intersect(bvh, j.camera, j.rays_o, j.rays_d, j.n_rays, j.max_hits, j.hit_tri, j.hit_t, j.hit_count,
-                                 overflow, j.tri_c ? 0 : 2 , j.cull_chunks,
-                                 overflow + 1, stream);
-    if (rc != QF_OK) return rc;
-    rc = qf_bvh_repair_overflow(bvh, j.rays_o, j.rays_d, j.n_rays, j.max_hits, w, j.hit_tri, j.hit_t, j.hit_count, nullptr,
-                                nullptr, overflow + 1, stream);
-    if (rc != QF_OK) return rc;
-    rc = qf_tile_offsets(j.hit_count, j.max_hits, w, h, j.tile_base, j.total, overflow, overflow + 1, j.host_block, j.dropped,
-                         stream);
-    if (rc != QF_OK) return rc;
-    rc = qf_pack_tiles(j.rays_o, j.rays_d, w, h, j.max_hits, j.hit_tri, j.hit_t, j.hit_count, j.tile_base, j.total, j.xyz_c,
-                       j.dirs_c, j.depth_c, j.tri_c, nullptr, nullptr, j.min_separation, j.final_count, j.dropped, nullptr, 1,
-                       stream);
-    if (rc != QF_OK) return rc;
+    const int32_t cull = j.cull_chunks & 1;
+    const int64_t n_tiles = (int64_t)((w + 7) / 8) * ((h + 7) / 8);
+    const int64_t bins_bytes = qf_hit_bins_bytes(w, h, j.max_hits);
+    const bool use_bins = j.field && !cull && !(j.cull_chunks & QF_FRAME_PER_RAY_LISTS) && j.max_hits <= 32 &&
+                          qf_bvh_num_triangles(bvh) < (1 << 26) && bins_bytes >= 0 &&
+                          bins_bytes <= cap * 3 * (int64_t)sizeof(float) && n_tiles * 12 <= cap * (int64_t)sizeof(float) &&
+                          reinterpret_cast<uintptr_t>(j.rgb_c) % 8 == 0 && reinterpret_cast<uintptr_t>(j.sigma_c) % 8 == 0;
+    if (use_bins) {
+        uint64_t *tile_mask = reinterpret_cast<uint64_t *>(j.sigma_c);
+        int32_t *tile_cursor = reinterpret_cast<int32_t *>(tile_mask + n_tiles);
+        int rc = qf_raster_intersect_tiles(bvh, j.camera, j.rays_o, j.rays_d, j.n_rays, j.max_hits, tile_cursor, tile_mask,
+                                           j.rgb_c, bins_bytes, j.hit_count, overflow, overflow + 1, stream);
+        if (rc != QF_OK) return rc;
+        rc = qf_bvh_repair_overflow(bvh, j.rays_o, j.rays_d, j.n_rays, j.max_hits, w, j.hit_tri, j.hit_t, j.hit_count, nullptr,
+                                    nullptr, overflow + 1, stream);
+        if (rc != QF_OK) return rc;
+        rc = qf_tile_offsets(j.hit_count, j.max_hits, w, h, j.tile_base, j.total, overflow, overflow + 1, j.host_block,
+                             j.dropped, stream);
+        if (rc != QF_OK) return rc;
+        rc = qf_pack_tiles_bins(j.rays_o, j.rays_d, w, h, j.max_hits, j.hit_tri, j.hit_t, j.hit_count, j.tile_base, j.total,
+                                j.xyz_c, j.dirs_c, j.depth_c, j.tri_c, j.min_separation, j.final_count, j.dropped, nullptr, 1,
+                                tile_cursor, tile_mask, j.rgb_c, overflow + 1, stream);
+        if (rc != QF_OK) return rc;
+    } else {
+        int rc = qf_raster_intersect(bvh, j.camera, j.rays_o, j.rays_d, j.n_rays, j.max_hits, j.hit_tri, j.hit_t, j.hit_count,
+                                     overflow, j.tri_c ? 0 : 2 , cull,
+                                     overflow + 1, stream);
+        if (rc != QF_OK) return rc;
+        rc = qf_bvh_repair_overflow(bvh, j.rays_o, j.rays_d, j.n_rays, j.max_hits, w, j.hit_tri, j.hit_t, j.hit_count, nullptr,
+                                    nullptr, overflow + 1, stream);
+        if (rc != QF_OK) return rc;
+        rc = qf_tile_offsets(j.hit_count, j.max_hits, w, h, j.tile_base, j.total, overflow, overflow + 1, j.host_block, j.dropped,
+                             stream);
+        if (rc != QF_OK) return rc;
+        rc = qf_pack_tiles(j.rays_o, j.rays_d, w, h, j.max_hits, j.hit_tri, j.hit_t, j.hit_count, j.tile_base, j.total, j.xyz_c,
+                           j.dirs_c, j.depth_c, j.tri_c, nullptr, nullptr, j.min_separation, j.final_count, j.dropped, nullptr, 1,
+                           stream);
+        if (rc != QF_OK) return rc;
+    }
+    int rc = QF_OK;
     if (!j.field) return QF_OK;
     if (j.field_precision == QF_FIELD_FP32) {
         rc = qf_field_forward(j.field, static_cast<const float *>(j.table), static_cast<const float *>(j.base_w),
diff --git a/quadraturefields_amd/csrc/raster.hip b/quadraturefields_amd/csrc/raster.hip
--- a/quadraturefields_amd/csrc/raster.hip
+++ b/quadraturefields_amd/csrc/raster.hip
@@ -77,12 +77,40 @@
     return true;
 }
 
-template <int kRasterLanes, bool kWide, bool kSlab = false>
+constexpr int kBinStage = 256;
+constexpr int kBinIdBits = 26;
+struct BinStage { int n; int tile[kBinStage]; uint2 rec[kBinStage]; };
+struct TileBins {
+    int32_t *cursor;
+    uint2 *bins;
+    int cap;
+    BinStage *stage;
+};
+
+__device__ __forceinline__ void bin_records(const TileBins &tb, int tile, uint2 rec)
+{
+    const int lane = (int)__lane_id();
+    for (;;) {
+        const int t0 = __builtin_amdgcn_readfirstlane(tile);
+        const unsigned long long m = __ballot(tile == t0);
+        if (tile == t0) {
+            const int rank = __popcll(m & ((1ull << lane) - 1ull));
+            int base = 0;
+            if (rank == 0) base = atomicAdd(&tb.cursor[t0], __popcll(m));
+            base = __shfl(base, __ffsll((long long)m) - 1, 64);
+            if (base + rank < tb.cap) tb.bins[(int64_t)t0 * tb.cap + base + rank] = rec;
+            break;
+        }
+    }
+}
+
+template <int kRasterLanes, bool kWide, bool kSlab = false, bool kBins = false>
 __device__ __forceinline__ void raster_triangle(const float4 *__restrict__ tris, int64_t tri_i, int sub, const RasterCam &cam,
                                                 const float *__restrict__ rays_o, const float *__restrict__ rays_d,
                                                 int max_hits, int32_t *__restrict__ hit_tri, float *__restrict__ hit_t,
                                                 int32_t *__restrict__ hit_count, int32_t *__restrict__ overflow,
-                                                const bool cam_origin, const SlabArgs slab = SlabArgs())
+                                                const bool cam_origin, const SlabArgs slab = SlabArgs(),
+                                                const TileBins bins = TileBins())
 {
     const float4 a = tris[tri_i * 3 + 0], b = tris[tri_i * 3 + 1], c = tris[tri_i * 3 + 2];
     const int id = __float_as_int(a.w);
@@ -125,6 +153,14 @@
             else atomicAdd(overflow, 1);
             continue;
         }
+        if (kBins) {
+            const int tile = (cy_ >> 3) * ((cam.w + 7) >> 3) + (cx_ >> 3);
+            const uint2 rec = make_uint2(__float_as_uint(t), ((uint32_t)id << 6) | (uint32_t)((cy_ & 7) * 8 + (cx_ & 7)));
+            const int at = atomicAdd(&bins.stage->n, 1);
+            if (at < kBinStage) { bins.stage->tile[at] = tile; bins.stage->rec[at] = rec; }
+            else bin_records(bins, tile, rec);
+            continue;
+        }
         const int slot = atomicAdd(&hit_count[ray], 1);
         if (slot < max_hits) {
             const int64_t at = kWide ? (int64_t)slot * ((int64_t)cam.w * cam.h) + ray : ray * max_hits + slot;
@@ -151,6 +187,73 @@
     const bool cam_origin = ray_flag != nullptr;
     raster_triangle<kRasterLanes, kWide>(tris, tri_i, sub, cam, rays_o, rays_d, max_hits, hit_tri, hit_t, hit_count, overflow,
                                          cam_origin);
+}
+
+template <int kRasterLanes>
+__global__ __launch_bounds__(256) void raster_bins_kernel(const float4 *__restrict__ tris, int64_t n_tri, RasterCam cam,
+                                                          const float *__restrict__ rays_o, const float *__restrict__ rays_d,
+                                                          int max_hits, int32_t *__restrict__ tile_cursor,
+                                                          uint2 *__restrict__ bin_records_out,
+                                                          const int32_t *__restrict__ ray_flag)
+{
+    __shared__ BinStage s_stage[4];
+    const int64_t gid = (int64_t)blockIdx.x * blockDim.x + threadIdx.x;
+    const int64_t tri_i = gid / kRasterLanes;
+    const int sub = (int)(gid % kRasterLanes);
+    if (ray_flag && *ray_flag) return;
+    const bool cam_origin = ray_flag != nullptr;
+    const int lane = (int)(threadIdx.x & 63);
+    TileBins tb;
+    tb.cursor = tile_cursor;
+    tb.bins = bin_records_out;
+    tb.cap = 64 * max_hits;
+    tb.stage = &s_stage[threadIdx.x >> 6];
+    if (lane == 0) tb.stage->n = 0;
+    __builtin_amdgcn_fence(__ATOMIC_ACQ_REL, "workgroup");
+    __builtin_amdgcn_wave_barrier();
+    if (tri_i < n_tri)
+        raster_triangle<kRasterLanes, false, false, true>(tris, tri_i, sub, cam, rays_o, rays_d, max_hits, nullptr, nullptr,
+                                                          nullptr, nullptr, cam_origin, SlabArgs(), tb);
+    __builtin_amdgcn_fence(__ATOMIC_ACQ_REL, "workgroup");
+    __builtin_amdgcn_wave_barrier();
+    const int n = tb.stage->n < kBinStage ? tb.stage->n : kBinStage;
+    for (int i = lane; i < n; i += 64) bin_records(tb, tb.stage->tile[i], tb.stage->rec[i]);
+}
+
+__global__ __launch_bounds__(64) void tile_count_kernel(const int32_t *__restrict__ tile_cursor, const uint2 *__restrict__ bins,
+                                                        int max_hits, int w, int h, int tiles_x,
+                                                        int32_t *__restrict__ hit_count, int32_t *__restrict__ overflow,
+                                                        uint64_t *__restrict__ tile_mask)
+{
+    __shared__ int s_cnt[64];
+    const int tile = blockIdx.x, lane = threadIdx.x;
+    const int cap = 64 * max_hits;
+    const int cursor = tile_cursor[tile];
+    const int n = cursor < cap ? cursor : cap;
+    const int px = (tile % tiles_x) * 8 + (lane & 7), py = (tile / tiles_x) * 8 + (lane >> 3);
+    const bool inside = px < w && py < h;
+    int c = 0;
+    if (n > 0) {
+        s_cnt[lane] = 0;
+        __syncthreads();
+        const uint2 *run = bins + (int64_t)tile * cap;
+        for (int i = lane; i < n; i += 64) atomicAdd(&s_cnt[run[i].y & 63u], 1);
+        __syncthreads();
+        c = s_cnt[lane];
+    }
+    int over = c > max_hits ? c - max_hits : 0;
+    if (cursor > cap) {
+        c = c > max_hits ? c : max_hits + 1;
+        over = lane == 0 ? cursor - cap : 0;
+    }
+    if (inside) hit_count[(int64_t)py * w + px] = c;
+    const unsigned long long mask = __ballot(inside && c > max_hits);
+    if (mask) {
+#pragma unroll
+        for (int off = 32; off > 0; off >>= 1) over += __shfl_xor(over, off, 64);
+        if (lane == 0) atomicAdd(overflow, over);
+    }
+    if (lane == 0) tile_mask[tile] = mask;
 }
 
 constexpr float kRayPixelTol = 0.02f;
@@ -762,6 +865,52 @@
     return QF_OK;
 }
 
+extern "C" int64_t qf_hit_bins_bytes(int32_t width, int32_t height, int32_t max_hits)
+{
+    if (width < 1 || height < 1 || max_hits < 1 || max_hits > kMaxHits) return -1;
+    return (int64_t)((width + 7) / 8) * ((height + 7) / 8) * 64 * max_hits * (int64_t)sizeof(uint2);
+}
+
+extern "C" int qf_raster_intersect_tiles(qf_bvh *bvh, const qf_camera *cam, const float *rays_o, const float *rays_d,
+                                         int64_t n_rays, int32_t max_hits, int32_t *tile_cursor, uint64_t *tile_mask,
+                                         void *bins, int64_t bins_bytes, int32_t *hit_count, int32_t *overflow,
+                                         int32_t *origin_flag, void *stream)
+{
+    if (!raster_args_ok(bvh, cam, n_rays, max_hits)) return QF_ERR_INVALID_ARGUMENT;
+    if (!rays_o || !rays_d || !tile_cursor || !tile_mask || !bins || !hit_count || !overflow) return QF_ERR_INVALID_ARGUMENT;
+    if (bins_bytes < qf_hit_bins_bytes(cam->width, cam->height, max_hits)) return QF_ERR_INVALID_ARGUMENT;
+    if (reinterpret_cast<uintptr_t>(bins) % sizeof(uint2) || reinterpret_cast<uintptr_t>(tile_mask) % sizeof(uint64_t))
+        return QF_ERR_INVALID_ARGUMENT;
+    if (bvh->n_tri >= (1 << kBinIdBits)) return QF_ERR_UNSUPPORTED;
+    hipStream_t st = qf_stream(stream);
+    const int tiles_x = (cam->width + 7) / 8, n_tiles = tiles_x * ((cam->height + 7) / 8);
+    QF_HIP_TRY(hipMemsetAsync(tile_cursor, 0, (size_t)n_tiles * sizeof(int32_t), st));
+    if (origin_flag == overflow + 1) {
+        QF_HIP_TRY(hipMemsetAsync(overflow, 0, 2 * sizeof(int32_t), st));
+    } else {
+        QF_HIP_TRY(hipMemsetAsync(overflow, 0, sizeof(int32_t), st));
+        if (origin_flag) QF_HIP_TRY(hipMemsetAsync(origin_flag, 0, sizeof(int32_t), st));
+    }
+    const RasterCam rc = make_raster_cam(cam);
+    uint2 *records = reinterpret_cast<uint2 *>(bins);
+    if (bvh->n_tri > 0) {
+        const int lanes = raster_lanes(n_rays, bvh->n_tri);
+        const int64_t blocks = qf_div_up(bvh->n_tri * lanes, 256);
+        if (blocks > 0x7fffffff) return QF_ERR_UNSUPPORTED;
+        camera_check_launch(rc, rays_o, rays_d, n_rays, origin_flag, st);
+        QF_LAUNCH_CHECK();
+        with_lanes(lanes, [&](auto L) {
+            hipLaunchKernelGGL(raster_bins_kernel<decltype(L)::value>, dim3((unsigned)blocks), dim3(256), 0, st,
+                               reinterpret_cast<const float4 *>(bvh->d_tris), bvh->n_tri, rc, rays_o, rays_d, (int)max_hits,
+                               tile_cursor, records, origin_flag);
+        });
+    }
+    hipLaunchKernelGGL(tile_count_kernel, dim3((unsigned)n_tiles), dim3(64), 0, st, tile_cursor, records, (int)max_hits,
+                       rc.w, rc.h, tiles_x, hit_count, overflow, tile_mask);
+    QF_LAUNCH_CHECK();
+    return QF_OK;
+}
+
 extern "C" int qf_raster_intersect_wide(qf_bvh *bvh, const qf_camera *cam, const float *rays_o, const float *rays_d,
                                         int64_t n_rays, int32_t max_hits, int32_t wide_hits, int32_t *wide_tri,
                                         float *wide_t, int32_t *hit_tri, float *hit_t, int32_t *hit_count,
diff --git a/quadraturefields_amd/csrc/sample_pack.hip b/quadraturefields_amd/csrc/sample_pack.hip
--- a/quadraturefields_amd/csrc/sample_pack.hip
+++ b/quadraturefields_amd/csrc/sample_pack.hip
@@ -3,6 +3,57 @@
 #pragma clang fp contract(off)
 
 namespace {
+
+template <int kN, bool kTri>
+__device__ __forceinline__ void sort_to_row(float (&t)[kN], int32_t (&id)[kN], int cnt, float *row_t, int32_t *row_i)
+{
+    if (kTri) {
+        uint64_t key[kN];
+#pragma unroll
+        for (int k = 0; k < kN; ++k) key[k] = k < cnt ? hit_key(t[k], id[k]) : ~0ull;
+#pragma unroll
+        for (int k = 2; k <= kN; k <<= 1) {
+#pragma unroll
+            for (int i = 0; i < kN; ++i) {
+                const int l = i ^ (k - 1);
+                if (l > i) { const uint64_t a = key[i], b = key[l]; key[i] = a < b ? a : b; key[l] = a < b ? b : a; }
+            }
+#pragma unroll
+            for (int j = k >> 2; j > 0; j >>= 1) {
+#pragma unroll
+                for (int i = 0; i < kN; ++i) {
+                    const int l = i ^ j;
+                    if (l > i) { const uint64_t a = key[i], b = key[l]; key[i] = a < b ? a : b; key[l] = a < b ? b : a; }
+                }
+            }
+        }
+#pragma unroll
+        for (int k = 0; k < kN; ++k)
+            if (k < cnt) { row_t[k] = key_t(key[k]); row_i[k] = key_id(key[k]); }
+    } else {
+#pragma unroll
+        for (int k = 0; k < kN; ++k) t[k] = k < cnt ? t[k] : INFINITY;
+#pragma unroll
+        for (int k = 2; k <= kN; k <<= 1) {
+#pragma unroll
+            for (int i = 0; i < kN; ++i) {
+                const int l = i ^ (k - 1);
+                if (l > i) { const float a = t[i], b = t[l]; t[i] = fminf(a, b); t[l] = fmaxf(a, b); }
+            }
+#pragma unroll
+            for (int j = k >> 2; j > 0; j >>= 1) {
+#pragma unroll
+                for (int i = 0; i < kN; ++i) {
+                    const int l = i ^ j;
+                    if (l > i) { const float a = t[i], b = t[l]; t[i] = fminf(a, b); t[l] = fmaxf(a, b); }
+                }
+            }
+        }
+#pragma unroll
+        for (int k = 0; k < kN; ++k)
+            if (k < cnt) row_t[k] = t[k];
+    }
+}
 
 template <int kN, bool kTri>
 __device__ __forceinline__ void load_sort_row(const float *__restrict__ g_t, const int32_t *__restrict__ g_i, int K,
@@ -30,52 +81,24 @@
 #pragma unroll
         for (int e = 0; e < 4; ++e) { t[4 * j + e] = v[e]; id[4 * j + e] = w[e]; }
     }
-    if (kTri) {
-        uint64_t key[kN];
-#pragma unroll
-        for (int k = 0; k < kN; ++k) key[k] = k < cnt ? hit_key(t[k], id[k]) : ~0ull;
-#pragma unroll
-        for (int k = 2; k <= kN; k <<= 1) {
-#pragma unroll
-            for (int i = 0; i < kN; ++i) {
-                const int l = i ^ (k - 1);
-                if (l > i) { const uint64_t a = key[i], b = key[l]; key[i] = a < b ? a : b; key[l] = a < b ? b : a; }
-            }
-#pragma unroll
-            for (int j = k >> 2; j > 0; j >>= 1) {
-#pragma unroll
-                for (int i = 0; i < kN; ++i) {
-                    const int l = i ^ j;
-                    if (l > i) { const uint64_t a = key[i], b = key[l]; key[i] = a < b ? a : b; key[l] = a < b ? b : a; }
-                }
-            }
-        }
-#pragma unroll
-        for (int k = 0; k < kN; ++k)
-            if (k < cnt) { row_t[k] = key_t(key[k]); row_i[k] = key_id(key[k]); }
-    } else {
-#pragma unroll
-        for (int k = 0; k < kN; ++k) t[k] = k < cnt ? t[k] : INFINITY;
-#pragma unroll
-        for (int k = 2; k <= kN; k <<= 1) {
-#pragma unroll
-            for (int i = 0; i < kN; ++i) {
-                const int l = i ^ (k - 1);
-                if (l > i) { const float a = t[i], b = t[l]; t[i] = fminf(a, b); t[l] = fmaxf(a, b); }
-            }
-#pragma unroll
-            for (int j = k >> 2; j > 0; j >>= 1) {
-#pragma unroll
-                for (int i = 0; i < kN; ++i) {
-                    const int l = i ^ j;
-                    if (l > i) { const float a = t[i], b = t[l]; t[i] = fminf(a, b); t[l] = fmaxf(a, b); }
-                }
-            }
-        }
-#pragma unroll
-        for (int k = 0; k < kN; ++k)
-            if (k < cnt) row_t[k] = t[k];
-    }
+    sort_to_row<kN, kTri>(t, id, cnt, row_t, row_i);
+}
+
+template <int kN, bool kTri>
+__device__ __forceinline__ void sort_row_in_place(int cnt, int deepest, float *row_t, int32_t *row_i)
+{
+    float t[kN];
+    int32_t id[kN];
+#pragma unroll
+    for (int k = 0; k < kN; ++k) {
+        t[k] = INFINITY;
+        id[k] = -1;
+        if (k < deepest && k < cnt) {
+            t[k] = row_t[k];
+            if (kTri) id[k] = row_i[k];
+        }
+    }
+    sort_to_row<kN, kTri>(t, id, cnt, row_t, row_i);
 }
 
 constexpr int kPackRays = 128;
@@ -229,13 +252,15 @@
     }
 }
 
-template <bool kTri>
+template <bool kTri, bool kBins>
 __global__ __launch_bounds__(64) void pack_tiles_kernel(
     const float *__restrict__ rays_o, const float *__restrict__ rays_d, int w, int h, int tiles_x, int n_tiles, int max_hits,
     const int32_t *__restrict__ hit_tri, const float *__restrict__ hit_t, const int32_t *__restrict__ hit_count,
     const int64_t *__restrict__ tile_base, const int64_t *__restrict__ total, float *__restrict__ xyz_c,
     float *__restrict__ dirs_c, float *__restrict__ depth_c, int32_t *__restrict__ tri_c, const uint64_t *__restrict__ keep_mask,
-    const int32_t *__restrict__ raw_count, float min_sep, int32_t *__restrict__ final_count, int32_t *__restrict__ dropped)
+    const int32_t *__restrict__ raw_count, float min_sep, int32_t *__restrict__ final_count, int32_t *__restrict__ dropped,
+    const int32_t *__restrict__ tile_cursor, const uint64_t *__restrict__ tile_mask, const uint2 *__restrict__ bins,
+    const int32_t *__restrict__ ray_flag)
 {
     extern __shared__ __attribute__((aligned(16))) unsigned char smem[];
     const int K = max_hits, Kp = max_hits | 1;
@@ -267,7 +292,34 @@
     const float ox = rays_o[ray * 3], oy = rays_o[ray * 3 + 1], oz = rays_o[ray * 3 + 2];
     const float dx = rays_d[ray * 3], dy = rays_d[ray * 3 + 1], dz = rays_d[ray * 3 + 2];
     int64_t base = tile_base[tile];
-    if (K <= 32) {
+    if (kBins) {
+        __shared__ int s_fill[64];
+        const unsigned long long by_row = (ray_flag && *ray_flag) ? ~0ull : tile_mask[tile];
+        const int cap = 64 * K;
+        const int cursor = tile_cursor[tile];
+        const int n = by_row == ~0ull ? 0 : (cursor < cap ? cursor : cap);
+        const uint2 *run = bins + (int64_t)tile * cap;
+        s_fill[lane] = 0;
+        __syncthreads();
+        for (int i = lane; i < n; i += 64) {
+            const uint2 rec = run[i];
+            const int p = (int)(rec.y & 63u);
+            const int at = atomicAdd(&s_fill[p], 1);
+            if (!((by_row >> p) & 1ull) && at < K) {
+                s_t[p * Kp + at] = __uint_as_float(rec.x);
+                if (kTri) s_tri[p * Kp + at] = (int32_t)(rec.y >> 6);
+            }
+        }
+        __syncthreads();
+        const bool own_row = (by_row >> lane) & 1ull;
+        if (deepest <= 16) {
+            if (own_row) load_sort_row<16, kTri>(hit_t + ray * K, hit_tri + ray * K, K, cnt, deepest, row_t, row_i);
+            else sort_row_in_place<16, kTri>(cnt, deepest, row_t, row_i);
+        } else {
+            if (own_row) load_sort_row<32, kTri>(hit_t + ray * K, hit_tri + ray * K, K, cnt, deepest, row_t, row_i);
+            else sort_row_in_place<32, kTri>(cnt, deepest, row_t, row_i);
+        }
+    } else if (K <= 32) {
         if (deepest <= 16) load_sort_row<16, kTri>(hit_t + ray * K, hit_tri + ray * K, K, cnt, deepest, row_t, row_i);
         else load_sort_row<32, kTri>(hit_t + ray * K, hit_tri + ray * K, K, cnt, deepest, row_t, row_i);
     } else {
@@ -547,11 +599,12 @@
     return QF_OK;
 }
 
-extern "C" int qf_pack_tiles(const float *rays_o, const float *rays_d, int32_t width, int32_t height, int32_t max_hits,
+static int pack_tiles_launch(const float *rays_o, const float *rays_d, int32_t width, int32_t height, int32_t max_hits,
                              const int32_t *hit_tri, const float *hit_t, const int32_t *hit_count, const int64_t *tile_base,
                              const int64_t *total, float *xyz_c, float *dirs_c, float *depth_c, int32_t *tri_c,
                              const uint64_t *keep_mask, const int32_t *raw_count, float min_separation,
                              int32_t *final_count, int32_t *dropped, int64_t *host_out, int32_t dropped_is_zero,
+                             const int32_t *tile_cursor, const uint64_t *tile_mask, const void *bins, const int32_t *ray_flag,
                              void *stream)
 {
     if ((keep_mask == nullptr) != (raw_count == nullptr)) return QF_ERR_INVALID_ARGUMENT;
@@ -566,14 +619,42 @@
     if (dropped && !host_out && !dropped_is_zero) QF_HIP_TRY(hipMemsetAsync(dropped, 0, sizeof(int32_t), st));
     const int tiles_x = (width + 7) / 8, tiles_y = (height + 7) / 8;
     const float sep = rule_here ? min_separation : 0.0f;
-    auto *kernel = tri_c ? pack_tiles_kernel<true> : pack_tiles_kernel<false>;
+    auto *kernel = bins ? (tri_c ? pack_tiles_kernel<true, true> : pack_tiles_kernel<false, true>)
+                        : (tri_c ? pack_tiles_kernel<true, false> : pack_tiles_kernel<false, false>);
     const size_t lds = (size_t)64 * (max_hits | 1) * (tri_c ? 8 : 4);
     hipLaunchKernelGGL(kernel, dim3((unsigned)(tiles_x * tiles_y)), dim3(64), lds, st, rays_o, rays_d, (int)width, (int)height,
                        tiles_x, tiles_x * tiles_y, (int)max_hits, hit_tri, hit_t, hit_count, tile_base, total, xyz_c, dirs_c,
-                       depth_c, tri_c, keep_mask, raw_count, sep, final_count, dropped);
+                       depth_c, tri_c, keep_mask, raw_count, sep, final_count, dropped, tile_cursor, tile_mask,
+                       reinterpret_cast<const uint2 *>(bins), ray_flag);
     if (host_out) hipLaunchKernelGGL(publish_dropped_kernel, dim3(1), dim3(1), 0, st, dropped, host_out);
     QF_LAUNCH_CHECK();
     return QF_OK;
+}
+
+extern "C" int qf_pack_tiles(const float *rays_o, const float *rays_d, int32_t width, int32_t height, int32_t max_hits,
+                             const int32_t *hit_tri, const float *hit_t, const int32_t *hit_count, const int64_t *tile_base,
+                             const int64_t *total, float *xyz_c, float *dirs_c, float *depth_c, int32_t *tri_c,
+                             const uint64_t *keep_mask, const int32_t *raw_count, float min_separation,
+                             int32_t *final_count, int32_t *dropped, int64_t *host_out, int32_t dropped_is_zero,
+                             void *stream)
+{
+    return pack_tiles_launch(rays_o, rays_d, width, height, max_hits, hit_tri, hit_t, hit_count, tile_base, total, xyz_c, dirs_c,
+                             depth_c, tri_c, keep_mask, raw_count, min_separation, final_count, dropped, host_out,
+                             dropped_is_zero, nullptr, nullptr, nullptr, nullptr, stream);
+}
+
+extern "C" int qf_pack_tiles_bins(const float *rays_o, const float *rays_d, int32_t width, int32_t height, int32_t max_hits,
+                                  const int32_t *hit_tri, const float *hit_t, const int32_t *hit_count,
+                                  const int64_t *tile_base, const int64_t *total, float *xyz_c, float *dirs_c, float *depth_c,
+                                  int32_t *tri_c, float min_separation, int32_t *final_count, int32_t *dropped,
+                                  int64_t *host_out, int32_t dropped_is_zero, const int32_t *tile_cursor,
+                                  const uint64_t *tile_mask, const void *bins, const int32_t *ray_flag, void *stream)
+{
+    if (!tile_cursor || !tile_mask || !bins || max_hits > 32) return QF_ERR_INVALID_ARGUMENT;
+    if (!hit_tri) return QF_ERR_INVALID_ARGUMENT;
+    return pack_tiles_launch(rays_o, rays_d, width, height, max_hits, hit_tri, hit_t, hit_count, tile_base, total, xyz_c, dirs_c,
+                             depth_c, tri_c, nullptr, nullptr, min_separation, final_count, dropped, host_out, dropped_is_zero,
+                             tile_cursor, tile_mask, bins, ray_flag, stream);
 }
 
 extern "C" int qf_resort_by_depth(const int64_t *index_ray, const float *depth, int64_t n, int64_t *perm, void *stream)
diff --git a/quadraturefields_amd/mesh_utils.py b/quadraturefields_amd/mesh_utils.py
--- a/quadraturefields_amd/mesh_utils.py
+++ b/quadraturefields_amd/mesh_utils.py
@@ -348,8 +348,28 @@
         frame._scratch, frame._seq = self._scratch_stamp
         return frame
 
+    hit_bins = True
+
+    def _hit_bins_ready(self, k, camera) -> bool:
+        self._seed_policy(k)
+        return (self.hit_bins and int(self.raster_wide) <= k and k <= 32 and not getattr(camera, "cull", False)
+                and int(self.mesh.faces.shape[0]) < (1 << 26) and not (self.min_separation > 0 and self._rule_upfront > 0))
+
+    def _bin_scratch(self, camera, k):
+        key = (_C.raw_stream(), self.scratch_slot)
+        n_tiles = ((int(camera.width) + 7) // 8) * ((int(camera.height) + 7) // 8)
+        nbytes = int(_C.lib().qf_hit_bins_bytes(int(camera.width), int(camera.height), k))
+        if nbytes < 0:
+            raise _C.QFError("qf_hit_bins_bytes failed")
+        s = self.__dict__.setdefault("_bin_scratch_sets", {}).get(key)
+        if s is None or s[0].numel() < n_tiles or s[2].numel() < nbytes // 8:
+            s = self._bin_scratch_sets[key] = (torch.empty((n_tiles,), dtype=torch.int32, device=self.device),
+                                               torch.empty((n_tiles,), dtype=torch.int64, device=self.device),
+                                               torch.empty((nbytes // 8,), dtype=torch.int64, device=self.device))
+        return s
+
     @_on_device
-    def _hits_raster_frame(self, o, d, k, camera):
+    def _hits_raster_frame(self, o, d, k, camera, bins=False):
         n = o.shape[0]
         hit_tri, hit_t, _ = self._alloc_hits(n, k)
         counts = torch.empty((n + 2,), dtype=torch.int32, device=self.device)
@@ -357,6 +377,15 @@
         self._seed_policy(k)
         wide = max(int(self.raster_wide), 0)
         cull = 1 if getattr(camera, "cull", False) else 0
+        if bins:
+            cursor, mask, records = self._bin_scratch(camera, k)
+            _C.check(_C.lib().qf_raster_intersect_tiles(self._handle, ctypes.byref(camera), _C.ptr(o), _C.ptr(d), n, k,
+                                                        _C.ptr(cursor), _C.ptr(mask), _C.ptr(records), records.numel() * 8,
+                                                        _C.ptr(hit_count), _C.ptr(overflow), _C.ptr(origin_flag),
+                                                        _C.stream()), "qf_raster_intersect_tiles")
+            self._repair(o, d, k, int(camera.width), hit_tri, hit_t, hit_count, with_mask=False, all_flag=origin_flag)
+            hit_count._qf_bins = (cursor, mask, records, origin_flag)
+            return hit_tri, hit_t, hit_count, overflow
         if wide > k and self.raster_slabs >= 2:
             sel_cap = k + 8 if self.min_separation > 0 else k
             wide_s = min(sel_cap + 1 + self.SLAB_ROOM, 4096)
@@ -468,14 +497,24 @@
             optimistic = False
             final_count = torch.empty((n,), dtype=torch.int32, device=dev)
             frame.tri_c = torch.empty((cap,), dtype=torch.int32, device=dev) if want_tri else None
-            _C.check(_C.lib().qf_pack_tiles(_C.ptr(o), _C.ptr(d), int(width), n // int(width), k, _C.ptr(hit_tri),
-                                            _C.ptr(hit_t), _C.ptr(hit_count), _C.ptr(tile_base), _C.ptr(buf[n:]),
-                                            _C.ptr(xyz_c), _C.ptr(dirs_c), _C.ptr(depth_c), _C.ptr(frame.tri_c),
-                                            _C.ptr(keep[0]), _C.ptr(keep[1]),
-                                            float(self.min_separation) if keep[0] is None else 0.0,
-                                            _C.ptr(final_count), _C.ptr(dropped),
-                                            ctypes.c_void_p(host.data_ptr()) if publish else None, 1, _C.stream()),
-                     "qf_pack_tiles")
+            bins = getattr(hit_count, "_qf_bins", None)
+            if bins is not None:
+                _C.check(_C.lib().qf_pack_tiles_bins(_C.ptr(o), _C.ptr(d), int(width), n // int(width), k, _C.ptr(hit_tri),
+                                                     _C.ptr(hit_t), _C.ptr(hit_count), _C.ptr(tile_base), _C.ptr(buf[n:]),
+                                                     _C.ptr(xyz_c), _C.ptr(dirs_c), _C.ptr(depth_c), _C.ptr(frame.tri_c),
+                                                     float(self.min_separation), _C.ptr(final_count), _C.ptr(dropped),
+                                                     ctypes.c_void_p(host.data_ptr()) if publish else None, 1,
+                                                     _C.ptr(bins[0]), _C.ptr(bins[1]), _C.ptr(bins[2]), _C.ptr(bins[3]),
+                                                     _C.stream()), "qf_pack_tiles_bins")
+            else:
+                _C.check(_C.lib().qf_pack_tiles(_C.ptr(o), _C.ptr(d), int(width), n // int(width), k, _C.ptr(hit_tri),
+                                                _C.ptr(hit_t), _C.ptr(hit_count), _C.ptr(tile_base), _C.ptr(buf[n:]),
+                                                _C.ptr(xyz_c), _C.ptr(dirs_c), _C.ptr(depth_c), _C.ptr(frame.tri_c),
+                                                _C.ptr(keep[0]), _C.ptr(keep[1]),
+                                                float(self.min_separation) if keep[0] is None else 0.0,
+                                                _C.ptr(final_count), _C.ptr(dropped),
+                                                ctypes.c_void_p(host.data_ptr()) if publish else None, 1, _C.stream()),
+                         "qf_pack_tiles")
             frame.hit_count = final_count
             frame.dropped_dev = None if publish else dropped
             ev_flag.record()
@@ -671,7 +710,8 @@
             raise ValueError("sample_frame_device: origins / vectors must be the camera's full pixel grid")
         self._settle_deferred_policy()
         if self.want_raster(camera):
-            hit_tri, hit_t, hit_count, overflow = self._hits_raster_frame(o, d, k, camera)
+            hit_tri, hit_t, hit_count, overflow = self._hits_raster_frame(o, d, k, camera,
+                                                                          bins=self._hit_bins_ready(k, camera))
         else:
             hit_tri, hit_t, hit_count = self._hits_bvh(o, d, k, camera.width)
             overflow = None
@@ -715,7 +755,7 @@
         job = _C.FrameJob()
         job.camera = ctypes.addressof(camera)
         job.rays_o, job.rays_d, job.n_rays, job.max_hits = o.data_ptr(), d.data_ptr(), n, k
-        job.cull_chunks = 1 if getattr(camera, "cull", False) else 0
+        job.cull_chunks = (1 if getattr(camera, "cull", False) else 0) | (0 if self.hit_bins else 2)
         job.min_separation = float(self.min_separation)
         job.hit_tri, job.hit_t, job.hit_count = hit_tri.data_ptr(), hit_t.data_ptr(), counts.data_ptr()
         job.final_count, job.tile_base = final_count.data_ptr(), tile_base.data_ptr()
```

Result: faster. 409.7 million rays/s (median of 6 runs) (+2.6%).
